# cdglissov/recurrent-flows-msc

Measured on AMD Instinct MI355X. Metric: frames/sec, RFN SM-MNIST 64x64 train step (fwd+bwd+Adam), higher is better.
Workload: dtype f32 (forward convolutions fp32-grade: fused scaled-fp16 split f16x3s / three-piece bf16x6 split; gradient convolutions bf16x3 split MFMA; fp32 accumulate everywhere); 1 GPU; RFN SM-MNIST 64x64 canonical (K=10 L=5 Hd=256 h=200 z=56), global_batch=32, seq_len=20, train step; global_batch=32, seq_len=20, parallelism=dp1

## Files before the change

include/rfn_hip.h:

```cpp
#ifndef RFN_HIP_H
#define RFN_HIP_H

#ifdef __cplusplus
extern "C" {
#endif

typedef void* rfn_stream_t;

int rfn_abi_version(void);
const char* rfn_last_error(void);

int rfn_squeeze2d_f32(const float* x, long x_ns, float* y, long y_ns, int N, int C, int H, int W, int undo,
                      rfn_stream_t stream);

int rfn_channel_stats_f32(const float* x, long x_ns, float* mean, float* var_unbiased, int N, int C, int HW,
                          rfn_stream_t stream);

int rfn_actnorm_invconv_fwd_f32(const float* x, long x_ns, const float* bias, const float* logs, const float* Wm,
                                float* z, long z_ns, int N, int C, int HW, rfn_stream_t stream);
int rfn_actnorm_invconv_bwd_f32(const float* x, long x_ns, const float* bias, const float* logs, const float* Wm,
                                const float* gz, long gz_ns, float* gx, long gx_ns, float* gW, float* gbias,
                                float* glogs, int N, int C, int HW, rfn_stream_t stream);
#define RFN_INVCONV_MAX_STEPS 32
#define RFN_INVCONV_MAX_CHANNELS 96
int rfn_invconv_weights_fwd_f32(const float* const* p, const float* const* lower, const float* const* upper,
                                const float* const* log_s, const float* const* sign_s, float* W, float* logdet, int K,
                                int C, int HW, rfn_stream_t stream);
int rfn_invconv_weights_bwd_f32(const float* const* p, const float* const* lower, const float* const* upper,
                                const float* const* log_s, const float* const* sign_s, const float* gW, const float* gc,
                                float* g_lower, float* g_upper, float* g_log_s, int K, int C, int HW, rfn_stream_t stream);
int rfn_invconv_actnorm_rev_f32(const float* z, long z_ns, const float* bias, const float* logs, const float* Winv,
                                float* x, long x_ns, int N, int C, int HW, rfn_stream_t stream);

int rfn_conv2d_fwd_f32(const float* in1, long in1_ns, int C1, const float* in2, long in2_ns, int C2,
                       const float* wpk, float* out1, long out1_ns, float* out2, long out2_ns, int Cout,
                       int cout_split, int acc1, int acc2, int N, int H, int W, int ks, int ep_mode,
                       const float* p0, const float* p1, int act, rfn_stream_t stream);
const char* rfn_conv2d_kernel_label_f32(int ks, int Cout, int N, int H, int W);

int rfn_conv2d_fwd_bf16x3(const float* in1, long in1_ns, int C1, const float* in2, long in2_ns, int C2,
                          const float* wpk, float* out1, long out1_ns, float* out2, long out2_ns, int Cout,
                          int cout_split, int acc1, int acc2, int N, int H, int W, int ks, int ep_mode,
                          const float* p0, const float* p1, int act, rfn_stream_t stream);
long rfn_packed_weight_size_bf16x3(int Cout, int Cin, int ks);
int rfn_pack_conv_weight_bf16x3(const float* w, float* wpk, int Cout, int Cin, int ks, int transpose_flip,
                                rfn_stream_t stream);
long rfn_packed_weight_size_bf16x6(int Cout, int Cin, int ks);
int rfn_pack_conv_weight_bf16x6(const float* w, float* wpk, int Cout, int Cin, int ks, int transpose_flip,
                                rfn_stream_t stream);
int rfn_conv2d_fwd_bf16x6(const float* in1, long in1_ns, int C1, const float* in2, long in2_ns, int C2,
                          const float* wpk, float* out1, long out1_ns, float* out2, long out2_ns, int Cout,
                          int cout_split, int acc1, int acc2, int N, int H, int W, int ks, int ep_mode,
                          const float* p0, const float* p1, int act, rfn_stream_t stream);
const char* rfn_conv2d_kernel_label_bf16x3(int npl, int ks, int C1, int C2, int Cout, int cout_split, int acc1,
                                          int ep_mode, int N, int H, int W);

int rfn_conv3x3_fewcin_supported(int Cin, int Cout);
int rfn_conv3x3_fewcin_fwd_f32(const float* in, long in_ns, int Cin, const float* w, float* out, long out_ns, int Cout,
                               int N, int H, int W, rfn_stream_t stream);
int rfn_conv3x3_c1_wgrad16_f32(const float* in, long in_ns, const float* g, long g_ns, float* gw, int N, int H, int W,
                               rfn_stream_t stream);

int rfn_conv2d_dgrad_act_rows_bf16x3(int N, int H, int W, int ks, int Cout, int Cin);
int rfn_conv2d_dgrad_act_bf16x3(const float* gin, long gin_ns, int Cin, const float* wpk, const float* y, long y_ns,
                                const float* logs, int act, float* out, long out_ns, float* part, int Cout, int N,
                                int H, int W, int ks, rfn_stream_t stream);

typedef struct {
    const float* w;
    float* wpk;
    int Cout, Cin, ks, mode;
} rfn_pack_desc;
int rfn_pack_conv_weights_hostdescs_bf16x3(const void* descs_host, int n, rfn_stream_t stream);

typedef struct {
    const float* w1;
    const float* w2;
    const float* w3;
    float* dst;
    int Cin, C;
} rfn_po_pack_desc;
int rfn_coupling_po_supported(int N, int C, int Cc, int Hd, int H, int W);
long rfn_coupling_po_packed_bytes(int Cin, int C);
int rfn_coupling_po_pack(const void* descs_device, int n, rfn_stream_t stream);
int rfn_coupling_po_fwd(const float* z, long z_ns, const float* cond, long cond_ns, const void* wpk, const float* n1b,
                        const float* n1l, const float* n2b, const float* n2l, float* h1, long h1_ns, float* h2,
                        long h2_ns, float* P, long P_ns, float* m1, float* m2, int N, int C, int Cc, int H, int W, int act,
                        rfn_stream_t stream);
long rfn_coupling_po_mask_floats(int N, int H, int W);
int rfn_coupling_po_bwd_supported(int N, int C, int H, int W);
long rfn_coupling_po_bwd_packed_bytes(int C);
int rfn_coupling_po_pack_bwd(const void* descs_device, int n, rfn_stream_t stream);
long rfn_coupling_po_bwd_part_floats(int N, int H, int W);
int rfn_coupling_po_bwd(const float* go, long go_ns, const void* wpk, const float* n1l, const float* n2l,
                        const float* m_h1, const float* m_h2, float* ga2, long ga2_ns, float* ga1, long ga1_ns,
                        float* part, int N, int C, int H, int W, int act, rfn_stream_t stream);
int rfn_coupling_po_bwd_finish(const float* const* part, const float* const* w1, const float* const* gw1,
                               const float* const* n1b, const float* const* w2, const float* const* gw2,
                               const float* const* n2b, float* const* out, int n, int nblk, int K1,
                               rfn_stream_t stream);

int rfn_gather_affine_f32(const float* P, const float* o_in, long o_ns, const float* b3, const float* l3, float* o_out,
                          float* z, long z_ns, const float* scale, const float* scale_shift, float* logdet,
                          int clamp_type, int N, int C, int H, int W, rfn_stream_t stream);
int rfn_affine_zeros_bwd_f32(const float* zout, long zout_ns, const float* o, long o_ns, const float* gout, long gout_ns,
                             const float* glogdet, const float* scale, const float* scale_shift, const float* l3,
                             float* gz, long gz_ns, float* gpre, long gpre_ns, float* gscale, float* gscale_shift,
                             float* gb3, float* gl3, int clamp_type, int N, int C, int HW, rfn_stream_t stream);

int rfn_glow_shell_fwd_f32(float* z, long z_ns, const float* P, const float* o_in, long o_ns, const float* b3,
                           const float* l3, float* o_out, const float* scale, const float* scale_shift, float* logdet,
                           int clamp_type, const float* bias, const float* logs, const float* Wm, float* znext,
                           long znext_ns, int ld_const, int N, int C, int H, int W, rfn_stream_t stream);
long rfn_glow_shell_fwd_ld_floats(int N, int C, int H, int W);
int rfn_logdet_reduce_f32(const float* part, int n_launch, float* logdet, int accumulate, int N, int C, int H, int W,
                          rfn_stream_t stream);
const char* rfn_glow_shell_fwd_kernel_label(int N, int C, int H, int W, int head);
const char* rfn_glow_shell_bwd_kernel_label(int N, int C, int HW, int tail);
int rfn_glow_shell_supported(int N, int C, int H, int W);
int rfn_glow_shell_bwd_f32(const float* x, long x_ns, const float* bias, const float* logs, const float* Wm,
                           const float* gz, long gz_ns, float* gW, float* gbias, float* glogs, const float* o, long o_ns,
                           const float* glogdet, const float* scale, const float* scale_shift, const float* l3,
                           float* gz_prev, long gz_prev_ns, float* gpre, long gpre_ns, float* gscale,
                           float* gscale_shift, float* gb3, float* gl3, int clamp_type, int ld_const, int N, int C,
                           int HW, rfn_stream_t stream);
int rfn_actnorm_invconv_bwd_ld_f32(const float* x, long x_ns, const float* bias, const float* logs, const float* Wm,
                                   const float* gz, long gz_ns, float* gx, long gx_ns, float* gW, float* gbias,
                                   float* glogs, const float* glogdet, int N, int C, int HW, rfn_stream_t stream);

int rfn_dgrad_small_supported(int N, int Cin, int Cout, int H, int W);
int rfn_conv3x3_smallcout_bf16x3(const float* in, long in_ns, int Cin, const float* wpk, float* out1, long out1_ns,
                                 float* out2, long out2_ns, int Cout, int cout_split, int acc1, int acc2, int N, int H,
                                 int W, rfn_stream_t stream);

int rfn_gemm_wgrad_bf16x3(const float* a, long a_ns, int M, const float* b, long b_ns, int Nc, float* gw, int F, int HW,
                          rfn_stream_t stream);
int rfn_gemm_wgrad_grouped_bf16x3(const float* const* a, long a_ns, int M, const float* const* b, long b_ns, int Nc,
                                  float* const* gw, int G, int F, int HW, rfn_stream_t stream);
const char* rfn_gemm_wgrad_kernel_label_bf16x3(int M, int Nc, long a_ns, long b_ns, int G, int F, int HW);
int rfn_conv3x3_wgrad_implicit_bf16x3(const float* g, long g_ns, int Cout, const float* in1, long in1_ns, int C1,
                                      const float* in2, long in2_ns, int C2, float* gw, int F, int H, int W,
                                      rfn_stream_t stream);
int rfn_conv3x3_wgrad_implicit_grouped_bf16x3(const float* const* g, long g_ns, int Cout, const float* const* in1,
                                              long in1_ns, int C1, const float* const* in2, long in2_ns, int C2,
                                              float* const* gw, int G, int F, int H, int W, rfn_stream_t stream);
const char* rfn_conv3x3_wgrad_implicit_kernel_label_bf16x3(int Cout, long g_ns, int G, int F, int H, int W);
int rfn_im2col3x3_f32(const float* in1, long in1_ns, int C1, const float* in2, long in2_ns, int C2, float* out, int N,
                      int H, int W, rfn_stream_t stream);

long rfn_packed_weight_size(int Cout, int Cin, int ks);
int rfn_pack_conv_weight_f32(const float* w, float* wpk, int Cout, int Cin, int ks, int transpose_flip,
                             rfn_stream_t stream);

int rfn_conv2d_wgrad_f32(const float* in1, long in1_ns, int C1, const float* in2, long in2_ns, int C2,
                         const float* g, long g_ns, int Cout, float* gwt, int N, int H, int W, int ks,
                         rfn_stream_t stream);
const char* rfn_conv2d_wgrad_kernel_label_f32(int ks, int Cin, int Cout, int H, int W);
int rfn_wgrad_finish_f32(const float* gwt, float* gw, int Cout, int Cin, int ks, int accumulate, rfn_stream_t stream);

int rfn_tap_gather_f32(const float* P, const float* bias, const float* logs, float* o, int N, int C, int H, int W,
                       rfn_stream_t stream);
int rfn_tap_scatter_f32(const float* g, float* Gs, int N, int C, int H, int W, rfn_stream_t stream);

int rfn_conv_epilogue_bwd_f32(const float* y, long y_ns, const float* gy, long gy_ns, float* gu, long gu_ns,
                              const float* logs, float* gb, float* gl, int N, int C, int HW, int ep_mode, int act,
                              rfn_stream_t stream);

int rfn_affine_coupling_f32(float* z, long z_ns, const float* o, long o_ns, const float* scale,
                            const float* scale_shift, float* logdet, int clamp_type, int reverse, int N, int C, int HW,
                            rfn_stream_t stream);
int rfn_affine_coupling_bwd_f32(const float* zout, long zout_ns, const float* o, long o_ns, const float* gout,
                                long gout_ns, const float* glogdet, const float* scale, const float* scale_shift,
                                float* gz, long gz_ns, float* go, long go_ns, float* gscale, float* gscale_shift,
                                int clamp_type, int N, int C, int HW, rfn_stream_t stream);

int rfn_gauss_logp_f32(const float* z, long z_ns, const float* o, long o_ns, float* logp, int layout, int std_mode,
                       int N, int Cz, int HW, rfn_stream_t stream);
int rfn_gauss_logp_bwd_f32(const float* z, long z_ns, const float* o, long o_ns, const float* glogp, float* gz,
                           long gz_ns, float* go, long go_ns, int layout, int std_mode, int N, int Cz, int HW,
                           rfn_stream_t stream);
int rfn_gauss_sample_f32(const float* o, long o_ns, const float* eps, float* z, long z_ns, float temperature, int layout,
                         int std_mode, int N, int Cz, int HW, rfn_stream_t stream);

int rfn_latent_step_fwd_f32(const float* enc, const float* pri, const float* eps_p, const float* eps_q, float* zt,
                            float* zxt, float* kl, float* em, float* es, int B, int ZHW, int res_q, rfn_stream_t stream);
int rfn_latent_step_bwd_f32(const float* enc, const float* pri, const float* eps_p, const float* eps_q,
                            const float* g_zt, long g_zt_ns, const float* g_zxt, long g_zxt_ns, const float* g_kl,
                            const float* g_em, const float* g_es, float* g_enc, float* g_pri, int B, int ZHW, int res_q,
                            rfn_stream_t stream);

long rfn_smallmap_packed_size(int Cout, int Cin, int H, int W, int transpose);
int rfn_smallmap_pack_bf16x3(const float* w, int Cout, int Cin, int H, int W, int transpose, float* packed,
                             rfn_stream_t stream);
typedef struct {
    const float* w;
    float* packed;
    int Cout, Cin, H, W, transpose, pad_;
} rfn_smallmap_pack_desc;
int rfn_smallmap_pack_batched_bf16x3(const void* descs_host, int n, rfn_stream_t stream);
int rfn_smallmap_dense_bf16x3(const float* a, const float* y, float slope_in, const float* packed, const float* bias,
                              const float* add, int act_out, float slope_out, float* out, float* a_out, int B, int K, int N,
                              int HW, rfn_stream_t stream);

int rfn_smallmap_dense_pair_bf16x3(const float* a0, const float* y0, float slope_in0, const float* packed0,
                                   const float* bias0, const float* add0, int act_out0, float slope_out0, float* out0,
                                   float* a_out0, int K0, int N0, const float* a1, const float* y1, float slope_in1,
                                   const float* packed1, const float* bias1, const float* add1, int act_out1,
                                   float slope_out1, float* out1, float* a_out1, int K1, int N1, int B, int HW,
                                   rfn_stream_t stream);

int rfn_smallmap_conv_bf16x3(const float* in1, long in1_ns, int C1, const float* in2, long in2_ns, int C2,
                             const float* packed, float* out1, long out1_ns, float* out2, long out2_ns, int Cout,
                             int cout_split, int acc1, int N, int H, int W, int ep_mode, const float* p0,
                             const float* p1, int act, rfn_stream_t stream);

long rfn_stepbn_scratch_floats(int S, int B, int C);
int rfn_stepbn_fwd_f32(const float* x, const float* gamma, const float* beta, float* y, float* mean, float* var, float* acc,
                       float* run_mean, float* run_var, const float* coef, const float* coef_u, float decay,
                       long long* num_batches_tracked, int S, int B, int C, int HW, float eps, int act, float slope,
                       rfn_stream_t stream);
int rfn_stepbn_bwd_f32(const float* x, const float* gamma, const float* beta, const float* g, const float* mean,
                       const float* var, float* sums, float* gx, float* ggamma, float* gbeta, int S, int B, int C, int HW,
                       float eps, int act, float slope, int stage, int world, rfn_stream_t stream);
int rfn_stepbn_apply_f32(const float* x, const float* gamma, const float* beta, float* y, const float* mean,
                         const float* var, int S, int B, int C, int HW, float eps, int act, float slope,
                         rfn_stream_t stream);
const char* rfn_stepbn_kernel_label(int S, int B, int C, int HW, int aligned, int bwd);

const char* rfn_latent_step_kernel_label(int B, int ZHW);
const char* rfn_convlstm_gates_kernel_label(int N, int Hc, int HW);
int rfn_convlstm_gates_fwd_f32(const float* cc, const float* c_prev, long c_ns, const float* Wci, const float* Wcf,
                               const float* Wco, float* h_out, long h_ns, float* c_out, long co_ns, float* gates,
                               int N, int Hc, int HW, rfn_stream_t stream);
int rfn_convlstm_gates_bwd_f32(const float* gates, const float* c_prev, long c_ns, const float* c_out, long co_ns,
                               const float* gh, long gh_ns, const float* gc_next, long gcn_ns, const float* Wci,
                               const float* Wcf, const float* Wco, float* gcc, float* gc_prev, long gcp_ns, int N,
                               int Hc, int HW, rfn_stream_t stream);

typedef struct rfn_adam_entry {
    float* p;
    const float* g;
    float* m;
    float* v;
    long n;
    int step_offset;
    int reserved;
} rfn_adam_entry;
int rfn_adam_chunk_elems(void);
int rfn_adam_step_f32(const rfn_adam_entry* table, const int* chunks, int n_chunks, double lr, double beta1, double beta2,
                      double eps, double weight_decay, int t, rfn_stream_t stream);

int rfn_frame_quality_u8(const void* a, long a_ns, const void* b, long b_ns, float* mse, float* psnr, float* ssim,
                         int N, int C, int H, int W, rfn_stream_t stream);

int rfn_moving_mnist_render_f32(const void* digits, int N, float* out, long long* traj, int B, int T, int C, int S,
                                int num_digits, int step_length, int deterministic, long seed, long split,
                                long first_id, rfn_stream_t stream);

int rfn_clip_gather_u8_f32(const void* store, long n_frames, const void* first, float* out, int B, int T, int C, int Cs,
                           int H, int W, rfn_stream_t stream);

#define RFN_SHEET_MAX_ROWS 32
typedef struct rfn_sheet_row {
    const void* ptr;
    long step;
    int kind;
    int count;
} rfn_sheet_row;
int rfn_sheet_max_rows(void);
int rfn_sheet_compose_u8(const void* rows_table, int R, int N, int C, int H, int W, int gutter, int bg, int n_bits,
                         int range_half, int lead, long out_addr, rfn_stream_t stream);

int rfn_lpips_alex_sizes(int H, int W, long long* out);
int rfn_lpips_alex_weight_layout(long long* out);
int rfn_lpips_alex_features_u8(const void* frames, long frame_stride, int N, int C, int H, int W, const float* wpack,
                               long wpack_floats, float* feats_out, float* workspace, long workspace_floats,
                               rfn_stream_t stream);
int rfn_lpips_alex_distance(const float* feats_a, const float* feats_b, const float* lin, int N, int H, int W,
                            float* per_layer_out, float* out, rfn_stream_t stream);

int rfn_i3d_same(int in, int k, int s, long long* out);
int rfn_i3d_conv_pack_dims(int Cin, int Cout, int k, long long* out);
int rfn_i3d_conv3d_f32(const float* in, long in_floats, int N, int T, int H, int W, int Cin, const float* wpack,
                       long wpack_floats, const float* bias, int Cout, int k, int stride, int relu, float* out,
                       long out_floats, int out_coff, int out_pitch, rfn_stream_t stream);
int rfn_i3d_maxpool3d_f32(const float* in, long in_floats, int N, int T, int H, int W, int C, int kt, int khw, int st,
                          int shw, float* out, long out_floats, rfn_stream_t stream);
int rfn_i3d_resize_u8(const void* frames, long frame_stride, int NF, int C, int H, int W, float* out, long out_floats,
                      rfn_stream_t stream);
int rfn_i3d_head_f32(const float* in, long in_floats, int N, int Tp, int P, int C, const float* wpack, long wpack_floats,
                     const float* bias, int Cout, float* out, rfn_stream_t stream);

#ifdef __cplusplus
}
#endif
#endif
```

recurrent-flows-msc_amd/csrc/wgrad_bf16x3.hip:

```cpp
#include "conv_common.h"

typedef __bf16 bf16x8 __attribute__((ext_vector_type(8)));

struct GemmWgradParams {
    const float* a;
    const float* b;
    long a_ns, b_ns;
    int M, N;
    float* gw;
    int F, HW;
    long total;
    int n_stages;
    const float* b2;
    long b2_ns;
    int C1, C2, H, W;
    int G, mtiles;
    const float* ga[16];
    const float* gb[16];
    const float* gb2[16];
    float* ggw[16];
};

struct WgOperands { const float* a; const float* b; const float* b2; float* gw; };
__device__ __forceinline__ WgOperands wg_operands(const GemmWgradParams& p, const int grp) {
    WgOperands o = {p.a, p.b, p.b2, p.gw};
    if (p.G > 0) {
#pragma unroll
        for (int i = 0; i < 16; ++i)
            if (i == grp) {
                o.a = p.ga[i];
                o.b = p.gb[i];
                o.b2 = p.gb2[i];
                o.gw = p.ggw[i];
            }
    }
    return o;
}

template <int WM, int WN, int TM, int TN, int KP, int IMPL = 0>
__global__ __launch_bounds__(64 * WM * WN) void gemm_wgrad_b3_kernel(const GemmWgradParams p) {
    constexpr int NT = 64 * WM * WN;
    constexpr int BM = 32 * TM * WM, BN = 32 * TN * WN;
    constexpr int NU = KP / 8;
    constexpr int RS = NU + 1;
    constexpr int AU = (BM * NU + NT - 1) / NT;
    constexpr int BU = (BN * NU + NT - 1) / NT;
    constexpr bool AX = (BM * NU) % NT == 0, BX = (BN * NU) % NT == 0;
    static_assert(WM * WN == 4 || WM * WN == 8, "tile/stage shape");
    extern __shared__ __attribute__((aligned(16))) unsigned char lds_raw[];
    bf16x8* Ah = reinterpret_cast<bf16x8*>(lds_raw);
    bf16x8* Al = Ah + BM * RS;
    bf16x8* Bh = Al + BM * RS;
    bf16x8* Bl = Bh + BN * RS;
    const int tid = threadIdx.x, lane = tid & 63, wave = tid >> 6;
    const int wm = wave / WN, wn = wave % WN;
    const int l31 = lane & 31, kk = lane >> 5;
    const int grp = p.G > 0 ? (int)blockIdx.z / p.mtiles : 0;
    const int m0 = (p.G > 0 ? (int)blockIdx.z - grp * p.mtiles : (int)blockIdx.z) * BM, n0 = blockIdx.y * BN;
    const WgOperands ops_ = wg_operands(p, grp);
    const float* const pa_ = ops_.a;
    const float* const pb_ = ops_.b;
    const float* const pb2_ = ops_.b2;
    float* const pgw_ = ops_.gw;

    f32x16 acc[TM][TN];
#pragma unroll
    for (int i = 0; i < TM; ++i)
#pragma unroll
        for (int j = 0; j < TN; ++j)
#pragma unroll
            for (int r = 0; r < 16; ++r) acc[i][j][r] = 0.f;

    float4 ast[AU][2], bst[BU][2];
    static_assert(NT % NU == 0, "k-group must be a per-thread constant");
    const int kg = tid % NU, r0 = tid / NU;
    const unsigned uHW = (unsigned)p.HW;
    bool okq[2] = {false, false};
    const float* uplane[IMPL ? BU : 1];
    long uns[IMPL ? BU : 1];
    int udy[IMPL ? BU : 1], udx[IMPL ? BU : 1];
    float bedge[IMPL ? BU : 1];
    unsigned rowmask = 0, edgemask = 0;
    if (IMPL) {
#pragma unroll
        for (int u = 0; u < BU; ++u) {
            int row = n0 + r0 + u * (NT / NU);
            if (row >= p.N) row = 0;
            const int ci = row / 9, tap = row - ci * 9;
            udy[u] = tap / 3 - 1;
            udx[u] = tap % 3 - 1;
            const bool first = ci < p.C1;
            uplane[u] = first ? pb_ + (long)ci * p.HW : pb2_ + (long)(ci - p.C1) * p.HW;
            uns[u] = first ? p.b_ns : p.b2_ns;
        }
    }
    auto prefetch = [&](int stage) {
        const unsigned q0 = (unsigned)stage * KP + 8u * kg;
        long offa[2], offb[2];
#pragma unroll
        for (int h = 0; h < 2; ++h) {
            const unsigned q = q0 + 4u * h;
            okq[h] = stage < p.n_stages && q < (unsigned)p.total;
            const unsigned qq = okq[h] ? q : 0u;
            const unsigned f = qq / uHW, px = qq - f * uHW;
            offa[h] = (long)f * p.a_ns + px;
            offb[h] = (long)f * p.b_ns + px;
        }
#pragma unroll
        for (int u = 0; u < AU; ++u) {
            const int row = m0 + r0 + u * (NT / NU);
            const float* base = pa_ + (long)(row < p.M ? row : 0) * p.HW;
#pragma unroll
            for (int h = 0; h < 2; ++h) ast[u][h] = *reinterpret_cast<const float4*>(base + offa[h]);
        }
        if (IMPL) {
            const unsigned qq = okq[0] ? q0 : 0u;
            const unsigned f = qq / uHW, pix = qq - f * uHW;
            const int y = (int)(pix / (unsigned)p.W), x0 = (int)(pix - (unsigned)y * (unsigned)p.W);
            rowmask = 0;
            edgemask = 0;
#pragma unroll
            for (int u = 0; u < BU; ++u) {
                const int yy = y + udy[u];
                const bool rok = yy >= 0 && yy < p.H;
                const float* src = uplane[u] + (long)f * uns[u] + (rok ? yy : y) * p.W + x0;
                bst[u][0] = *reinterpret_cast<const float4*>(src);
                bst[u][1] = *reinterpret_cast<const float4*>(src + 4);
                const bool eok = udx[u] < 0 ? x0 > 0 : x0 + 8 < p.W;
                bedge[u] = src[eok ? (udx[u] < 0 ? -1 : 8) : 0];
                rowmask |= (rok ? 1u : 0u) << u;
                edgemask |= (eok ? 1u : 0u) << u;
            }
        } else {
#pragma unroll
            for (int u = 0; u < BU; ++u) {
                const int row = n0 + r0 + u * (NT / NU);
                const float* base = pb_ + (long)(row < p.N ? row : 0) * p.HW;
#pragma unroll
                for (int h = 0; h < 2; ++h) bst[u][h] = *reinterpret_cast<const float4*>(base + offb[h]);
            }
        }
    };
    auto split_store_shift = [&](const float4 (&src)[2], float edge, int dx, bool okr, bool eok, bf16x8* hi_p, bf16x8* lo_p) {
        const float v[8] = {src[0].x, src[0].y, src[0].z, src[0].w, src[1].x, src[1].y, src[1].z, src[1].w};
        bf16x8 hi, lo;
#pragma unroll
        for (int c = 0; c < 8; ++c) {
            const float left = c == 0 ? (eok ? edge : 0.f) : v[c > 0 ? c - 1 : 0];
            const float right = c == 7 ? (eok ? edge : 0.f) : v[c < 7 ? c + 1 : 7];
            float x = dx < 0 ? left : (dx > 0 ? right : v[c]);
            x = (okr && okq[0]) ? x : 0.f;
            const __bf16 h = (__bf16)x;
            hi[c] = h;
            lo[c] = (__bf16)(x - (float)h);
        }
        *hi_p = hi;
        *lo_p = lo;
    };
    auto split_store = [&](const float4 (&src)[2], bool okr, bf16x8* hi_p, bf16x8* lo_p) {
        const float v[8] = {src[0].x, src[0].y, src[0].z, src[0].w, src[1].x, src[1].y, src[1].z, src[1].w};
        bf16x8 hi, lo;
#pragma unroll
        for (int c = 0; c < 8; ++c) {
            const float x = (okr && okq[c >> 2]) ? v[c] : 0.f;
            const __bf16 h = (__bf16)x;
            hi[c] = h;
            lo[c] = (__bf16)(x - (float)h);
        }
        *hi_p = hi;
        *lo_p = lo;
    };
    auto commit = [&]() {
#pragma unroll
        for (int u = 0; u < AU; ++u) {
            const int o = (r0 + u * (NT / NU)) * RS + kg;
            if (AX || r0 + u * (NT / NU) < BM) split_store(ast[u], m0 + r0 + u * (NT / NU) < p.M, Ah + o, Al + o);
        }
#pragma unroll
        for (int u = 0; u < BU; ++u) {
            const int o = (r0 + u * (NT / NU)) * RS + kg;
            if (BX || r0 + u * (NT / NU) < BN) {
                const bool okr = n0 + r0 + u * (NT / NU) < p.N;
                if (IMPL)
                    split_store_shift(bst[u], bedge[u], udx[u], okr && ((rowmask >> u) & 1u), (edgemask >> u) & 1u, Bh + o,
                                      Bl + o);
                else
                    split_store(bst[u], okr, Bh + o, Bl + o);
            }
        }
    };

    const int arow = (wm * TM * 32 + l31) * RS + kk;
    const int brow = (wn * TN * 32 + l31) * RS + kk;
    int stage = blockIdx.x;
    prefetch(stage);
    for (; stage < p.n_stages; stage += gridDim.x) {
        __syncthreads();
        commit();
        __syncthreads();
        prefetch(stage + gridDim.x);
        __builtin_amdgcn_sched_barrier(0);
#pragma unroll WM * WN == 8 && KP > 32 ? 1 : KP / 16
        for (int s = 0; s < KP / 16; ++s) {
            bf16x8 ah[TM], al[TM], bh[TN], bl[TN];
#pragma unroll
            for (int i = 0; i < TM; ++i) {
                ah[i] = Ah[arow + i * 32 * RS + 2 * s];
                al[i] = Al[arow + i * 32 * RS + 2 * s];
            }
#pragma unroll
            for (int j = 0; j < TN; ++j) {
                bh[j] = Bh[brow + j * 32 * RS + 2 * s];
                bl[j] = Bl[brow + j * 32 * RS + 2 * s];
            }
#pragma unroll
            for (int i = 0; i < TM; ++i)
#pragma unroll
                for (int j = 0; j < TN; ++j) {
                    acc[i][j] = __builtin_amdgcn_mfma_f32_32x32x16_bf16(al[i], bh[j], acc[i][j], 0, 0, 0);
                    acc[i][j] = __builtin_amdgcn_mfma_f32_32x32x16_bf16(ah[i], bl[j], acc[i][j], 0, 0, 0);
                    acc[i][j] = __builtin_amdgcn_mfma_f32_32x32x16_bf16(ah[i], bh[j], acc[i][j], 0, 0, 0);
                }
        }
    }
#pragma unroll
    for (int i = 0; i < TM; ++i)
#pragma unroll
        for (int j = 0; j < TN; ++j) {
            const int n = n0 + (wn * TN + j) * 32 + l31;
#pragma unroll
            for (int r = 0; r < 16; ++r) {
                const int m = m0 + (wm * TM + i) * 32 + (r & 3) + 8 * (r >> 2) + 4 * kk;
                if (m < p.M && n < p.N) atomicAdd(&pgw_[(long)m * p.N + n], acc[i][j][r]);
            }
        }
}

template <int N_>
__device__ __forceinline__ void wg_wait_vm() { asm volatile("s_waitcnt vmcnt(%0)" ::"n"(N_) : "memory"); }

__device__ __forceinline__ void wg_split8(const f32x4 lo4, const f32x4 hi4, bf16x8& hi, bf16x8& lo) {
    const float v[8] = {lo4[0], lo4[1], lo4[2], lo4[3], hi4[0], hi4[1], hi4[2], hi4[3]};
#pragma unroll
    for (int c = 0; c < 8; ++c) {
        const __bf16 h = (__bf16)v[c];
        hi[c] = h;
        lo[c] = (__bf16)(v[c] - (float)h);
    }
}

template <int WM, int WN, int TM, int TN, int KP, int NST>
__global__ __launch_bounds__(64 * WM * WN) void gemm_wgrad_dma_kernel(const GemmWgradParams p) {
    constexpr int NW = WM * WN;
    constexpr int BM = 32 * TM * WM, BN = 32 * TN * WN;
    constexpr int UPR = KP / 4, RPP = 64 / UPR, SWD = 16 / UPR;
    constexpr int RB = KP * 4;
    constexpr int ROWS = BM + BN, PIECES = ROWS / RPP, PPW = PIECES / NW;
    constexpr int STAGE = ROWS * RB;
    constexpr int NK = KP / 16, NU_ = NK * TM;
    static_assert(KP == 16 || KP == 32, "stage width");
    static_assert(PIECES % NW == 0 && BM % 16 == 0 && NST >= 2, "pieces shared evenly; swizzle period divides BM");
    constexpr bool LOOK = NST >= 3;
    static_assert(TM % 2 == 0 && TM >= TN + 1, "pipeline parities");
    extern __shared__ __attribute__((aligned(16))) unsigned char lds_raw[];
    const int tid = threadIdx.x, lane = tid & 63;
    const int wave = __builtin_amdgcn_readfirstlane(tid >> 6);
    const int wm = wave / WN, wn = wave % WN;
    const int l31 = lane & 31, kk = lane >> 5;
    const int grp = p.G > 0 ? (int)blockIdx.z / p.mtiles : 0;
    const int m0 = (p.G > 0 ? (int)blockIdx.z - grp * p.mtiles : (int)blockIdx.z) * BM, n0 = blockIdx.y * BN;
    const WgOperands ops_ = wg_operands(p, grp);
    const float* const pa_ = ops_.a;
    const float* const pb_ = ops_.b;
    float* const pgw_ = ops_.gw;

    f32x16 acc[TM][TN];
#pragma unroll
    for (int i = 0; i < TM; ++i)
#pragma unroll
        for (int j = 0; j < TN; ++j)
#pragma unroll
            for (int r = 0; r < 16; ++r) acc[i][j][r] = 0.f;

    const float* prow[PPW];
    bool pisa[PPW];
#pragma unroll
    for (int j = 0; j < PPW; ++j) {
        const int r = RPP * (wave + j * NW) + lane / UPR;
        const int u = (lane & (UPR - 1)) ^ ((r / SWD) & (UPR - 1));
        pisa[j] = r < BM;
        if (pisa[j]) {
            int row = m0 + r;
            row = row < p.M ? row : p.M - 1;
            prow[j] = pa_ + (long)row * p.HW + 4 * u;
        } else {
            int row = n0 + r - BM;
            row = row < p.N ? row : p.N - 1;
            prow[j] = pb_ + (long)row * p.HW + 4 * u;
        }
    }
    const unsigned uHW = (unsigned)p.HW;
    const int S = gridDim.x;
    const int nmine = (p.n_stages - (int)blockIdx.x + S - 1) / S;
    long offa = 0, offb = 0;
    auto stage_offsets = [&](int t) {
        t = t < nmine ? t : nmine - 1;
        const unsigned q0 = (unsigned)(blockIdx.x + t * S) * KP;
        const unsigned f = q0 / uHW, px = q0 - f * uHW;
        offa = (long)f * p.a_ns + px;
        offb = (long)f * p.b_ns + px;
    };
    auto piece = [&](const int j, const int slot) {
        __builtin_amdgcn_global_load_lds((const __attribute__((address_space(1))) void*)(prow[j] + (pisa[j] ? offa : offb)),
                                         (__attribute__((address_space(3))) void*)(lds_raw + slot * STAGE + (wave + j * NW) * 1024),
                                         16, 0, 0);
    };

    int aoff[TM], boff[TN];
#pragma unroll
    for (int i = 0; i < TM; ++i) {
        const int r = (wm * TM + i) * 32 + l31;
        aoff[i] = r * RB + (((2 * kk) ^ ((r / SWD) & (UPR - 1))) << 4);
    }
#pragma unroll
    for (int j = 0; j < TN; ++j) {
        const int r = BM + (wn * TN + j) * 32 + l31;
        boff[j] = r * RB + (((2 * kk) ^ ((r / SWD) & (UPR - 1))) << 4);
    }
    auto raw = [&](const unsigned char* sb, const int off, const int s_, f32x4 (&r)[2]) {
        const int o = off ^ (s_ << 6);
        r[0] = *reinterpret_cast<const f32x4*>(sb + o);
        r[1] = *reinterpret_cast<const f32x4*>(sb + (o ^ 16));
    };

#pragma unroll
    for (int t = 0; t < NST - 1; ++t) {
        stage_offsets(t);
#pragma unroll
        for (int j = 0; j < PPW; ++j) piece(j, t);
    }
    f32x4 ra[2][2], rb[TN][2];
    bf16x8 ah[2], al[2], bh[2][TN], bl[2][TN];
    auto first_fragments = [&](const unsigned char* sb0) {
#pragma unroll
        for (int j = 0; j < TN; ++j) raw(sb0, boff[j], 0, rb[j]);
        raw(sb0, aoff[0], 0, ra[0]);
        raw(sb0, aoff[1], 0, ra[1]);
#pragma unroll
        for (int j = 0; j < TN; ++j) wg_split8(rb[j][0], rb[j][1], bh[0][j], bl[0][j]);
        wg_split8(ra[0][0], ra[0][1], ah[0], al[0]);
    };
    if (LOOK) {
        wg_wait_vm<(NST - 2) * PPW>();
        __builtin_amdgcn_s_barrier();
        first_fragments(lds_raw);
    }

    int slot = 0;
    for (int it = 0; it < nmine; ++it) {
        wg_wait_vm<LOOK ? (NST - 3) * PPW : 0>();
        __builtin_amdgcn_s_barrier();
        const int nslot = slot + 1 == NST ? 0 : slot + 1;
        const int fslot = slot == 0 ? NST - 1 : slot - 1;
        const unsigned char* sb = lds_raw + slot * STAGE;
        const unsigned char* sn = lds_raw + nslot * STAGE;
        stage_offsets(it + NST - 1);
        if (!LOOK) {
#pragma unroll
            for (int j = 0; j < PPW; ++j) piece(j, fslot);
            first_fragments(sb);
        }
#pragma unroll
        for (int u = 0; u < NU_; ++u) {
            const int s_ = u / TM, i = u % TM, cur = u & 1, kb = s_ & 1;
            if (u + 2 < NU_) raw(sb, aoff[(u + 2) % TM], (u + 2) / TM, ra[cur]);
            else if (LOOK) raw(sn, aoff[(u + 2) % TM], 0, ra[cur]);
            if (i == 0) {
#pragma unroll
                for (int j = 0; j < TN; ++j) {
                    if (s_ + 1 < NK) raw(sb, boff[j], s_ + 1, rb[j]);
                    else if (LOOK) raw(sn, boff[j], 0, rb[j]);
                }
            }
            if (LOOK && u == 0) {
#pragma unroll
                for (int j = 0; j < PPW; ++j) piece(j, fslot);
            }
#pragma unroll
            for (int j = 0; j < TN; ++j) {
                acc[i][j] = __builtin_amdgcn_mfma_f32_32x32x16_bf16(al[cur], bh[kb][j], acc[i][j], 0, 0, 0);
                acc[i][j] = __builtin_amdgcn_mfma_f32_32x32x16_bf16(ah[cur], bl[kb][j], acc[i][j], 0, 0, 0);
                acc[i][j] = __builtin_amdgcn_mfma_f32_32x32x16_bf16(ah[cur], bh[kb][j], acc[i][j], 0, 0, 0);
            }
            if (LOOK || u + 1 < NU_) wg_split8(ra[cur ^ 1][0], ra[cur ^ 1][1], ah[cur ^ 1], al[cur ^ 1]);
            if (i >= 1 && i <= TN && (LOOK || s_ + 1 < NK))
                wg_split8(rb[i - 1][0], rb[i - 1][1], bh[kb ^ 1][i - 1], bl[kb ^ 1][i - 1]);
        }
        if (LOOK && (NK & 1)) {
#pragma unroll
            for (int j = 0; j < TN; ++j) {
                bh[0][j] = bh[1][j];
                bl[0][j] = bl[1][j];
            }
        }
        if (!LOOK) {
            __builtin_amdgcn_sched_group_barrier(0x020, PPW, 0);
            __builtin_amdgcn_sched_group_barrier(0x100, 2 * TN + 4, 0);
            __builtin_amdgcn_sched_group_barrier(0x002, 30 * (TN + 1), 0);
        }
#pragma unroll
        for (int g = 0; g < NU_ * TN * 3; ++g) {
            __builtin_amdgcn_sched_group_barrier(0x008, 1, 0);
            __builtin_amdgcn_sched_group_barrier(0x002, 6, 0);
            __builtin_amdgcn_sched_group_barrier(0x100, 1, 0);
            if (LOOK && g < PPW) __builtin_amdgcn_sched_group_barrier(0x020, 1, 0);
        }
        slot = nslot;
    }
    wg_wait_vm<0>();
#pragma unroll
    for (int i = 0; i < TM; ++i)
#pragma unroll
        for (int j = 0; j < TN; ++j) {
            const int n = n0 + (wn * TN + j) * 32 + l31;
#pragma unroll
            for (int r = 0; r < 16; ++r) {
                const int m = m0 + (wm * TM + i) * 32 + (r & 3) + 8 * (r >> 2) + 4 * kk;
                if (m < p.M && n < p.N) atomicAdd(&pgw_[(long)m * p.N + n], acc[i][j][r]);
            }
        }
}

template <int WM, int WN, int TM, int TN, int KP, int NST>
static void launch_gemm_wgrad_dma(GemmWgradParams& p, hipStream_t s) {
    constexpr int BM = 32 * TM * WM, BN = 32 * TN * WN;
    p.n_stages = (int)(p.total / KP);
    const size_t lds = (size_t)NST * (BM + BN) * KP * 4;
    const int tiles = ceil_div(p.M, BM) * ceil_div(p.N, BN);
    const int G = p.G > 0 ? p.G : 1;
    int S = 256 / (tiles * G);
    if (S > p.n_stages / 8) S = p.n_stages / 8;
    if (S < 1) S = 1;
    auto kern = gemm_wgrad_dma_kernel<WM, WN, TM, TN, KP, NST>;
    (void)hipFuncSetAttribute((const void*)kern, hipFuncAttributeMaxDynamicSharedMemorySize, (int)lds);
    p.mtiles = ceil_div(p.M, BM);
    dim3 grid(S, ceil_div(p.N, BN), p.mtiles * G);
    hipLaunchKernelGGL(kern, grid, dim3(64 * WM * WN), lds, s, p);
}

template <int WM, int WN, int TM, int TN>
__global__ __launch_bounds__(64 * WM * WN) void gemm_wgrad_dma_impl_kernel(const GemmWgradParams p) {
    constexpr int NW = WM * WN, NT = 64 * NW, KP = 32, NK = KP / 16;
    constexpr int BM = 32 * TM * WM, BN = 32 * TN * WN;
    constexpr int PIECES = BM / 8, PPW = PIECES / NW;
    constexpr int ASLOT = BM * 128;
    constexpr int NU = KP / 8, RS = NU + 1;
    constexpr int BU = (BN * NU + NT - 1) / NT;
    constexpr int BPLANE = BN * RS;
    static_assert(PIECES % NW == 0 && NT % NU == 0 && TM % 2 == 0, "shares / parities");
    extern __shared__ __attribute__((aligned(16))) unsigned char lds_raw[];
    bf16x8* const Bbase = reinterpret_cast<bf16x8*>(lds_raw + 2 * ASLOT);
    const int tid = threadIdx.x, lane = tid & 63;
    const int wave = __builtin_amdgcn_readfirstlane(tid >> 6);
    const int wm = wave / WN, wn = wave % WN;
    const int l31 = lane & 31, kk = lane >> 5;
    const int grp = p.G > 0 ? (int)blockIdx.z / p.mtiles : 0;
    const int m0 = (p.G > 0 ? (int)blockIdx.z - grp * p.mtiles : (int)blockIdx.z) * BM, n0 = blockIdx.y * BN;
    const WgOperands ops_ = wg_operands(p, grp);
    const float* const pa_ = ops_.a;
    const float* const pb_ = ops_.b;
    const float* const pb2_ = ops_.b2;
    float* const pgw_ = ops_.gw;

    f32x16 acc[TM][TN];
#pragma unroll
    for (int i = 0; i < TM; ++i)
#pragma unroll
        for (int j = 0; j < TN; ++j)
#pragma unroll
            for (int r = 0; r < 16; ++r) acc[i][j][r] = 0.f;

    const float* prow[PPW];
#pragma unroll
    for (int j = 0; j < PPW; ++j) {
        const int r = 8 * (wave + j * NW) + (lane >> 3);
        const int u = (lane & 7) ^ ((r >> 1) & 7);
        int row = m0 + r;
        row = row < p.M ? row : p.M - 1;
        prow[j] = pa_ + (long)row * p.HW + 4 * u;
    }
    int aoff[TM];
#pragma unroll
    for (int i = 0; i < TM; ++i) {
        const int r = (wm * TM + i) * 32 + l31;
        aoff[i] = r * 128 + (((2 * kk) ^ ((r >> 1) & 7)) << 4);
    }
    const int kg = tid % NU, r0 = tid / NU;
    const float* uplane[BU];
    long uns[BU];
    int udy[BU], udx[BU];
#pragma unroll
    for (int u = 0; u < BU; ++u) {
        int row = n0 + r0 + u * (NT / NU);
        if (row >= p.N) row = 0;
        const int ci = row / 9, tap = row - ci * 9;
        udy[u] = tap / 3 - 1;
        udx[u] = tap % 3 - 1;
        const bool first = ci < p.C1;
        uplane[u] = first ? pb_ + (long)ci * p.HW : pb2_ + (long)(ci - p.C1) * p.HW;
        uns[u] = first ? p.b_ns : p.b2_ns;
    }
    const unsigned uHW = (unsigned)p.HW;
    const int S = gridDim.x;
    const int nmine = (p.n_stages - (int)blockIdx.x + S - 1) / S;
    float4 bst[BU][2];
    float bedge[BU];
    unsigned rowmask = 0, edgemask = 0;
    auto fetch = [&](int t, const int slot) {
        t = t < nmine ? t : nmine - 1;
        const unsigned q0 = (unsigned)(blockIdx.x + t * S) * KP;
        const unsigned f = q0 / uHW, px = q0 - f * uHW;
        const long offa = (long)f * p.a_ns + px;
#pragma unroll
        for (int j = 0; j < PPW; ++j)
            __builtin_amdgcn_global_load_lds((const __attribute__((address_space(1))) void*)(prow[j] + offa),
                                             (__attribute__((address_space(3))) void*)(lds_raw + slot * ASLOT + (wave + j * NW) * 1024),
                                             16, 0, 0);
        const unsigned pix = px + 8u * kg;
        const int y = (int)(pix / (unsigned)p.W), x0 = (int)(pix - (unsigned)y * (unsigned)p.W);
        rowmask = 0;
        edgemask = 0;
#pragma unroll
        for (int u = 0; u < BU; ++u) {
            const int yy = y + udy[u];
            const bool rok = yy >= 0 && yy < p.H;
            const float* src = uplane[u] + (long)f * uns[u] + (rok ? yy : y) * p.W + x0;
            bst[u][0] = *reinterpret_cast<const float4*>(src);
            bst[u][1] = *reinterpret_cast<const float4*>(src + 4);
            const bool eok = udx[u] < 0 ? x0 > 0 : x0 + 8 < p.W;
            bedge[u] = src[eok ? (udx[u] < 0 ? -1 : 8) : 0];
            rowmask |= (rok ? 1u : 0u) << u;
            edgemask |= (eok ? 1u : 0u) << u;
        }
    };
    auto commit = [&](const int buf) {
        bf16x8* Bh = Bbase + buf * 2 * BPLANE;
        bf16x8* Bl = Bh + BPLANE;
#pragma unroll
        for (int u = 0; u < BU; ++u) {
            const int row = r0 + u * (NT / NU);
            if (row < BN) {
                const bool okr = n0 + row < p.N && ((rowmask >> u) & 1u);
                const bool eok = (edgemask >> u) & 1u;
                const float v[8] = {bst[u][0].x, bst[u][0].y, bst[u][0].z, bst[u][0].w,
                                    bst[u][1].x, bst[u][1].y, bst[u][1].z, bst[u][1].w};
                bf16x8 hi, lo;
#pragma unroll
                for (int c = 0; c < 8; ++c) {
                    const float left = c == 0 ? (eok ? bedge[u] : 0.f) : v[c > 0 ? c - 1 : 0];
                    const float right = c == 7 ? (eok ? bedge[u] : 0.f) : v[c < 7 ? c + 1 : 7];
                    float x = udx[u] < 0 ? left : (udx[u] > 0 ? right : v[c]);
                    x = okr ? x : 0.f;
                    const __bf16 h = (__bf16)x;
                    hi[c] = h;
                    lo[c] = (__bf16)(x - (float)h);
                }
                Bh[row * RS + kg] = hi;
                Bl[row * RS + kg] = lo;
            }
        }
    };
    auto rawA = [&](const unsigned char* sb, const int i, const int s_, f32x4 (&r)[2]) {
        const int o = aoff[i] ^ (s_ << 6);
        r[0] = *reinterpret_cast<const f32x4*>(sb + o);
        r[1] = *reinterpret_cast<const f32x4*>(sb + (o ^ 16));
    };
    const int brow = (wn * TN * 32 + l31) * RS + kk;

    fetch(0, 0);
    commit(0);
    int slot = 0;
    for (int it = 0; it < nmine; ++it) {
        wg_wait_vm<0>();
        asm volatile("s_waitcnt lgkmcnt(0)" ::: "memory");
        __builtin_amdgcn_s_barrier();
        fetch(it + 1, slot ^ 1);
        const unsigned char* sb = lds_raw + slot * ASLOT;
        const bf16x8* Bh = Bbase + slot * 2 * BPLANE;
        const bf16x8* Bl = Bh + BPLANE;
        f32x4 ra[2][TM][2];
        bf16x8 ah[2][TM], al[2][TM];
#pragma unroll
        for (int i = 0; i < TM; ++i) rawA(sb, i, 0, ra[0][i]);
#pragma unroll
        for (int i = 0; i < TM; ++i) wg_split8(ra[0][i][0], ra[0][i][1], ah[0][i], al[0][i]);
#pragma unroll
        for (int s_ = 0; s_ < NK; ++s_) {
            const int cur = s_ & 1;
            if (s_ + 1 < NK) {
#pragma unroll
                for (int i = 0; i < TM; ++i) rawA(sb, i, s_ + 1, ra[cur ^ 1][i]);
            }
            bf16x8 bh[TN], bl[TN];
#pragma unroll
            for (int j = 0; j < TN; ++j) {
                bh[j] = Bh[brow + j * 32 * RS + 2 * s_];
                bl[j] = Bl[brow + j * 32 * RS + 2 * s_];
            }
#pragma unroll
            for (int i = 0; i < TM; ++i)
#pragma unroll
                for (int j = 0; j < TN; ++j) {
                    acc[i][j] = __builtin_amdgcn_mfma_f32_32x32x16_bf16(al[cur][i], bh[j], acc[i][j], 0, 0, 0);
                    acc[i][j] = __builtin_amdgcn_mfma_f32_32x32x16_bf16(ah[cur][i], bl[j], acc[i][j], 0, 0, 0);
                    acc[i][j] = __builtin_amdgcn_mfma_f32_32x32x16_bf16(ah[cur][i], bh[j], acc[i][j], 0, 0, 0);
                }
            if (s_ + 1 < NK) {
#pragma unroll
                for (int i = 0; i < TM; ++i) wg_split8(ra[cur ^ 1][i][0], ra[cur ^ 1][i][1], ah[cur ^ 1][i], al[cur ^ 1][i]);
            }
        }
        commit(slot ^ 1);
        slot ^= 1;
    }
    wg_wait_vm<0>();
#pragma unroll
    for (int i = 0; i < TM; ++i)
#pragma unroll
        for (int j = 0; j < TN; ++j) {
            const int n = n0 + (wn * TN + j) * 32 + l31;
#pragma unroll
            for (int r = 0; r < 16; ++r) {
                const int m = m0 + (wm * TM + i) * 32 + (r & 3) + 8 * (r >> 2) + 4 * kk;
                if (m < p.M && n < p.N) atomicAdd(&pgw_[(long)m * p.N + n], acc[i][j][r]);
            }
        }
}

template <int WM, int WN, int TM, int TN>
static void launch_gemm_wgrad_dma_impl(GemmWgradParams& p, hipStream_t s) {
    constexpr int BM = 32 * TM * WM, BN = 32 * TN * WN;
    p.n_stages = (int)(p.total / 32);
    const size_t lds = (size_t)2 * BM * 128 + (size_t)2 * 2 * BN * 5 * 16;
    const int tiles = ceil_div(p.M, BM) * ceil_div(p.N, BN);
    const int G = p.G > 0 ? p.G : 1;
    int S = 256 / (tiles * G);
    if (S > p.n_stages / 8) S = p.n_stages / 8;
    if (S < 1) S = 1;
    auto kern = gemm_wgrad_dma_impl_kernel<WM, WN, TM, TN>;
    (void)hipFuncSetAttribute((const void*)kern, hipFuncAttributeMaxDynamicSharedMemorySize, (int)lds);
    p.mtiles = ceil_div(p.M, BM);
    dim3 grid(S, ceil_div(p.N, BN), p.mtiles * G);
    hipLaunchKernelGGL(kern, grid, dim3(64 * WM * WN), lds, s, p);
}

template <int WM, int WN, int TM, int TN, int KP, int IMPL = 0>
static void launch_gemm_wgrad(GemmWgradParams& p, hipStream_t s) {
    constexpr int BM = 32 * TM * WM, BN = 32 * TN * WN;
    p.n_stages = (int)((p.total + KP - 1) / KP);
    size_t lds = (size_t)2 * (BM + BN) * (KP / 8 + 1) * 16;
    int tiles = ceil_div(p.M, BM) * ceil_div(p.N, BN);
    static const int sdiv = getenv("RFN_WGRAD_SPLIT") ? atoi(getenv("RFN_WGRAD_SPLIT")) : 0;
    const int G = p.G > 0 ? p.G : 1;
    int S = (sdiv > 0 ? sdiv : (WM * WN == 8 ? 256 : 512)) / (tiles * G);
    if (S > p.n_stages / 4) S = p.n_stages / 4;
    if (S < 1) S = 1;
    auto kern = gemm_wgrad_b3_kernel<WM, WN, TM, TN, KP, IMPL>;
    if (lds > 65536) (void)hipFuncSetAttribute((const void*)kern, hipFuncAttributeMaxDynamicSharedMemorySize, (int)lds);
    p.mtiles = ceil_div(p.M, BM);
    dim3 grid(S, ceil_div(p.N, BN), p.mtiles * G);
    hipLaunchKernelGGL(kern, grid, dim3(64 * WM * WN), lds, s, p);
}

enum WgradB3Route { DMA_256x256, DMA_64x256, R_256x192, R_256x192_KP32, R_256x256, R_256x256_KP32, R_64x256, R_256x64,
                    R_128x128, IMPL_DMA_256x192, IMPL_256x192, IMPL_32x256, IMPL_128x128 };
static const char* const kWgradB3Labels[] = {
    "gemm_wgrad_dma_kernel<2,4,4,2,32,2>",
    "gemm_wgrad_dma_kernel<1,8,2,1,32,3>",
    "gemm_wgrad_b3_kernel<4,2,2,3,64>",
    "gemm_wgrad_b3_kernel<4,2,2,3,32>",
    "gemm_wgrad_b3_kernel<2,4,4,2,64>",
    "gemm_wgrad_b3_kernel<2,4,4,2,32>",
    "gemm_wgrad_b3_kernel<1,4,2,2,32>",
    "gemm_wgrad_b3_kernel<4,1,2,2,32>",
    "gemm_wgrad_b3_kernel<2,2,2,2,64>",
    "gemm_wgrad_dma_impl_kernel<4,2,2,3>",
    "gemm_wgrad_b3_kernel<4,2,2,3,64,1>",
    "gemm_wgrad_b3_kernel<1,4,1,2,32,1>",
    "gemm_wgrad_b3_kernel<2,2,2,2,64,1>",
};
static_assert(sizeof(kWgradB3Labels) / sizeof(kWgradB3Labels[0]) == IMPL_128x128 + 1, "one label per route");
static bool wgrad_dma_off() {
    static const int off = getenv("RFN_WGRAD_DMA") ? atoi(getenv("RFN_WGRAD_DMA")) == 0 : 0;
    return off;
}
static GemmWgradParams wgrad_shape(int M, int Nc, long a_ns, long b_ns, int G, int F, int HW) {
    GemmWgradParams p;
    memset(&p, 0, sizeof(p));
    p.M = M; p.N = Nc; p.a_ns = a_ns; p.b_ns = b_ns; p.G = G; p.F = F; p.HW = HW; p.total = (long)F * HW;
    return p;
}

static WgradB3Route choose_gemm_wgrad(const GemmWgradParams& p) {
    const int M = p.M, Nc = p.N;
    static const int variant = getenv("RFN_WGRAD_VARIANT") ? atoi(getenv("RFN_WGRAD_VARIANT")) : 0;
    if (variant == 0 && !wgrad_dma_off() && p.HW % 32 == 0 && p.total * (p.G > 0 ? p.G : 1) >= 100000 && p.total >= 2048 &&
        p.a_ns % 4 == 0 && p.b_ns % 4 == 0 && Nc > 128 && Nc % 256 == 0) {
        if (M >= 192) return DMA_256x256;
        if (M <= 64) return DMA_64x256;
    }
    if (variant != 1 && M > 128 && Nc > 128 && p.total >= 100000) {
        if (ceil_div(Nc, 192) * 192 < ceil_div(Nc, 256) * 256) return variant == 2 ? R_256x192_KP32 : R_256x192;
        return variant == 2 ? R_256x256_KP32 : R_256x256;
    }
    return M <= 64 ? R_64x256 : (Nc <= 64 ? R_256x64 : R_128x128);
}
extern "C" const char* rfn_gemm_wgrad_kernel_label_bf16x3(int M, int Nc, long a_ns, long b_ns, int G, int F, int HW) {
    return kWgradB3Labels[choose_gemm_wgrad(wgrad_shape(M, Nc, a_ns, b_ns, G, F, HW))];
}

static WgradB3Route choose_wgrad_implicit(const GemmWgradParams& p) {
    if (p.M > 128 && p.total * (p.G > 0 ? p.G : 1) >= 100000 && p.total >= 2048 && !wgrad_dma_off() && p.HW % 32 == 0 &&
        p.a_ns % 4 == 0)
        return IMPL_DMA_256x192;
    if (p.M > 128 && p.total >= 100000) return IMPL_256x192;
    return p.M <= 32 && p.G == 0 ? IMPL_32x256 : IMPL_128x128;
}
extern "C" const char* rfn_conv3x3_wgrad_implicit_kernel_label_bf16x3(int Cout, long g_ns, int G, int F, int H, int W) {
    return kWgradB3Labels[choose_wgrad_implicit(wgrad_shape(Cout, 0, g_ns, 0, G, F, H * W))];
}

static void launch_wgrad_route(GemmWgradParams& p, WgradB3Route r, hipStream_t s) {
    switch (r) {
        case DMA_256x256:      return launch_gemm_wgrad_dma<2, 4, 4, 2, 32, 2>(p, s);
        case DMA_64x256:       return launch_gemm_wgrad_dma<1, 8, 2, 1, 32, 3>(p, s);
        case R_256x192:        return launch_gemm_wgrad<4, 2, 2, 3, 64>(p, s);
        case R_256x192_KP32:   return launch_gemm_wgrad<4, 2, 2, 3, 32>(p, s);
        case R_256x256:        return launch_gemm_wgrad<2, 4, 4, 2, 64>(p, s);
        case R_256x256_KP32:   return launch_gemm_wgrad<2, 4, 4, 2, 32>(p, s);
        case R_64x256:         return launch_gemm_wgrad<1, 4, 2, 2, 32>(p, s);
        case R_256x64:         return launch_gemm_wgrad<4, 1, 2, 2, 32>(p, s);
        case R_128x128:        return launch_gemm_wgrad<2, 2, 2, 2, 64>(p, s);
        case IMPL_DMA_256x192: return launch_gemm_wgrad_dma_impl<4, 2, 2, 3>(p, s);
        case IMPL_256x192:     return launch_gemm_wgrad<4, 2, 2, 3, 64, 1>(p, s);
        case IMPL_32x256:      return launch_gemm_wgrad<1, 4, 1, 2, 32, 1>(p, s);
        case IMPL_128x128:     return launch_gemm_wgrad<2, 2, 2, 2, 64, 1>(p, s);
    }
}

extern "C" int rfn_gemm_wgrad_bf16x3(const float* a, long a_ns, int M, const float* b, long b_ns, int Nc, float* gw,
                                     int F, int HW, rfn_stream_t stream) {
    RFN_CHECK_ARG(a && b && gw && M > 0 && Nc > 0 && F >= 0 && HW > 0, -1);
    RFN_CHECK_ARG(HW % 4 == 0 && a_ns % 4 == 0 && b_ns % 4 == 0, -2);
    RFN_CHECK_ARG((((uintptr_t)a | (uintptr_t)b) & 15) == 0, -3);
    RFN_CHECK_ARG((long)F * HW < (1L << 31) - 4096, -4);
    if (F == 0) return 0;
    GemmWgradParams p;
    memset(&p, 0, sizeof(p));
    p.a = a; p.b = b; p.a_ns = a_ns; p.b_ns = b_ns; p.M = M; p.N = Nc; p.gw = gw; p.F = F; p.HW = HW;
    p.total = (long)F * HW;
    launch_wgrad_route(p, choose_gemm_wgrad(p), (hipStream_t)stream);
    RFN_LAUNCH_CHECK();
    return 0;
}

extern "C" int rfn_gemm_wgrad_grouped_bf16x3(const float* const* a, long a_ns, int M, const float* const* b, long b_ns,
                                             int Nc, float* const* gw, int G, int F, int HW, rfn_stream_t stream) {
    RFN_CHECK_ARG(a && b && gw && G >= 1 && G <= 16 && M > 0 && Nc > 0 && F >= 0 && HW > 0, -1);
    RFN_CHECK_ARG(HW % 4 == 0 && a_ns % 4 == 0 && b_ns % 4 == 0, -2);
    RFN_CHECK_ARG((long)F * HW < (1L << 31) - 4096, -4);
    if (F == 0) return 0;
    GemmWgradParams p;
    memset(&p, 0, sizeof(p));
    for (int g = 0; g < G; ++g) {
        RFN_CHECK_ARG(a[g] && b[g] && gw[g] && (((uintptr_t)a[g] | (uintptr_t)b[g]) & 15) == 0, -3);
        p.ga[g] = a[g]; p.gb[g] = b[g]; p.gb2[g] = b[g]; p.ggw[g] = gw[g];
    }
    p.G = G; p.a = a[0]; p.b = b[0]; p.gw = gw[0];
    p.a_ns = a_ns; p.b_ns = b_ns; p.M = M; p.N = Nc; p.F = F; p.HW = HW;
    p.total = (long)F * HW;
    launch_wgrad_route(p, choose_gemm_wgrad(p), (hipStream_t)stream);
    RFN_LAUNCH_CHECK();
    return 0;
}

extern "C" int rfn_conv3x3_wgrad_implicit_bf16x3(const float* g, long g_ns, int Cout, const float* in1, long in1_ns, int C1,
                                                 const float* in2, long in2_ns, int C2, float* gw, int F, int H, int W,
                                                 rfn_stream_t stream) {
    RFN_CHECK_ARG(g && in1 && gw && Cout > 0 && C1 > 0 && C2 >= 0 && (C2 == 0 || in2) && F >= 0 && H > 0 && W > 0, -1);
    RFN_CHECK_ARG(W % 8 == 0 && g_ns % 4 == 0 && in1_ns % 4 == 0 && (C2 == 0 || in2_ns % 4 == 0), -2);
    RFN_CHECK_ARG((((uintptr_t)g | (uintptr_t)in1 | (uintptr_t)(C2 ? in2 : in1)) & 15) == 0, -3);
    RFN_CHECK_ARG((long)F * H * W < (1L << 31) - 4096, -4);
    if (F == 0) return 0;
    GemmWgradParams p;
    memset(&p, 0, sizeof(p));
    p.a = g; p.a_ns = g_ns; p.M = Cout; p.b = in1; p.b_ns = in1_ns; p.b2 = C2 ? in2 : in1; p.b2_ns = C2 ? in2_ns : in1_ns;
    p.C1 = C1; p.C2 = C2; p.H = H; p.W = W; p.N = 9 * (C1 + C2); p.gw = gw; p.F = F; p.HW = H * W;
    p.total = (long)F * H * W;
    launch_wgrad_route(p, choose_wgrad_implicit(p), (hipStream_t)stream);
    RFN_LAUNCH_CHECK();
    return 0;
}

extern "C" int rfn_conv3x3_wgrad_implicit_grouped_bf16x3(const float* const* g, long g_ns, int Cout,
                                                         const float* const* in1, long in1_ns, int C1,
                                                         const float* const* in2, long in2_ns, int C2, float* const* gw,
                                                         int G, int F, int H, int W, rfn_stream_t stream) {
    RFN_CHECK_ARG(g && in1 && gw && G >= 1 && G <= 16 && Cout > 0 && C1 > 0 && C2 >= 0 && (C2 == 0 || in2) && F >= 0, -1);
    RFN_CHECK_ARG(H > 0 && W > 0 && W % 8 == 0 && g_ns % 4 == 0 && in1_ns % 4 == 0 && (C2 == 0 || in2_ns % 4 == 0), -2);
    RFN_CHECK_ARG((long)F * H * W < (1L << 31) - 4096, -4);
    if (F == 0) return 0;
    GemmWgradParams p;
    memset(&p, 0, sizeof(p));
    for (int i = 0; i < G; ++i) {
        RFN_CHECK_ARG(g[i] && in1[i] && gw[i] && (C2 == 0 || in2[i]), -3);
        RFN_CHECK_ARG((((uintptr_t)g[i] | (uintptr_t)in1[i] | (uintptr_t)(C2 ? in2[i] : in1[i])) & 15) == 0, -3);
        p.ga[i] = g[i]; p.gb[i] = in1[i]; p.gb2[i] = C2 ? in2[i] : in1[i]; p.ggw[i] = gw[i];
    }
    p.G = G; p.a = g[0]; p.b = in1[0]; p.b2 = p.gb2[0]; p.gw = gw[0];
    p.a_ns = g_ns; p.M = Cout; p.b_ns = in1_ns; p.b2_ns = C2 ? in2_ns : in1_ns;
    p.C1 = C1; p.C2 = C2; p.H = H; p.W = W; p.N = 9 * (C1 + C2); p.F = F; p.HW = H * W;
    p.total = (long)F * H * W;
    launch_wgrad_route(p, choose_wgrad_implicit(p), (hipStream_t)stream);
    RFN_LAUNCH_CHECK();
    return 0;
}

__global__ void im2col3x3_kernel(const float* __restrict__ in1, long in1_ns, int C1, const float* __restrict__ in2,
                                 long in2_ns, int C2, float* __restrict__ out, int N, int H, int W) {
    const int Cin = C1 + C2;
    const long HW = (long)H * W, total = (long)N * 9 * Cin * HW;
    for (long idx = (long)blockIdx.x * blockDim.x + threadIdx.x; idx < total; idx += (long)gridDim.x * blockDim.x) {
        const int x = (int)(idx % W);
        long r = idx / W;
        const int y = (int)(r % H);
        r /= H;
        const int tc = (int)(r % (9 * Cin));
        const long n = r / (9 * Cin);
        const int t = tc / Cin, ci = tc - t * Cin;
        const int yy = y + t / 3 - 1, xx = x + t % 3 - 1;
        float v = 0.f;
        if (yy >= 0 && yy < H && xx >= 0 && xx < W)
            v = ci < C1 ? in1[n * in1_ns + (long)ci * HW + (long)yy * W + xx]
                        : in2[n * in2_ns + (long)(ci - C1) * HW + (long)yy * W + xx];
        out[idx] = v;
    }
}
__global__ void im2col3x3_v4_kernel(const float* __restrict__ in1, long in1_ns, int C1, const float* __restrict__ in2,
                                    long in2_ns, int C2, float* __restrict__ out, int N, int H, int W) {
    const int Cin = C1 + C2, HW4 = H * W / 4, W4 = W / 4;
    const long HW = (long)H * W, total = (long)N * 9 * Cin * HW4;
    for (long idx = (long)blockIdx.x * blockDim.x + threadIdx.x; idx < total; idx += (long)gridDim.x * blockDim.x) {
        const int q = (int)(idx % HW4);
        const long r = idx / HW4;
        const int tc = (int)(r % (9 * Cin));
        const long n = r / (9 * Cin);
        const int t = tc / Cin, ci = tc - t * Cin;
        const int y = q / W4, x0 = (q - y * W4) * 4;
        const int yy = y + t / 3 - 1, dx = t % 3 - 1;
        float4 v = {0.f, 0.f, 0.f, 0.f};
        if (yy >= 0 && yy < H) {
            const float* src = (ci < C1 ? in1 + n * in1_ns + (long)ci * HW : in2 + n * in2_ns + (long)(ci - C1) * HW) +
                               (long)yy * W;
            if (dx == 0) {
                v = *reinterpret_cast<const float4*>(src + x0);
            } else {
                const float4 c = *reinterpret_cast<const float4*>(src + x0);
                if (dx < 0) {
                    v.x = x0 > 0 ? src[x0 - 1] : 0.f;
                    v.y = c.x; v.z = c.y; v.w = c.z;
                } else {
                    v.x = c.y; v.y = c.z; v.z = c.w;
                    v.w = x0 + 4 < W ? src[x0 + 4] : 0.f;
                }
            }
        }
        *reinterpret_cast<float4*>(out + idx * 4) = v;
    }
}
extern "C" int rfn_im2col3x3_f32(const float* in1, long in1_ns, int C1, const float* in2, long in2_ns, int C2,
                                 float* out, int N, int H, int W, rfn_stream_t stream) {
    RFN_CHECK_ARG(in1 && out && C1 > 0 && C2 >= 0 && (C2 == 0 || in2) && N >= 0 && H > 0 && W > 0, -1);
    if (N == 0) return 0;
    hipStream_t s = (hipStream_t)stream;
    const long HWl = (long)H * W;
    if (W % 4 == 0 && in1_ns % 4 == 0 && (C2 == 0 || in2_ns % 4 == 0) && HWl % 4 == 0 &&
        (((uintptr_t)in1 | (uintptr_t)out | (uintptr_t)(C2 ? in2 : in1)) & 15) == 0) {
        long tot4 = (long)N * 9 * (C1 + C2) * (HWl / 4);
        int grid4 = (int)((tot4 + 255) / 256 < 16384 ? (tot4 + 255) / 256 : 16384);
        hipLaunchKernelGGL(im2col3x3_v4_kernel, dim3(grid4), dim3(256), 0, s, in1, in1_ns, C1, in2, in2_ns, C2, out, N, H, W);
        RFN_LAUNCH_CHECK();
        return 0;
    }
    long tot = (long)N * 9 * (C1 + C2) * H * W;
    int grid = (int)((tot + 255) / 256 < 8192 ? (tot + 255) / 256 : 8192);
    hipLaunchKernelGGL(im2col3x3_kernel, dim3(grid), dim3(256), 0, (hipStream_t)stream, in1, in1_ns, C1, in2, in2_ns, C2,
                       out, N, H, W);
    RFN_LAUNCH_CHECK();
    return 0;
}
```

recurrent-flows-msc_amd/rfn_hip/lib.py:

```python
import ctypes
import os

import torch

_HERE = os.path.dirname(os.path.abspath(__file__))
LIB_PATH = os.path.join(_HERE, "librfn_hip.so")

_c_f = ctypes.c_void_p
_c_i = ctypes.c_int
_c_l = ctypes.c_long
_c_s = ctypes.c_void_p

SIGNATURES = {
    "rfn_abi_version": [],
    "rfn_last_error": [],
    "rfn_squeeze2d_f32": [_c_f, _c_l, _c_f, _c_l, _c_i, _c_i, _c_i, _c_i, _c_i, _c_s],
    "rfn_channel_stats_f32": [_c_f, _c_l, _c_f, _c_f, _c_i, _c_i, _c_i, _c_s],
    "rfn_actnorm_invconv_fwd_f32": [_c_f, _c_l, _c_f, _c_f, _c_f, _c_f, _c_l, _c_i, _c_i, _c_i, _c_s],
    "rfn_actnorm_invconv_bwd_f32": [_c_f, _c_l, _c_f, _c_f, _c_f, _c_f, _c_l, _c_f, _c_l, _c_f, _c_f, _c_f,
                                    _c_i, _c_i, _c_i, _c_s],
    "rfn_invconv_weights_fwd_f32": [ctypes.c_void_p] * 5 + [_c_f, _c_f, _c_i, _c_i, _c_i, _c_s],
    "rfn_invconv_weights_bwd_f32": [ctypes.c_void_p] * 5 + [_c_f, _c_f, _c_f, _c_f, _c_f, _c_i, _c_i, _c_i, _c_s],
    "rfn_invconv_actnorm_rev_f32": [_c_f, _c_l, _c_f, _c_f, _c_f, _c_f, _c_l, _c_i, _c_i, _c_i, _c_s],
    "rfn_conv2d_fwd_f32": [_c_f, _c_l, _c_i, _c_f, _c_l, _c_i, _c_f, _c_f, _c_l, _c_f, _c_l, _c_i, _c_i, _c_i, _c_i,
                           _c_i, _c_i, _c_i, _c_i, _c_i, _c_f, _c_f, _c_i, _c_s],
    "rfn_conv2d_kernel_label_f32": [_c_i] * 5,
    "rfn_conv2d_fwd_bf16x3": [_c_f, _c_l, _c_i, _c_f, _c_l, _c_i, _c_f, _c_f, _c_l, _c_f, _c_l, _c_i, _c_i, _c_i, _c_i,
                              _c_i, _c_i, _c_i, _c_i, _c_i, _c_f, _c_f, _c_i, _c_s],
    "rfn_packed_weight_size_bf16x3": [_c_i, _c_i, _c_i],
    "rfn_pack_conv_weight_bf16x3": [_c_f, _c_f, _c_i, _c_i, _c_i, _c_i, _c_s],
    "rfn_packed_weight_size_bf16x6": [_c_i, _c_i, _c_i],
    "rfn_pack_conv_weight_bf16x6": [_c_f, _c_f, _c_i, _c_i, _c_i, _c_i, _c_s],
    "rfn_conv2d_fwd_bf16x6": [_c_f, _c_l, _c_i, _c_f, _c_l, _c_i, _c_f, _c_f, _c_l, _c_f, _c_l, _c_i, _c_i, _c_i, _c_i,
                              _c_i, _c_i, _c_i, _c_i, _c_i, _c_f, _c_f, _c_i, _c_s],
    "rfn_conv2d_kernel_label_bf16x3": [_c_i] * 11,
    "rfn_conv2d_dgrad_act_rows_bf16x3": [_c_i, _c_i, _c_i, _c_i, _c_i, _c_i],
    "rfn_conv2d_dgrad_act_bf16x3": [_c_f, _c_l, _c_i, _c_f, _c_f, _c_l, _c_f, _c_i, _c_f, _c_l, _c_f, _c_i, _c_i, _c_i,
                                    _c_i, _c_i, _c_s],
    "rfn_gather_affine_f32": [_c_f, _c_f, _c_l, _c_f, _c_f, _c_f, _c_f, _c_l, _c_f, _c_f, _c_f, _c_i, _c_i, _c_i, _c_i,
                              _c_i, _c_s],
    "rfn_affine_zeros_bwd_f32": [_c_f, _c_l, _c_f, _c_l, _c_f, _c_l, _c_f, _c_f, _c_f, _c_f, _c_f, _c_l, _c_f, _c_l, _c_f,
                                 _c_f, _c_f, _c_f, _c_i, _c_i, _c_i, _c_i, _c_s],
    "rfn_glow_shell_fwd_f32": [_c_f, _c_l, _c_f, _c_f, _c_l, _c_f, _c_f, _c_f, _c_f, _c_f, _c_f, _c_i, _c_f, _c_f, _c_f,
                               _c_f, _c_l, _c_i, _c_i, _c_i, _c_i, _c_i, _c_s],
    "rfn_glow_shell_bwd_f32": [_c_f, _c_l, _c_f, _c_f, _c_f, _c_f, _c_l, _c_f, _c_f, _c_f, _c_f, _c_l, _c_f, _c_f, _c_f,
                               _c_f, _c_f, _c_l, _c_f, _c_l, _c_f, _c_f, _c_f, _c_f, _c_i, _c_i, _c_i, _c_i, _c_i, _c_s],
    "rfn_actnorm_invconv_bwd_ld_f32": [_c_f, _c_l, _c_f, _c_f, _c_f, _c_f, _c_l, _c_f, _c_l, _c_f, _c_f, _c_f, _c_f, _c_i,
                                       _c_i, _c_i, _c_s],
    "rfn_dgrad_small_supported": [_c_i, _c_i, _c_i, _c_i, _c_i],
    "rfn_conv3x3_smallcout_bf16x3": [_c_f, _c_l, _c_i, _c_f, _c_f, _c_l, _c_f, _c_l, _c_i, _c_i, _c_i, _c_i, _c_i, _c_i,
                                     _c_i, _c_s],
    "rfn_gemm_wgrad_grouped_bf16x3": [_c_f, _c_l, _c_i, _c_f, _c_l, _c_i, _c_f, _c_i, _c_i, _c_i, _c_s],
    "rfn_conv3x3_wgrad_implicit_grouped_bf16x3": [_c_f, _c_l, _c_i, _c_f, _c_l, _c_i, _c_f, _c_l, _c_i, _c_f, _c_i, _c_i,
                                                  _c_i, _c_i, _c_s],
    "rfn_coupling_po_supported": [_c_i, _c_i, _c_i, _c_i, _c_i, _c_i],
    "rfn_coupling_po_packed_bytes": [_c_i, _c_i],
    "rfn_coupling_po_pack": [_c_f, _c_i, _c_s],
    "rfn_coupling_po_fwd": [_c_f, _c_l, _c_f, _c_l, _c_f, _c_f, _c_f, _c_f, _c_f, _c_f, _c_l, _c_f, _c_l, _c_f, _c_l,
                            _c_f, _c_f, _c_i, _c_i, _c_i, _c_i, _c_i, _c_i, _c_s],
    "rfn_glow_shell_fwd_ld_floats": [_c_i, _c_i, _c_i, _c_i],
    "rfn_logdet_reduce_f32": [_c_f, _c_i, _c_f, _c_i, _c_i, _c_i, _c_i, _c_i, _c_s],
    "rfn_glow_shell_fwd_kernel_label": [_c_i] * 5,
    "rfn_glow_shell_bwd_kernel_label": [_c_i] * 4,
    "rfn_glow_shell_supported": [_c_i] * 4,
    "rfn_coupling_po_mask_floats": [_c_i, _c_i, _c_i],
    "rfn_coupling_po_bwd_supported": [_c_i, _c_i, _c_i, _c_i],
    "rfn_coupling_po_bwd_packed_bytes": [_c_i],
    "rfn_coupling_po_pack_bwd": [_c_f, _c_i, _c_s],
    "rfn_coupling_po_bwd_part_floats": [_c_i, _c_i, _c_i],
    "rfn_coupling_po_bwd": [_c_f, _c_l, _c_f, _c_f, _c_f, _c_f, _c_f, _c_f, _c_l, _c_f, _c_l, _c_f, _c_i, _c_i, _c_i, _c_i,
                            _c_i, _c_s],
    "rfn_coupling_po_bwd_finish": [ctypes.c_void_p] * 8 + [_c_i, _c_i, _c_i, _c_s],
    "rfn_gemm_wgrad_bf16x3": [_c_f, _c_l, _c_i, _c_f, _c_l, _c_i, _c_f, _c_i, _c_i, _c_s],
    "rfn_conv3x3_wgrad_implicit_bf16x3": [_c_f, _c_l, _c_i, _c_f, _c_l, _c_i, _c_f, _c_l, _c_i, _c_f, _c_i, _c_i, _c_i,
                                          _c_s],
    "rfn_gemm_wgrad_kernel_label_bf16x3": [_c_i, _c_i, _c_l, _c_l, _c_i, _c_i, _c_i],
    "rfn_conv3x3_wgrad_implicit_kernel_label_bf16x3": [_c_i, _c_l, _c_i, _c_i, _c_i, _c_i],
    "rfn_im2col3x3_f32": [_c_f, _c_l, _c_i, _c_f, _c_l, _c_i, _c_f, _c_i, _c_i, _c_i, _c_s],
    "rfn_packed_weight_size": [_c_i, _c_i, _c_i],
    "rfn_pack_conv_weight_f32": [_c_f, _c_f, _c_i, _c_i, _c_i, _c_i, _c_s],
    "rfn_conv2d_wgrad_f32": [_c_f, _c_l, _c_i, _c_f, _c_l, _c_i, _c_f, _c_l, _c_i, _c_f, _c_i, _c_i, _c_i, _c_i, _c_s],
    "rfn_conv2d_wgrad_kernel_label_f32": [_c_i] * 5,
    "rfn_wgrad_finish_f32": [_c_f, _c_f, _c_i, _c_i, _c_i, _c_i, _c_s],
    "rfn_tap_gather_f32": [_c_f, _c_f, _c_f, _c_f, _c_i, _c_i, _c_i, _c_i, _c_s],
    "rfn_tap_scatter_f32": [_c_f, _c_f, _c_i, _c_i, _c_i, _c_i, _c_s],
    "rfn_conv_epilogue_bwd_f32": [_c_f, _c_l, _c_f, _c_l, _c_f, _c_l, _c_f, _c_f, _c_f, _c_i, _c_i, _c_i, _c_i, _c_i,
                                  _c_s],
    "rfn_affine_coupling_f32": [_c_f, _c_l, _c_f, _c_l, _c_f, _c_f, _c_f, _c_i, _c_i, _c_i, _c_i, _c_i, _c_s],
    "rfn_affine_coupling_bwd_f32": [_c_f, _c_l, _c_f, _c_l, _c_f, _c_l, _c_f, _c_f, _c_f, _c_f, _c_l, _c_f, _c_l,
                                    _c_f, _c_f, _c_i, _c_i, _c_i, _c_i, _c_s],
    "rfn_gauss_logp_f32": [_c_f, _c_l, _c_f, _c_l, _c_f, _c_i, _c_i, _c_i, _c_i, _c_i, _c_s],
    "rfn_gauss_logp_bwd_f32": [_c_f, _c_l, _c_f, _c_l, _c_f, _c_f, _c_l, _c_f, _c_l, _c_i, _c_i, _c_i, _c_i, _c_i,
                               _c_s],
    "rfn_gauss_sample_f32": [_c_f, _c_l, _c_f, _c_f, _c_l, ctypes.c_float, _c_i, _c_i, _c_i, _c_i, _c_i, _c_s],
    "rfn_latent_step_fwd_f32": [_c_f, _c_f, _c_f, _c_f, _c_f, _c_f, _c_f, _c_f, _c_f, _c_i, _c_i, _c_i, _c_s],
    "rfn_latent_step_bwd_f32": [_c_f, _c_f, _c_f, _c_f, _c_f, _c_l, _c_f, _c_l, _c_f, _c_f, _c_f, _c_f, _c_f, _c_i, _c_i, _c_i,
                                _c_s],
    "rfn_conv3x3_fewcin_supported": [_c_i, _c_i],
    "rfn_conv3x3_fewcin_fwd_f32": [_c_f, _c_l, _c_i, _c_f, _c_f, _c_l, _c_i, _c_i, _c_i, _c_i, _c_s],
    "rfn_conv3x3_c1_wgrad16_f32": [_c_f, _c_l, _c_f, _c_l, _c_f, _c_i, _c_i, _c_i, _c_s],
    "rfn_smallmap_packed_size": [_c_i, _c_i, _c_i, _c_i, _c_i],
    "rfn_smallmap_pack_bf16x3": [_c_f, _c_i, _c_i, _c_i, _c_i, _c_i, _c_f, _c_s],
    "rfn_smallmap_pack_batched_bf16x3": [ctypes.c_void_p, _c_i, _c_s],
    "rfn_pack_conv_weights_hostdescs_bf16x3": [ctypes.c_void_p, _c_i, _c_s],
    "rfn_smallmap_dense_bf16x3": [_c_f, _c_f, ctypes.c_float, _c_f, _c_f, _c_f, _c_i, ctypes.c_float, _c_f, _c_f, _c_i,
                                  _c_i, _c_i, _c_i, _c_s],
    "rfn_smallmap_dense_pair_bf16x3": [_c_f, _c_f, ctypes.c_float, _c_f, _c_f, _c_f, _c_i, ctypes.c_float, _c_f, _c_f, _c_i,
                                       _c_i, _c_f, _c_f, ctypes.c_float, _c_f, _c_f, _c_f, _c_i, ctypes.c_float, _c_f, _c_f,
                                       _c_i, _c_i, _c_i, _c_i, _c_s],
    "rfn_smallmap_conv_bf16x3": [_c_f, _c_l, _c_i, _c_f, _c_l, _c_i, _c_f, _c_f, _c_l, _c_f, _c_l, _c_i, _c_i, _c_i, _c_i,
                                 _c_i, _c_i, _c_i, _c_f, _c_f, _c_i, _c_s],
    "rfn_stepbn_scratch_floats": [_c_i, _c_i, _c_i],
    "rfn_stepbn_kernel_label": [_c_i] * 6,
    "rfn_convlstm_gates_kernel_label": [_c_i] * 3,
    "rfn_latent_step_kernel_label": [_c_i] * 2,
    "rfn_stepbn_fwd_f32": [_c_f, _c_f, _c_f, _c_f, _c_f, _c_f, _c_f, _c_f, _c_f, _c_f, _c_f, ctypes.c_float, ctypes.c_void_p,
                           _c_i, _c_i, _c_i, _c_i, ctypes.c_float, _c_i, ctypes.c_float, _c_s],
    "rfn_stepbn_bwd_f32": [_c_f, _c_f, _c_f, _c_f, _c_f, _c_f, _c_f, _c_f, _c_f, _c_f, _c_i, _c_i, _c_i, _c_i, ctypes.c_float,
                           _c_i, ctypes.c_float, _c_i, _c_i, _c_s],
    "rfn_stepbn_apply_f32": [_c_f, _c_f, _c_f, _c_f, _c_f, _c_f, _c_i, _c_i, _c_i, _c_i, ctypes.c_float, _c_i, ctypes.c_float,
                             _c_s],
    "rfn_adam_chunk_elems": [],
    "rfn_adam_step_f32": [ctypes.c_void_p, ctypes.c_void_p, _c_i, ctypes.c_double, ctypes.c_double, ctypes.c_double,
                          ctypes.c_double, ctypes.c_double, _c_i, _c_s],
    "rfn_convlstm_gates_fwd_f32": [_c_f, _c_f, _c_l, _c_f, _c_f, _c_f, _c_f, _c_l, _c_f, _c_l, _c_f, _c_i, _c_i, _c_i,
                                   _c_s],
    "rfn_convlstm_gates_bwd_f32": [_c_f, _c_f, _c_l, _c_f, _c_l, _c_f, _c_l, _c_f, _c_l, _c_f, _c_f, _c_f, _c_f, _c_f,
                                   _c_l, _c_i, _c_i, _c_i, _c_s],
    "rfn_frame_quality_u8": [ctypes.c_void_p, _c_l, ctypes.c_void_p, _c_l, _c_f, _c_f, _c_f, _c_i, _c_i, _c_i, _c_i, _c_s],
    "rfn_moving_mnist_render_f32": [ctypes.c_void_p, _c_i, _c_f, ctypes.c_void_p, _c_i, _c_i, _c_i, _c_i, _c_i, _c_i, _c_i,
                                    _c_l, _c_l, _c_l, _c_s],
    "rfn_clip_gather_u8_f32": [ctypes.c_void_p, _c_l, ctypes.c_void_p, _c_f, _c_i, _c_i, _c_i, _c_i, _c_i, _c_i, _c_s],
    "rfn_sheet_max_rows": [],
    "rfn_sheet_compose_u8": [ctypes.c_void_p] + [_c_i] * 10 + [_c_l, _c_s],
    "rfn_lpips_alex_sizes": [_c_i, _c_i, ctypes.c_void_p],
    "rfn_lpips_alex_weight_layout": [ctypes.c_void_p],
    "rfn_lpips_alex_features_u8": [ctypes.c_void_p, _c_l, _c_i, _c_i, _c_i, _c_i, _c_f, _c_l, _c_f, _c_f, _c_l, _c_s],
    "rfn_lpips_alex_distance": [_c_f, _c_f, _c_f, _c_i, _c_i, _c_i, _c_f, _c_f, _c_s],
    "rfn_i3d_same": [_c_i, _c_i, _c_i, ctypes.c_void_p],
    "rfn_i3d_conv_pack_dims": [_c_i, _c_i, _c_i, ctypes.c_void_p],
    "rfn_i3d_conv3d_f32": [_c_f, _c_l, _c_i, _c_i, _c_i, _c_i, _c_i, _c_f, _c_l, _c_f, _c_i, _c_i, _c_i, _c_i, _c_f, _c_l,
                           _c_i, _c_i, _c_s],
    "rfn_i3d_maxpool3d_f32": [_c_f, _c_l, _c_i, _c_i, _c_i, _c_i, _c_i, _c_i, _c_i, _c_i, _c_i, _c_f, _c_l, _c_s],
    "rfn_i3d_resize_u8": [ctypes.c_void_p, _c_l, _c_i, _c_i, _c_i, _c_i, _c_f, _c_l, _c_s],
    "rfn_i3d_head_f32": [_c_f, _c_l, _c_i, _c_i, _c_i, _c_i, _c_f, _c_l, _c_f, _c_i, _c_f, _c_s],
}
_RESTYPES = {"rfn_last_error": ctypes.c_char_p, "rfn_conv2d_kernel_label_f32": ctypes.c_char_p,
             "rfn_conv2d_kernel_label_bf16x3": ctypes.c_char_p, "rfn_conv2d_wgrad_kernel_label_f32": ctypes.c_char_p,
             "rfn_gemm_wgrad_kernel_label_bf16x3": ctypes.c_char_p,
             "rfn_conv3x3_wgrad_implicit_kernel_label_bf16x3": ctypes.c_char_p,
             "rfn_glow_shell_fwd_kernel_label": ctypes.c_char_p, "rfn_glow_shell_bwd_kernel_label": ctypes.c_char_p,
             "rfn_stepbn_kernel_label": ctypes.c_char_p, "rfn_convlstm_gates_kernel_label": ctypes.c_char_p,
             "rfn_latent_step_kernel_label": ctypes.c_char_p,
             "rfn_stepbn_scratch_floats": ctypes.c_long, "rfn_packed_weight_size": ctypes.c_long,
             "rfn_packed_weight_size_bf16x3": ctypes.c_long, "rfn_packed_weight_size_bf16x6": ctypes.c_long,
             "rfn_smallmap_packed_size": ctypes.c_long,
             "rfn_coupling_po_packed_bytes": ctypes.c_long, "rfn_coupling_po_mask_floats": ctypes.c_long, "rfn_glow_shell_fwd_ld_floats": ctypes.c_long,
             "rfn_coupling_po_bwd_packed_bytes": ctypes.c_long, "rfn_coupling_po_bwd_part_floats": ctypes.c_long}

ABI_VERSION = 2

_lib = None


def load():
    global _lib
    if _lib is not None:
        return _lib
    if not os.path.exists(LIB_PATH):
        raise RuntimeError(
            "librfn_hip.so not found at %s — build it with `python -c 'import __graft_entry__ as g; g.build()'` "
            "or `make -C recurrent-flows-msc_amd/csrc`. There is no fallback path." % LIB_PATH)
    lib = ctypes.CDLL(LIB_PATH)
    lib.rfn_abi_version.restype = ctypes.c_int
    if lib.rfn_abi_version() != ABI_VERSION:
        raise RuntimeError("%s has ABI version %d, this package needs %d: rebuild the library (`make -C "
                           "recurrent-flows-msc_amd/csrc`)" % (LIB_PATH, lib.rfn_abi_version(), ABI_VERSION))
    for name, argtypes in SIGNATURES.items():
        fn = getattr(lib, name)
        fn.argtypes = argtypes
        fn.restype = _RESTYPES.get(name, ctypes.c_int)
    _lib = lib
    return lib


PROFILE = None


def call(name, *args, meta=None):
    lib = load()
    cur = torch.cuda.current_stream()
    stream = ctypes.c_void_p(cur.cuda_stream)
    if PROFILE is not None:
        e0, e1 = torch.cuda.Event(enable_timing=True), torch.cuda.Event(enable_timing=True)
        e0.record(cur)
        rc = getattr(lib, name)(*args, stream)
        e1.record(cur)
        PROFILE.append((name, meta, e0, e1))
    else:
        rc = getattr(lib, name)(*args, stream)
    if rc != 0:
        raise RuntimeError("%s failed (code %d): %s" % (name, rc, lib.rfn_last_error().decode()))


def ptr_array(tensors, name="tensor"):
    arr = (ctypes.c_void_p * len(tensors))(*[dev(t, name, check_contiguous=False).value for t in tensors])
    return arr


def dev(t, name="tensor", check_contiguous=True):
    if t is None:
        return None
    if not t.is_cuda:
        raise RuntimeError("rfn_hip kernels need device tensors; %s is on %s (no CPU fallback)" % (name, t.device))
    if t.dtype != torch.float32:
        raise RuntimeError("rfn_hip kernels are fp32; %s is %s" % (name, t.dtype))
    if check_contiguous and not t.is_contiguous():
        raise RuntimeError("rfn_hip kernels need dense tensors; %s has shape %s stride %s" %
                           (name, tuple(t.shape), tuple(t.stride())))
    return ctypes.c_void_p(t.data_ptr())


def frames(t, name="tensor"):
    p = dev(t, name, check_contiguous=False)
    shape, stride = t.shape, t.stride()
    exp = 1
    for d in range(t.dim() - 1, 0, -1):
        if shape[d] != 1 and stride[d] != exp:
            raise RuntimeError("%s: per-frame layout must be dense NCHW, got shape %s stride %s" %
                               (name, tuple(shape), tuple(stride)))
        exp *= shape[d]
    ns = stride[0] if shape[0] > 1 else exp
    return p, int(ns)
```

recurrent-flows-msc_amd/rfn_hip/ops.py:

```python
import collections
import ctypes
import functools

import torch

from . import lib as L

_i = ctypes.c_int
_l = ctypes.c_long

import os

CONV_PRECISION = os.environ.get("RFN_CONV_PRECISION", "mixed")


def bwd_b3():
    return CONV_PRECISION in ("bf16x3", "mixed")


MIXED_FWD = os.environ.get("RFN_MIXED_FWD", "bf16x6")


def fwd_prec(H, W):
    if CONV_PRECISION == "mixed":
# ... 101 lines not shown
    _fields_ = [("w", ctypes.c_void_p), ("wpk", ctypes.c_void_p), ("Cout", ctypes.c_int), ("Cin", ctypes.c_int),
                ("ks", ctypes.c_int), ("mode", ctypes.c_int)]


class _SmallmapPackDesc(ctypes.Structure):
    _fields_ = [("w", ctypes.c_void_p), ("packed", ctypes.c_void_p), ("Cout", ctypes.c_int), ("Cin", ctypes.c_int),
                ("H", ctypes.c_int), ("W", ctypes.c_int), ("transpose", ctypes.c_int), ("pad_", ctypes.c_int)]


class PackBatch:

    def __init__(self):
        self._conv, self._dense, self._keep = [], [], []

    def __enter__(self):
        return self

    def __exit__(self, exc_type, exc, tb):
        if exc_type is None:
            if self._conv:
                arr = (_ConvPackDesc * len(self._conv))(*self._conv)
                L.call("rfn_pack_conv_weights_hostdescs_bf16x3", ctypes.cast(arr, ctypes.c_void_p), _i(len(arr)))
            if self._dense:
                arr = (_SmallmapPackDesc * len(self._dense))(*self._dense)
                L.call("rfn_smallmap_pack_batched_bf16x3", ctypes.cast(arr, ctypes.c_void_p), _i(len(arr)))
        self._conv, self._dense, self._keep = [], [], []

    def conv(self, w, flip=False, prec=None):
        Cout, Cin, ks = int(w.shape[0]), int(w.shape[1]), int(w.shape[2])
        prec = prec if prec is not None else ("bf16x3" if bwd_b3() else "f32")
        sfx = {"bf16x3": "_bf16x3", "bf16x6": "_bf16x6", "f32": ""}[prec]
        wpk = torch.empty(getattr(L.load(), "rfn_packed_weight_size" + sfx)(Cout, Cin, ks), device=w.device,
                          dtype=torch.float32)
        wc = w.detach().contiguous()
        if prec == "f32":
            L.call("rfn_pack_conv_weight_f32", L.dev(wc, "w"), L.dev(wpk), _i(Cout), _i(Cin), _i(ks), _i(1 if flip else 0))
            return wpk
        self._conv.append(_ConvPackDesc(L.dev(wc, "w").value, wpk.data_ptr(), Cout, Cin, ks,
                                        (1 if flip else 0) + (4 if prec == "bf16x6" else 0)))
        self._keep += [wc, wpk]
        return wpk

    def dense(self, w, H, W, transpose):
        Cout, Cin = int(w.shape[0]), int(w.shape[1])
        nbytes = int(L.load().rfn_smallmap_packed_size(Cout, Cin, H, W, 1 if transpose else 0))
        buf = torch.empty(nbytes // 4, device=w.device, dtype=torch.float32)
        wc = w.detach().contiguous()
        self._dense.append(_SmallmapPackDesc(L.dev(wc, "w").value, buf.data_ptr(), Cout, Cin, int(H), int(W),
                                             1 if transpose else 0, 0))
        self._keep += [wc, buf]
        return buf


def pack_weight(w, flip=False, prec=None):
    with PackBatch() as b:
        return b.conv(w, flip, prec)


def conv2d_dgrad_act(gin, wpk_flip, y, logs, act, Cout, ks, arena=None):
    N, Cin, H, W = gin.shape
    gp, gns = L.frames(gin, "gin")
    yp, yns = L.frames(y, "y")
    gu = torch.empty((N, Cout, H, W), device=gin.device, dtype=torch.float32)
    up, uns = L.frames(gu, "gu")
    sums = _zeros(arena, 2, Cout, device=gin.device)
    L.call("rfn_conv2d_dgrad_act_bf16x3", gp, _l(gns), _i(Cin), L.dev(wpk_flip), yp, _l(yns), L.dev(logs), _i(act), up,
           _l(uns), L.dev(sums), _i(Cout), _i(N), _i(H), _i(W), _i(ks),
           meta=("conv", kernel_label("rfn_conv2d_kernel_label_bf16x3", 2, ks, Cin, 0, Cout, Cout, 0, 4, N, H, W) + "+actbwd",
                 2.0 * N * H * W * Cin * Cout * ks * ks,
                 "N%d %d->%d %dx%d k%d dgrad+actbwd" % (N, Cin, Cout, H, W, ks),
                 4.0 * (N * H * W * (Cin + 2 * Cout) + Cin * Cout * ks * ks)))
    return gu, sums[0], sums[1]


class PackPlan:

    def __init__(self, items):
        self.items = list(items)
        self.ptrs = [w.data_ptr() for w, _ in self.items]
        lib = L.load()
        self.bufs = []
        for w, mode in self.items:
            Cout, Cin, ks = int(w.shape[0]), int(w.shape[1]), int(w.shape[2])
            assert w.is_contiguous() and w.dtype == torch.float32
            lc, lk = (9 * Cout, 1) if (mode & 3) == 2 else (Cout, ks)
            size_fn = lib.rfn_packed_weight_size_bf16x6 if (mode & 4) else lib.rfn_packed_weight_size_bf16x3
            self.bufs.append(torch.empty(size_fn(lc, Cin, lk), device=w.device, dtype=torch.float32))
        self.descs = (_ConvPackDesc * len(self.items))(*[
            _ConvPackDesc(w.data_ptr(), b.data_ptr(), int(w.shape[0]), int(w.shape[1]), int(w.shape[2]), mode)
            for (w, mode), b in zip(self.items, self.bufs)])

    def valid_for(self, items):
        return (len(items) == len(self.items) and all(w.data_ptr() == p for (w, _), p in zip(items, self.ptrs))
                and all(m == m0 for (_, m), (_, m0) in zip(items, self.items)))

    def run(self):
        L.call("rfn_pack_conv_weights_hostdescs_bf16x3", ctypes.cast(self.descs, ctypes.c_void_p), _i(len(self.descs)))


def coupling_po_ok(N, C, Cc, Hd, H, W, w1, w3, any_size=False):
    if os.environ.get("RFN_COUPLING_PO") == "0" or CONV_PRECISION != "mixed":
        return False
    if tuple(w1.shape[2:]) != (3, 3) or tuple(w3.shape[2:]) != (3, 3):
        return False
    if not any_size and C // 2 + Cc > 40 and N * H * W < 128 * 128:
        return False
    return bool(L.load().rfn_coupling_po_supported(int(N), int(C), int(Cc), int(Hd), int(H), int(W)))


class POPackPlan:

    def __init__(self, nets):
        import numpy as np
        self.nets = [tuple(n) for n in nets]
        self.ptrs = [tuple(w.data_ptr() for w in n) for n in self.nets]
        dev = self.nets[0][0].device
        lib = L.load()
        rec = np.zeros(len(self.nets), dtype=np.dtype([("w1", "<u8"), ("w2", "<u8"), ("w3", "<u8"), ("dst", "<u8"),
                                                       ("Cin", "<i4"), ("C", "<i4")]))
        self.bufs = []
        for i, (w1, w2, w3) in enumerate(self.nets):
            Cin, C = int(w1.shape[1]), int(w3.shape[0])
            for w in (w1, w2, w3):
                assert w.is_contiguous() and w.dtype == torch.float32
            assert tuple(w2.shape) == (256, 256, 1, 1) and int(w1.shape[0]) == 256 and int(w3.shape[1]) == 256
            buf = torch.empty(int(lib.rfn_coupling_po_packed_bytes(Cin, C)) // 4, device=dev, dtype=torch.float32)
            self.bufs.append(buf)
            rec[i] = (w1.data_ptr(), w2.data_ptr(), w3.data_ptr(), buf.data_ptr(), Cin, C)
        self.table = torch.from_numpy(rec.view(np.uint8).copy()).to(dev)

        self.bwd_bufs = [None] * len(self.nets)
        recb = []
        for i, (w1, w2, w3) in enumerate(self.nets):
            C = int(w3.shape[0])
            if C <= 16:
                buf = torch.empty(int(lib.rfn_coupling_po_bwd_packed_bytes(C)) // 4, device=dev, dtype=torch.float32)
                self.bwd_bufs[i] = buf
                recb.append((w1.data_ptr(), w2.data_ptr(), w3.data_ptr(), buf.data_ptr(), int(w1.shape[1]), C))
        self.n_bwd = len(recb)
        if recb:
            rb = np.zeros(len(recb), dtype=rec.dtype)
            for i, r in enumerate(recb):
                rb[i] = r
            self.table_bwd = torch.from_numpy(rb.view(np.uint8).copy()).to(dev)

    def valid_for(self, nets):
        return len(nets) == len(self.nets) and all(tuple(w.data_ptr() for w in n) == p for n, p in zip(nets, self.ptrs))

    def run(self, bwd=True):
        L.call("rfn_coupling_po_pack", L._c_f(self.table.data_ptr()), _i(len(self.nets)))
        if bwd and self.n_bwd:
            L.call("rfn_coupling_po_pack_bwd", L._c_f(self.table_bwd.data_ptr()), _i(self.n_bwd))


def coupling_po_fwd(z, cond, wpk, n1b, n1l, n2b, n2l, C, act, want_masks=False):
    N, _, H, W = z.shape
    Cc = 0 if cond is None else int(cond.shape[1])
    zp, zns = L.frames(z, "z")
    cp, cns = (None, 0) if cond is None else L.frames(cond, "cond")
    h1 = torch.empty((N, 256, H, W), device=z.device, dtype=torch.float32)
    h2 = torch.empty((N, 256, H, W), device=z.device, dtype=torch.float32)
    P = torch.empty((N, 9 * C, H, W), device=z.device, dtype=torch.float32)
    Cin = C // 2 + Cc
    npx = float(N * H * W)
    masks = None
    if want_masks and act != 0:
        nm = int(L.load().rfn_coupling_po_mask_floats(N, H, W))
        masks = (torch.empty(nm, device=z.device, dtype=torch.float32), torch.empty(nm, device=z.device, dtype=torch.float32))
    m1, m2 = masks if masks is not None else (None, None)
    L.call("rfn_coupling_po_fwd", zp, _l(zns), cp, _l(cns), L.dev(wpk), L.dev(n1b), L.dev(n1l), L.dev(n2b), L.dev(n2l),
           L.dev(h1), _l(256 * H * W), L.dev(h2), _l(256 * H * W), L.dev(P), _l(9 * C * H * W), L.dev(m1), L.dev(m2),
           _i(N), _i(C), _i(Cc), _i(H), _i(W), _i(act),
           meta=("conv", "coupling_po_fwd_kernel", 2.0 * npx * (9 * Cin * 256 + 256 * 256 + 9 * C * 256),
                 "N%d %d+%d->256->256->9x%d %dx%d" % (N, C // 2, Cc, C, H, W),
                 4.0 * npx * (Cin + 512 + 9 * C + (16 if masks is not None else 0))
                 + 4.0 * (9 * Cin * 256 + 65536 + 9 * C * 256)))
    return h1, h2, P, masks


def coupling_po_bwd_ok(N, C, H, W):
    return (os.environ.get("RFN_COUPLING_PO_BWD") != "0" and CONV_PRECISION == "mixed"
            and bool(L.load().rfn_coupling_po_bwd_supported(int(N), int(C), int(H), int(W))))


def coupling_po_bwd(go, wpk_bwd, n1l, n2l, masks, act):
    N, C, H, W = go.shape
    gp, gns = L.frames(go, "go")
    ga2 = torch.empty((N, 256, H, W), device=go.device, dtype=torch.float32)
    ga1 = torch.empty((N, 256, H, W), device=go.device, dtype=torch.float32)
    part = torch.empty(int(L.load().rfn_coupling_po_bwd_part_floats(N, H, W)), device=go.device, dtype=torch.float32)
    m1, m2 = masks if masks is not None else (None, None)
    npx = float(N * H * W)
    L.call("rfn_coupling_po_bwd", gp, _l(gns), L.dev(wpk_bwd), L.dev(n1l), L.dev(n2l), L.dev(m1), L.dev(m2),
           L.dev(ga2), _l(256 * H * W), L.dev(ga1), _l(256 * H * W), L.dev(part), _i(N), _i(C), _i(H), _i(W), _i(act),
           meta=("conv", "coupling_po_bwd_kernel", 2.0 * npx * (9 * C * 256 + 256 * 256),
                 "N%d %d->256->256 %dx%d dgrad chain" % (N, C, H, W),
                 4.0 * npx * (C + 512 + (16 if masks is not None else 0)) + 4.0 * (9 * C * 256 + 65536)))
    return ga2, ga1, part


def coupling_po_bwd_finish(tickets):
    for i0 in range(0, len(tickets), 16):
        tk = tickets[i0:i0 + 16]
        cols = [L.ptr_array([t[j].detach() for t in tk], "finish") for j in range(8)]
        nblk = int(tk[0][0].numel()) // 512
        K1 = int(tk[0][1].numel()) // 256
        for t in tk:
            assert t[0].numel() == nblk * 512 and t[1].numel() == K1 * 256 and t[2].numel() == K1 * 256
            assert t[4].numel() == 65536 and t[5].numel() == 65536 and t[2].is_contiguous() and t[5].is_contiguous()
        L.call("rfn_coupling_po_bwd_finish", *cols, _i(len(tk)), _i(nblk), _i(K1),
               meta=_shell("po_bwd_finish", tk[0][7], len(tk) * (nblk * 512 + 512 * K1 + 131072 + 1024) / 1024.0))


def conv2d_raw(in1, in2, wpk, Cout, ks, ep_mode=0, p0=None, p1=None, act=0, out1=None, out2=None, cout_split=None,
               acc1=False, acc2=False, prec=None):
    N, C1, H, W = in1.shape
    C2 = 0 if in2 is None else int(in2.shape[1])
    i1p, i1ns = L.frames(in1, "in1")
    i2p, i2ns = (None, 0) if in2 is None else L.frames(in2, "in2")
    if cout_split is None:
        cout_split = Cout
    if out1 is None:
        out1 = torch.empty((N, cout_split, H, W), device=in1.device, dtype=torch.float32)
    o1p, o1ns = L.frames(out1, "out1")
    o2p, o2ns = (None, 0) if out2 is None else L.frames(out2, "out2")
    prec = prec if prec is not None else ("bf16x3" if bwd_b3() else "f32")
    fn = {"bf16x3": "rfn_conv2d_fwd_bf16x3", "bf16x6": "rfn_conv2d_fwd_bf16x6", "f32": "rfn_conv2d_fwd_f32"}[prec]
    x6 = prec == "bf16x6"
    kname = (kernel_label("rfn_conv2d_kernel_label_f32", ks, Cout, N, H, W) if prec == "f32" else
             kernel_label("rfn_conv2d_kernel_label_bf16x3", 3 if x6 else 2, ks, C1, C2, Cout, cout_split, 1 if acc1 else 0,
                          ep_mode, N, H, W) + (" x6" if x6 else ""))
    L.call(fn, i1p, _l(i1ns), _i(C1), i2p, _l(i2ns), _i(C2),
           L.dev(wpk), o1p, _l(o1ns), o2p,
           _l(o2ns), _i(Cout), _i(cout_split), _i(1 if acc1 else 0), _i(1 if acc2 else 0), _i(N), _i(H), _i(W), _i(ks),
           _i(ep_mode), L.dev(p0), L.dev(p1), _i(act),
           meta=("conv", kname,
                 2.0 * N * H * W * (C1 + C2) * Cout * ks * ks,
                 "N%d %d+%d->%d %dx%d k%d ep%d%s" % (N, C1, C2, Cout, H, W, ks, ep_mode,
                                                  "" if cout_split == Cout else " split"),
                 4.0 * (N * H * W * (C1 + C2 + Cout) + (C1 + C2) * Cout * ks * ks)))
    return out1


def gemm_wgrad(a, b, M, Nc, arena=None):
    F_, HW = int(a.shape[0]), _hw(a)
    ap, ans = L.frames(a, "a")
    bp, bns = L.frames(b, "b")
    gw = _zeros(arena, M, Nc, device=a.device)
    L.call("rfn_gemm_wgrad_bf16x3", ap, _l(ans), _i(M), bp, _l(bns), _i(Nc), L.dev(gw), _i(F_), _i(HW),
           meta=("wgrad", kernel_label("rfn_gemm_wgrad_kernel_label_bf16x3", M, Nc, ans, bns, 0, F_, HW),
                 2.0 * F_ * HW * M * Nc, "F%d %dx%d HW%d" % (F_, M, Nc, HW), 4.0 * (F_ * HW * (M + Nc) + M * Nc)))
    return gw


def conv2d_wgrad_b3(in1, in2, g, Cout, ks, arena=None):
    N, C1, H, W = in1.shape
    C2 = 0 if in2 is None else int(in2.shape[1])
    Cin = C1 + C2
    if ks == 1:
        x = in1 if in2 is None else torch.cat((in1, in2), 1)
        return gemm_wgrad(g, x, Cout, Cin, arena).view(Cout, Cin, 1, 1)
    if Cin <= Cout and W % 8 == 0 and os.environ.get("RFN_WGRAD_IMPLICIT") != "0":
        i1p, i1ns = L.frames(in1, "in1")
        i2p, i2ns = (None, 0) if in2 is None else L.frames(in2, "in2")
        gp, gns = L.frames(g, "g")
        gw = _zeros(arena, Cout, 9 * Cin, device=in1.device)
        L.call("rfn_conv3x3_wgrad_implicit_bf16x3", gp, _l(gns), _i(Cout), i1p, _l(i1ns), _i(C1), i2p, _l(i2ns), _i(C2),
               L.dev(gw), _i(N), _i(H), _i(W),
               meta=("wgrad", kernel_label("rfn_conv3x3_wgrad_implicit_kernel_label_bf16x3", Cout, gns, 0, N, H, W),
                     2.0 * N * H * W * Cout * 9 * Cin, "F%d %dx%d HW%d implicit3x3" % (N, Cout, 9 * Cin, H * W),
                     4.0 * (N * H * W * (Cout + Cin) + Cout * 9 * Cin)))
        return gw.view(Cout, Cin, 3, 3)
    if Cin <= Cout:
        i1p, i1ns = L.frames(in1, "in1")
        i2p, i2ns = (None, 0) if in2 is None else L.frames(in2, "in2")
        x9 = torch.empty((N, 9 * Cin, H, W), device=in1.device, dtype=torch.float32)
        L.call("rfn_im2col3x3_f32", i1p, _l(i1ns), _i(C1), i2p, _l(i2ns), _i(C2), L.dev(x9), _i(N), _i(H), _i(W),
               meta=_shell("im2col3x3", x9, 10.0 / 9.0))
        gw = gemm_wgrad(g, x9, Cout, 9 * Cin, arena)
        return gw.view(Cout, 9, Cin).permute(0, 2, 1).reshape(Cout, Cin, 3, 3)
    x = in1 if in2 is None else torch.cat((in1, in2), 1)
    gs = torch.empty((N, 9 * Cout, H, W), device=in1.device, dtype=torch.float32)
    L.call("rfn_tap_scatter_f32", L.dev(g.contiguous()), L.dev(gs), _i(N), _i(Cout), _i(H), _i(W),
           meta=_shell("tap_scatter", gs, 10.0 / 9.0))
    gw = gemm_wgrad(gs, x, 9 * Cout, Cin, arena)
    return gw.view(3, 3, Cout, Cin).permute(2, 3, 0, 1).contiguous()


def gemm_wgrad_grouped(a_list, b_list, M, Nc, arena=None):
    G = len(a_list)
    F_, HW = int(a_list[0].shape[0]), _hw(a_list[0])
    ans, bns = L.frames(a_list[0], "a")[1], L.frames(b_list[0], "b")[1]
    gw = _zeros(arena, G, M, Nc, device=a_list[0].device)
    pa, pb = L.ptr_array(a_list, "a"), L.ptr_array(b_list, "b")
    pg = L.ptr_array([gw[g] for g in range(G)], "gw")
    L.call("rfn_gemm_wgrad_grouped_bf16x3", pa, _l(ans), _i(M), pb, _l(bns), _i(Nc), pg, _i(G), _i(F_), _i(HW),
           meta=("wgrad", kernel_label("rfn_gemm_wgrad_kernel_label_bf16x3", M, Nc, ans, bns, G, F_,
                                       HW).replace("<", "<grouped "),
                 2.0 * G * F_ * HW * M * Nc, "G%d F%d %dx%d HW%d" % (G, F_, M, Nc, HW),
                 4.0 * G * (F_ * HW * (M + Nc) + M * Nc)))
    return gw


GROUPED_WGRAD_MAX_PIX = 100000


def conv2d_wgrad_grouped(in1_list, in2_list, g_list, Cout, ks, arena=None, g_stacked=None):
    G = len(g_list)
    N, C1, H, W = in1_list[0].shape
    has2 = in2_list is not None and in2_list[0] is not None
    C2 = int(in2_list[0].shape[1]) if has2 else 0
    Cin = C1 + C2
    dev_ = in1_list[0].device
    if ks == 1:
        xs = in1_list if not has2 else [torch.cat((a, b), 1) for a, b in zip(in1_list, in2_list)]
        gw = gemm_wgrad_grouped(g_list, xs, Cout, Cin, arena)
        return [gw[i].view(Cout, Cin, 1, 1) for i in range(G)]
    if Cin <= Cout and W % 8 == 0 and os.environ.get("RFN_WGRAD_IMPLICIT") != "0":
        gw = _zeros(arena, G, Cout, 9 * Cin, device=dev_)
        gns, i1ns = L.frames(g_list[0], "g")[1], L.frames(in1_list[0], "in1")[1]
        i2ns = L.frames(in2_list[0], "in2")[1] if has2 else 0
        pg, p1 = L.ptr_array(g_list, "g"), L.ptr_array(in1_list, "in1")
        p2 = L.ptr_array(in2_list, "in2") if has2 else None
        pw = L.ptr_array([gw[i] for i in range(G)], "gw")
        L.call("rfn_conv3x3_wgrad_implicit_grouped_bf16x3", pg, _l(gns), _i(Cout), p1, _l(i1ns), _i(C1), p2, _l(i2ns),
               _i(C2), pw, _i(G), _i(N), _i(H), _i(W),
               meta=("wgrad", kernel_label("rfn_conv3x3_wgrad_implicit_kernel_label_bf16x3", Cout, gns, G, N, H,
                                           W).replace("<", "<grouped "),
                     2.0 * G * N * H * W * Cout * 9 * Cin,
                     "G%d F%d %dx%d HW%d implicit3x3" % (G, N, Cout, 9 * Cin, H * W),
                     4.0 * G * (N * H * W * (Cout + Cin) + Cout * 9 * Cin)))
        return [gw[i].view(Cout, Cin, 3, 3) for i in range(G)]
    if Cin <= Cout:
        x9s = []
        for i in range(G):
            i1p, i1ns = L.frames(in1_list[i], "in1")
            i2p, i2ns = (None, 0) if not has2 else L.frames(in2_list[i], "in2")
            x9 = torch.empty((N, 9 * Cin, H, W), device=dev_, dtype=torch.float32)
            L.call("rfn_im2col3x3_f32", i1p, _l(i1ns), _i(C1), i2p, _l(i2ns), _i(C2), L.dev(x9), _i(N), _i(H), _i(W),
                   meta=_shell("im2col3x3", x9, 10.0 / 9.0))
            x9s.append(x9)
        gw = gemm_wgrad_grouped(g_list, x9s, Cout, 9 * Cin, arena)
        gwt = gw.view(G, Cout, 9, Cin).permute(0, 1, 3, 2).reshape(G, Cout, Cin, 3, 3)
        return [gwt[i] for i in range(G)]
    xs = in1_list if not has2 else [torch.cat((a, b), 1) for a, b in zip(in1_list, in2_list)]
    gss = []
    if g_stacked is not None and g_stacked.is_contiguous() and tuple(g_stacked.shape) == (G, N, Cout, H, W):
        gs_all = torch.empty((G, N, 9 * Cout, H, W), device=dev_, dtype=torch.float32)
        L.call("rfn_tap_scatter_f32", L.dev(g_stacked), L.dev(gs_all), _i(G * N), _i(Cout), _i(H), _i(W),
               meta=_shell("tap_scatter", gs_all, 10.0 / 9.0))
        gss = [gs_all[i] for i in range(G)]
    else:
        for i in range(G):
            gs = torch.empty((N, 9 * Cout, H, W), device=dev_, dtype=torch.float32)
            gi = g_list[i].contiguous()
            L.call("rfn_tap_scatter_f32", L.dev(gi), L.dev(gs), _i(N), _i(Cout), _i(H), _i(W),
                   meta=_shell("tap_scatter", gs, 10.0 / 9.0))
            gss.append(gs)
    gw = gemm_wgrad_grouped(gss, xs, 9 * Cout, Cin, arena)
    gwt = gw.view(G, 3, 3, Cout, Cin).permute(0, 3, 4, 1, 2).contiguous()
    return [gwt[i] for i in range(G)]


def conv2d_wgrad(in1, in2, g, Cout, ks, arena=None):
    N, C1, H, W = in1.shape
    C2 = 0 if in2 is None else int(in2.shape[1])
    Cin = C1 + C2
    if bwd_b3() and (H * W) % 4 == 0:
        return conv2d_wgrad_b3(in1, in2, g, Cout, ks, arena)
    i1p, i1ns = L.frames(in1, "in1")
    i2p, i2ns = (None, 0) if in2 is None else L.frames(in2, "in2")
    gp, gns = L.frames(g, "g")
    gwt = _zeros(arena, ks * ks, Cout, Cin, device=in1.device)
    L.call("rfn_conv2d_wgrad_f32", i1p, _l(i1ns), _i(C1), i2p, _l(i2ns), _i(C2), gp, _l(gns), _i(Cout), L.dev(gwt),
           _i(N), _i(H), _i(W), _i(ks),
           meta=("wgrad", kernel_label("rfn_conv2d_wgrad_kernel_label_f32", ks, Cin, Cout, H, W),
                 2.0 * N * H * W * Cin * Cout * ks * ks,
                 "N%d %d->%d %dx%d k%d" % (N, Cin, Cout, H, W, ks), 4.0 * (N * H * W * (Cin + Cout) + Cin * Cout * ks * ks)))
    if ks == 1:
        return gwt.view(Cout, Cin, 1, 1)
    gw = torch.empty((Cout, Cin, ks, ks), device=in1.device, dtype=torch.float32)
    L.call("rfn_wgrad_finish_f32", L.dev(gwt), L.dev(gw), _i(Cout), _i(Cin), _i(ks), _i(0), meta=_shell("wgrad_finish", gw, 2))
    return gw


TAP_MAX_COUT = 8


def zeros_conv_uses_taps(w):
    return int(w.shape[2]) == 3 and int(w.shape[0]) <= TAP_MAX_COUT


def zeros_conv_fwd(x, w, b, logs, wpk=None, prec=None):
    C, Cin, ks = int(w.shape[0]), int(w.shape[1]), int(w.shape[2])
    N, _, H, W = x.shape
    if prec is None:
        prec = fwd_prec(H, W)
    if not zeros_conv_uses_taps(w):
        return conv2d_raw(x, None, wpk if wpk is not None else pack_weight(w, prec=prec), C, ks, 2, b, logs, 0, prec=prec)
    if wpk is None:
        wpk = pack_weight(w.detach().permute(2, 3, 0, 1).reshape(9 * C, Cin, 1, 1).contiguous(), prec=prec)
    P = conv2d_raw(x, None, wpk, 9 * C, 1, prec=prec)
    o = torch.empty((N, C, H, W), device=x.device, dtype=torch.float32)
    L.call("rfn_tap_gather_f32", L.dev(P), L.dev(b), L.dev(logs), L.dev(o), _i(N), _i(C), _i(H), _i(W),
           meta=_shell("tap_gather", P, 10.0 / 9.0))
    return o


def zeros_conv_wgrad(x, g_pre, C, ks, arena=None):
    if ks != 3 or C > TAP_MAX_COUT or (bwd_b3() and _hw(x) % 4 == 0):
        return conv2d_wgrad(x, None, g_pre, C, ks, arena)
    N, Cin, H, W = x.shape
    Gs = torch.empty((N, 9 * C, H, W), device=x.device, dtype=torch.float32)
    L.call("rfn_tap_scatter_f32", L.dev(g_pre.contiguous()), L.dev(Gs), _i(N), _i(C), _i(H), _i(W),
           meta=_shell("tap_scatter", Gs, 10.0 / 9.0))
    gw = conv2d_wgrad(x, None, Gs, 9 * C, 1, arena)
    return gw.view(3, 3, C, Cin).permute(2, 3, 0, 1).contiguous()


def conv_epilogue_bwd(y, gy, logs, ep_mode, act, want_gl=True, arena=None, inplace=True):
    N, C = gy.shape[0], gy.shape[1]
    yp, yns = (None, 0) if y is None else L.frames(y, "y")
    gp, gns = L.frames(gy, "gy")
    gu = gy if inplace else torch.empty_like(gy, memory_format=torch.contiguous_format)
    up, uns = L.frames(gu, "gu")
    gbl = _zeros(arena, 2 if want_gl else 1, C, device=gy.device)
    gb, gl = gbl[0], (gbl[1] if want_gl else None)
    L.call("rfn_conv_epilogue_bwd_f32", yp, _l(yns), gp, _l(gns), up, _l(uns), L.dev(logs), L.dev(gb), L.dev(gl),
           _i(N), _i(C), _i(_hw(gy)), _i(ep_mode), _i(act), meta=_shell("conv_epilogue_bwd", gy, 3))
    return gu, gb, gl


def affine_coupling_(z, o, scale, scale_shift, logdet, clamp_type, reverse):
    N, C = z.shape[0], z.shape[1]
    zp, zns = L.frames(z, "z")
    op, ons = L.frames(o, "o")
    L.call("rfn_affine_coupling_f32", zp, _l(zns), op, _l(ons), L.dev(scale), L.dev(scale_shift), L.dev(logdet),
           _i(clamp_type), _i(1 if reverse else 0), _i(N), _i(C), _i(_hw(z)), meta=_shell("affine_coupling", z, 2))


def gather_affine_(z, o, P, b3, l3, scale, scale_shift, clamp_type):
    N, C, H, W = z.shape
    zp, zns = L.frames(z, "z")
    dlogdet = torch.empty(N, device=z.device, dtype=torch.float32)
    if P is not None:
        o = torch.empty((N, C, H, W), device=z.device, dtype=torch.float32)
        L.call("rfn_gather_affine_f32", L.dev(P), None, _l(0), L.dev(b3), L.dev(l3), L.dev(o), zp, _l(zns), L.dev(scale),
               L.dev(scale_shift), L.dev(dlogdet), _i(clamp_type), _i(N), _i(C), _i(H), _i(W),
               meta=_shell("gather_affine", z, 9 + 1 + 1))
    else:
        op, ons = L.frames(o, "o")
        L.call("rfn_gather_affine_f32", None, op, _l(ons), None, None, None, zp, _l(zns), L.dev(scale),
               L.dev(scale_shift), L.dev(dlogdet), _i(clamp_type), _i(N), _i(C), _i(H), _i(W),
               meta=_shell("gather_affine", z, 2))
    return o, dlogdet


def gauss_logp(z, o, layout, std_mode):
    N, Cz = z.shape[0], z.shape[1]
    zp, zns = L.frames(z, "z")
    op, ons = L.frames(o, "o")
    logp = torch.zeros(N, device=z.device, dtype=torch.float32)
    L.call("rfn_gauss_logp_f32", zp, _l(zns), op, _l(ons), L.dev(logp), _i(layout), _i(std_mode), _i(N), _i(Cz),
           _i(_hw(z)), meta=_shell("gauss_logp", z, 3))
    return logp


def gauss_sample(o, eps, layout, std_mode, temperature):
    N, C2 = o.shape[0], o.shape[1]
    Cz = C2 // 2
    z = torch.empty((N, Cz) + tuple(o.shape[2:]), device=o.device, dtype=torch.float32)
    op, ons = L.frames(o, "o")
    zp, zns = L.frames(z, "z")
    L.call("rfn_gauss_sample_f32", op, _l(ons), L.dev(eps.contiguous(), "eps"), zp, _l(zns),
           ctypes.c_float(float(temperature)), _i(layout), _i(std_mode), _i(N), _i(Cz), _i(_hw(o)))
    return z


class Squeeze2dFn(torch.autograd.Function):

    @staticmethod
    def forward(ctx, x, undo):
        ctx.undo = undo
        return squeeze2d_raw(x, undo)

    @staticmethod
    def backward(ctx, g):
        return squeeze2d_raw(g.contiguous(), not ctx.undo), None


def fewcin_ok(in1, in2, w, ep_mode):
    return (in2 is None and ep_mode == 0 and tuple(w.shape[2:]) == (3, 3) and os.environ.get("RFN_FEWCIN") != "0"
            and bool(L.load().rfn_conv3x3_fewcin_supported(int(w.shape[1]), int(w.shape[0]))))


def conv3x3_fewcin(x, w):
    N, Cin, H, W = x.shape
    Cout = int(w.shape[0])
    xp, xns = L.frames(x, "x")
    out = torch.empty((N, Cout, H, W), device=x.device, dtype=torch.float32)
    wc = w.detach().contiguous()
    L.call("rfn_conv3x3_fewcin_fwd_f32", xp, _l(xns), _i(Cin), L.dev(wc), L.dev(out), _l(Cout * H * W), _i(Cout), _i(N),
           _i(H), _i(W), meta=_shell("conv3x3_fewcin_fwd", out, 1.0 + Cin / Cout))
    return out


def conv3x3_c1_wgrad16(x, g):
    N, _, H, W = x.shape
    xp, xns = L.frames(x, "x")
    gp, gns = L.frames(g, "g")
    gw = torch.zeros((16, 1, 3, 3), device=x.device, dtype=torch.float32)
    L.call("rfn_conv3x3_c1_wgrad16_f32", xp, _l(xns), gp, _l(gns), L.dev(gw), _i(N), _i(H), _i(W),
           meta=_shell("conv3x3_c1_wgrad", g, 1.0 + 1.0 / 16))
    return gw


class ConvFn(torch.autograd.Function):

    @staticmethod
    def forward(ctx, in1, in2, w, p0, p1, ep_mode, act, prec=None, packs=None):
        Cout, ks = int(w.shape[0]), int(w.shape[2])
        ctx.pk_b = None if packs is None else packs[1]
        p0f = None if p0 is None else p0.detach().reshape(-1).contiguous()
        p1f = None if p1 is None else p1.detach().reshape(-1).contiguous()
        fp = prec if prec is not None else fwd_prec(int(in1.shape[2]), int(in1.shape[3]))
        if fewcin_ok(in1, in2, w, ep_mode):
            y = conv3x3_fewcin(in1, w)
        else:
            y = conv2d_raw(in1, in2, packs[0] if packs is not None and packs[0] is not None else pack_weight(w, prec=fp),
                           Cout, ks, ep_mode, p0f, p1f, act, prec=fp)
        ctx.save_for_backward(in1, in2, w, p1f, y)
        ctx.cfg = (ep_mode, act, None if p0 is None else p0.shape, None if p1 is None else p1.shape)
        return y

    @staticmethod
    def backward(ctx, gy):
        in1, in2, w, p1f, y = ctx.saved_tensors
        ep_mode, act, p0shape, p1shape = ctx.cfg
        Cout, Cin, ks = int(w.shape[0]), int(w.shape[1]), int(w.shape[2])
        gy = gy.contiguous()
        gp0 = gp1 = None
        if ep_mode != 0:
            gy, gb, gl = conv_epilogue_bwd(y if ep_mode != 3 else None, gy, p1f, ep_mode, act, ep_mode != 3, inplace=False)
            gp0 = gb.view(p0shape)
            gp1 = gl.view(p1shape) if gl is not None else None
        g1 = g2 = gw = None
        C1 = int(in1.shape[1])
        need1, need2 = ctx.needs_input_grad[0], in2 is not None and ctx.needs_input_grad[1]
        if need1 or need2:
            wt = ctx.pk_b if ctx.pk_b is not None else pack_weight(w, flip=True)
            N, _, H, W = in1.shape
            g1 = torch.empty(in1.shape, device=gy.device, dtype=torch.float32)
            if in2 is not None:
                g2 = torch.empty(in2.shape, device=gy.device, dtype=torch.float32)
            conv2d_raw(gy, None, wt, Cin, ks, 0, None, None, 0, out1=g1, out2=g2, cout_split=C1)
        if ctx.needs_input_grad[2]:
            if fewcin_ok(in1, in2, w, ep_mode) and Cin == 1 and Cout == 16:
                gw = conv3x3_c1_wgrad16(in1, gy)
            else:
                gw = conv2d_wgrad(in1, in2, gy, Cout, ks)
        return g1, g2, gw, gp0, gp1, None, None, None, None


def conv_ep(in1, in2, w, p0, p1, ep_mode, act, prec=None, packs=None):
    return ConvFn.apply(in1, in2, w, p0, p1, ep_mode, act, prec, packs)


def _f(t):
    return None if t is None else t.detach().reshape(-1).contiguous()


StepPacks = collections.namedtuple("StepPacks", ["w1_fwd", "w1_dgrad", "w2_fwd", "w2_dgrad", "w3_fwd", "w3_dgrad",
                                                 "po_fwd", "po_bwd", "w1_dense_fwd", "w3_dense_fwd", "w1_dense_dgrad"],
                                   defaults=(None,) * 11)


def dgrad_small_ok(N, Cin, Cout, H, W, ks):
    return (ks == 3 and bwd_b3() and os.environ.get("RFN_DGRAD_SMALL") != "0"
            and bool(L.load().rfn_dgrad_small_supported(int(N), int(Cin), int(Cout), int(H), int(W))))


def conv3x3_smallcout(x, wpk, Cout, out1, out2=None, cout_split=None, acc1=False, acc2=False):
    N, Cin, H, W = x.shape
    if cout_split is None:
        cout_split = Cout
    xp, xns = L.frames(x, "x")
    o1p, o1ns = L.frames(out1, "out1")
    o2p, o2ns = (None, 0) if out2 is None else L.frames(out2, "out2")
    L.call("rfn_conv3x3_smallcout_bf16x3", xp, _l(xns), _i(Cin), L.dev(wpk), o1p, _l(o1ns), o2p, _l(o2ns), _i(Cout),
           _i(cout_split), _i(1 if acc1 else 0), _i(1 if acc2 else 0), _i(N), _i(H), _i(W),
           meta=("conv", "dgrad_small_kernel", 2.0 * N * H * W * Cin * Cout * 9,
                 "N%d %d->%d %dx%d k3 dgrad" % (N, Cin, Cout, H, W), 4.0 * (N * H * W * (Cin + Cout) + Cin * Cout * 9)))
    return out1


def _net_fwd(z, cond, w1, n1b, n1l, w2, n2b, n2l, w3, b3, l3, act, pk, want_masks=False):
    N, C, H, W = z.shape
    Ch = C // 2
    Hd = int(w1.shape[0])
    z1 = z[:, :Ch]
    cin2 = cond if cond.shape[1] > 0 else None
    Cc_ = 0 if cin2 is None else int(cin2.shape[1])
    k33 = int(w1.shape[2]) == 3 and int(w3.shape[2]) == 3
    fp = fwd_prec(H, W)
    if coupling_po_ok(N, C, Cc_, Hd, H, W, w1, w3) and int(w2.shape[2]) == 1:
        po = pk.po_fwd
        if po is None:
            plan = POPackPlan([(w1.detach(), w2.detach(), w3.detach())])
            plan.run()
            po = plan.bufs[0]
        want = want_masks and pk.po_bwd is not None and coupling_po_bwd_ok(N, C, H, W)
        h1, h2, P, masks = coupling_po_fwd(z, cin2, po, _f(n1b), _f(n1l), _f(n2b), _f(n2l), C, act, want_masks=want)
        return h1, h2, None, P, masks
    dense = k33 and smallmap_conv_ok(H, W, Ch, Cc_, Hd, N)
    dense3 = k33 and smallmap_conv_ok(H, W, Hd, 0, C, N) and not zeros_conv_uses_taps(w3)
    b3fwd = fp in ("bf16x3", "bf16x6")
    if dense:
        h1 = smallmap_conv(z1, cin2, pk.w1_dense_fwd if pk.w1_dense_fwd is not None else smallmap_pack(w1, H, W, False),
                           Hd, 1, _f(n1b), _f(n1l), act)
    else:
        h1 = conv2d_raw(z1, cin2, pk.w1_fwd if (pk.w1_fwd is not None and b3fwd) else pack_weight(w1, prec=fp), Hd,
                        int(w1.shape[2]), 1, _f(n1b), _f(n1l), act, prec=fp)
    h2 = conv2d_raw(h1, None, pk.w2_fwd if (pk.w2_fwd is not None and b3fwd) else pack_weight(w2, prec=fp), Hd,
                    int(w2.shape[2]), 1, _f(n2b), _f(n2l), act, prec=fp)
    if dense3:
        o = smallmap_conv(h2, None, pk.w3_dense_fwd if pk.w3_dense_fwd is not None else smallmap_pack(w3, H, W, False), C, 2,
                          _f(b3), _f(l3), 0)
    else:
        o = zeros_conv_fwd(h2, w3, _f(b3), _f(l3), pk.w3_fwd if b3fwd else None, prec=fp)
    return h1, h2, o, None, None


def _net_bwd(go, out, cond, h1, h2, w1, n1l, w2, n2l, w3, act, pk, arena, gz, gcond, acc_cond, defer=None,
             n1b=None, n2b=None, masks=None, fin=None):
    N, C, H, W = out.shape
    Ch = C // 2
    Hd = int(w1.shape[0])
    Cc = int(cond.shape[1])
    k1, k2, k3 = int(w1.shape[2]), int(w2.shape[2]), int(w3.shape[2])
    dfr = defer is not None and bwd_b3() and Hd % 64 == 0 and _hw(h2) % 4 == 0
    gw3 = None if dfr else zeros_conv_wgrad(h2, go, C, k3, arena)
    fused = (pk.po_bwd is not None and (masks is not None or act == 0) and n1b is not None and n2b is not None
             and k2 == 1 and k1 == 3 and k3 == 3 and Hd == 256 and coupling_po_bwd_ok(N, C, H, W))
    w3f, w2f = pk.w3_dgrad, pk.w2_dgrad
    if not fused and (w3f is None or w2f is None):
        with PackBatch() as b:
            w3f = w3f if w3f is not None else b.conv(w3, True)
            w2f = w2f if w2f is not None else b.conv(w2, True)
    if fused:
        gh2, gh1, part = coupling_po_bwd(go.contiguous(), pk.po_bwd, _f(n1l), _f(n2l), masks, act)
        gw2 = None if dfr else conv2d_wgrad(h1, None, gh2, Hd, k2, arena)
        o4 = torch.empty((4, 256), device=go.device, dtype=torch.float32)
        gn1b, gn1l, gn2b, gn2l = o4[0], o4[1], o4[2], o4[3]
    elif bwd_b3() and Hd % 64 == 0:
        gh2, gn2b, gn2l = conv2d_dgrad_act(go, w3f, h2, _f(n2l), act, Hd, k3, arena)
        gw2 = None if dfr else conv2d_wgrad(h1, None, gh2, Hd, k2, arena)
        gh1, gn1b, gn1l = conv2d_dgrad_act(gh2, w2f, h1, _f(n1l), act, Hd, k2, arena)
    else:
        gh2 = conv2d_raw(go, None, w3f, Hd, k3)
        gh2, gn2b, gn2l = conv_epilogue_bwd(h2, gh2, _f(n2l), 1, act, arena=arena)
        gw2 = conv2d_wgrad(h1, None, gh2, Hd, k2, arena)
        gh1 = conv2d_raw(gh2, None, w2f, Hd, k2)
        gh1, gn1b, gn1l = conv_epilogue_bwd(h1, gh1, _f(n1l), 1, act, arena=arena)
    z1 = out[:, :Ch]
    has_cond = Cc > 0
    gw1 = None if dfr else conv2d_wgrad(z1, cond if has_cond else None, gh1, Hd, k1, arena)
    if fused:
        ticket = [part, w1, gw1, _f(n1b), w2, gw2, _f(n2b), o4]
        if fin is not None:
            fin.append(ticket)
        else:
            assert not dfr
            coupling_po_bwd_finish([ticket])
    if dfr:
        defer["w3"].append((h2, go))
        defer["w2"].append((h1, gh2))
        defer["w1"].append((z1, cond if has_cond else None, gh1))
    if k1 == 3 and k3 == 3 and smallmap_conv_ok(H, W, Hd, 0, Ch + Cc, N, bwd=True):
        smallmap_conv(gh1, None, pk.w1_dense_dgrad if pk.w1_dense_dgrad is not None else smallmap_pack(w1, H, W, True),
                      Ch + Cc, 0, out1=gz[:, :Ch], out2=gcond if has_cond else None, cout_split=Ch, acc1=True,
                      acc2=acc_cond)
    elif dgrad_small_ok(N, Hd, Ch + Cc, H, W, k1):
        conv3x3_smallcout(gh1, pk.w1_dgrad if pk.w1_dgrad is not None else pack_weight(w1, True), Ch + Cc, gz[:, :Ch],
                          gcond if has_cond else None, Ch, True, acc_cond)
    else:
        conv2d_raw(gh1, None, pk.w1_dgrad if pk.w1_dgrad is not None else pack_weight(w1, True), Ch + Cc, k1, 0,
                   None, None, 0, out1=gz[:, :Ch], out2=gcond if has_cond else None, cout_split=Ch, acc1=True,
                   acc2=acc_cond)
    return gw1, gn1b, gn1l, gw2, gn2b, gn2l, gw3


def _net_arena_numel(C, Cc, Hd, k1, k2, k3):
    Ch = C // 2
    return (2 * Ch + 8 + 3 * 2 * (Hd + 4) + 2 * (C + 4) + k1 * k1 * Hd * (Ch + Cc) + k2 * k2 * Hd * Hd
            + max(k3 * k3 * C * Hd, 9 * C * Hd) + C * C + 2 * C + 64)


def _affine_zeros_bwd(out, o, gout, gdl, scale, scale_shift, l3, clamp_type, arena, go=None):
    N, C, H, W = out.shape
    Ch, HW = C // 2, H * W
    gz = torch.empty_like(gout)
    if go is None:
        go = torch.empty_like(o)
    gscale = gshift = None
    if clamp_type == 0:
        gscale = arena.take(Ch)
        gshift = arena.take(Ch)
    gb3 = arena.take(C)
    gl3 = arena.take(C)
    op, ons = L.frames(o, "o")
    outp, outns = L.frames(out, "out")
    gop, gons = L.frames(gout, "gout")
    gzp, gzns = L.frames(gz, "gz")
    gonp, gonns = L.frames(go, "go")
    scf, shf, l3f = _f(scale), _f(scale_shift), _f(l3)
    L.call("rfn_affine_zeros_bwd_f32", outp, _l(outns), op, _l(ons), gop, _l(gons), L.dev(gdl), L.dev(scf),
           L.dev(shf), L.dev(l3f), gzp, _l(gzns), gonp, _l(gonns), L.dev(gscale), L.dev(gshift), L.dev(gb3),
           L.dev(gl3), _i(clamp_type), _i(N), _i(C), _i(HW), meta=_shell("affine_zeros_bwd", gout, 4.5))
    return gz, go, gscale, gshift, gb3, gl3


class GlowStepFn(torch.autograd.Function):

    @staticmethod
    def forward(ctx, x, cond, Wm, an_bias, an_logs, w1, n1b, n1l, w2, n2b, n2l, w3, b3, l3, scale, scale_shift,
                act, clamp_type, packs=None):
        out = actnorm_invconv_fwd(x, _f(an_bias), _f(an_logs), Wm.detach())
        pk = StepPacks(*packs) if packs is not None else StepPacks()
        ctx.packs = pk
        h1, h2, o, P, masks = _net_fwd(out, cond, w1, n1b, n1l, w2, n2b, n2l, w3, b3, l3, act, pk,
                                       want_masks=any(ctx.needs_input_grad))
        o, dlogdet = gather_affine_(out, o, P, _f(b3), _f(l3), _f(scale), _f(scale_shift), clamp_type)
        ctx.save_for_backward(x, cond, Wm, an_bias, an_logs, w1, n1l, w2, n2l, w3, l3, scale, scale_shift, out, h1, h2, o,
                              n1b, n2b, *(masks if masks is not None else ()))
        ctx.cfg = (act, clamp_type)
        return out, dlogdet

    @staticmethod
    def backward(ctx, gout, gdl):
        (x, cond, Wm, an_bias, an_logs, w1, n1l, w2, n2l, w3, l3, scale, scale_shift, out, h1, h2, o, n1b, n2b) = ctx.saved_tensors[:19]
        masks = tuple(ctx.saved_tensors[19:21]) if len(ctx.saved_tensors) > 19 else None
        act, clamp_type = ctx.cfg
        N, C, H, W = x.shape
        gout = gout.contiguous()
        gdl = None if gdl is None else gdl.contiguous()
        Cc = int(cond.shape[1])
        k1, k2, k3 = int(w1.shape[2]), int(w2.shape[2]), int(w3.shape[2])
        arena = ZeroArena(_net_arena_numel(C, Cc, int(w1.shape[0]), k1, k2, k3), x.device)
        gz, go, gscale, gshift, gb3, gl3 = _affine_zeros_bwd(out, o, gout, gdl, scale, scale_shift, l3, clamp_type, arena)
        gcond = torch.empty_like(cond) if Cc > 0 else torch.zeros_like(cond)
        gw1, gn1b, gn1l, gw2, gn2b, gn2l, gw3 = _net_bwd(go, out, cond, h1, h2, w1, n1l, w2, n2l, w3, act, ctx.packs,
                                                         arena, gz, gcond, False, n1b=n1b, n2b=n2b, masks=masks)
        gx, gW, gab, gal = actnorm_invconv_bwd(x, _f(an_bias), _f(an_logs), Wm.detach(), gz, arena)
        return (gx, gcond, gW, gab.view(an_bias.shape), gal.view(an_logs.shape), gw1, gn1b.view(1, -1, 1, 1),
                gn1l.view(n1l.shape), gw2, gn2b.view(1, -1, 1, 1), gn2l.view(n2l.shape), gw3, gb3, gl3.view(l3.shape),
                None if gscale is None else gscale.view(scale.shape),
                None if gshift is None else gshift.view(scale_shift.shape), None, None, None)


STEP_NPARAM = 13


class GlowLevelFn(torch.autograd.Function):

    @staticmethod
    def forward(ctx, x, cond, Wst, act, clamp_type, packs, *flat):
        Kn = int(Wst.shape[0])
        assert len(flat) == STEP_NPARAM * Kn
        N, C, H, W = x.shape
        if not L.load().rfn_glow_shell_supported(N, C, H, W):
            raise RuntimeError("GlowLevelFn: a flow level of C=%d channels on %dx%d maps does not fit the shell kernels "
                               "(C must be even and at most 144: rfn_glow_shell_supported)" % (C, H, W))
        prm = [flat[STEP_NPARAM * k:STEP_NPARAM * (k + 1)] for k in range(Kn)]
        pks = [StepPacks(*packs[k]) if packs is not None and packs[k] is not None else StepPacks() for k in range(Kn)]
        want_masks = any(ctx.needs_input_grad)
        Wd = Wst.detach().contiguous()
        ldf = int(L.load().rfn_glow_shell_fwd_ld_floats(N, C, H, W))
        ldp = torch.empty((Kn + 1, ldf), device=x.device, dtype=torch.float32)
        dl = torch.empty(N, device=x.device, dtype=torch.float32)
        xp, xns = L.frames(x, "x")
        z = torch.empty_like(x)
        zp, zns = L.frames(z, "z")
        ab0, al0 = _f(prm[0][0]), _f(prm[0][1])
        L.call("rfn_glow_shell_fwd_f32", xp, _l(xns), None, None, _l(0), None, None, None, None, None, L.dev(ldp[0]), _i(0),
               L.dev(ab0), L.dev(al0), L.dev(Wd[0]), zp, _l(zns), _i(1), _i(N), _i(C), _i(H), _i(W),
               meta=_shell("glow_shell_fwd", x, 2))
        outs, h1s, h2s, os_, mks = [], [], [], [], []
        for k in range(Kn):
            (_, _, w1, n1b, n1l, w2, n2b, n2l, w3, b3, l3, scale, scale_shift) = prm[k]
            h1, h2, o, P, masks = _net_fwd(z, cond, w1, n1b, n1l, w2, n2b, n2l, w3, b3, l3, act, pks[k], want_masks)
            mks.append(masks)
            last = k == Kn - 1
            zn = None if last else torch.empty_like(z)
            znp, znns = (None, 0) if last else L.frames(zn, "znext")
            hold = [_f(b3), _f(l3), _f(scale), _f(scale_shift)] + ([None, None] if last else [_f(prm[k + 1][0]), _f(prm[k + 1][1])])
            zp, zns = L.frames(z, "z")
            if P is not None:
                o = torch.empty((N, C, H, W), device=x.device, dtype=torch.float32)
                args = (L.dev(P), None, _l(0), L.dev(hold[0]), L.dev(hold[1]), L.dev(o))
                nt = 12 + (0 if last else 1)
            else:
                op, ons = L.frames(o, "o")
                args = (None, op, _l(ons), None, None, None)
                nt = 2 + (0 if last else 1.5)
            L.call("rfn_glow_shell_fwd_f32", zp, _l(zns), *args, L.dev(hold[2]), L.dev(hold[3]), L.dev(ldp[k + 1]),
                   _i(clamp_type), L.dev(hold[4]), L.dev(hold[5]), None if last else L.dev(Wd[k + 1]), znp, _l(znns),
                   _i(0 if last else 1), _i(N), _i(C), _i(H), _i(W), meta=_shell("glow_shell_fwd", z, nt))
            outs.append(z)
            h1s.append(h1)
            h2s.append(h2)
            os_.append(o)
            z = zn
        L.call("rfn_logdet_reduce_f32", L.dev(ldp), _i(Kn + 1), L.dev(dl), _i(0), _i(N), _i(C), _i(H), _i(W),
               meta=_shell("logdet_reduce", ldp, 1))
        has_masks = all(m is not None for m in mks)
        ctx.save_for_backward(x, cond, Wst, *flat, *outs, *h1s, *h2s, *os_,
                              *([m[0] for m in mks] + [m[1] for m in mks] if has_masks else []))
        ctx.cfg = (act, clamp_type, Kn, pks, has_masks)
        return outs[-1], dl

    @staticmethod
    def backward(ctx, gout, gdl):
        act, clamp_type, Kn, pks, has_masks = ctx.cfg
        sv = ctx.saved_tensors
        x, cond, Wst = sv[0], sv[1], sv[2]
        nf = STEP_NPARAM * Kn
        flat = sv[3:3 + nf]
        rest = sv[3 + nf:]
        outs, h1s, h2s, os_ = (rest[i * Kn:(i + 1) * Kn] for i in range(4))
        mks = [(rest[4 * Kn + k], rest[5 * Kn + k]) for k in range(Kn)] if has_masks else [None] * Kn
        fin = []
        prm = [flat[STEP_NPARAM * k:STEP_NPARAM * (k + 1)] for k in range(Kn)]
        N, C, H, W = x.shape
        Ch, HW = C // 2, H * W
        Cc = int(cond.shape[1])
        gout = gout.contiguous()
        gdl = None if gdl is None else gdl.contiguous()
        Wd = Wst.detach().contiguous()
        w1 = prm[0][2]
        k1, k2, k3 = int(prm[0][2].shape[2]), int(prm[0][5].shape[2]), int(prm[0][8].shape[2])
        arena = ZeroArena(Kn * _net_arena_numel(C, Cc, int(w1.shape[0]), k1, k2, k3), x.device)
        gWst = arena.take(Kn, C, C)
        gcond = torch.empty_like(cond) if Cc > 0 else torch.zeros_like(cond)
        grads = [None] * nf
        (_, _, _, _, _, _, _, _, _, _, l3, scale, scale_shift) = prm[Kn - 1]
        go_all = (torch.empty((Kn,) + tuple(os_[0].shape), device=x.device, dtype=torch.float32)
                  if (N * HW <= GROUPED_WGRAD_MAX_PIX and 1 < Kn <= 16 and os.environ.get("RFN_WGRAD_GROUPED") != "0")
                  else None)
        gz, go, gscale, gshift, gb3, gl3 = _affine_zeros_bwd(outs[Kn - 1], os_[Kn - 1], gout, gdl, scale, scale_shift, l3,
                                                            clamp_type, arena, None if go_all is None else go_all[Kn - 1])
        gx = None
        defer = ({"w1": [], "w2": [], "w3": []}
                 if (N * HW <= GROUPED_WGRAD_MAX_PIX and 1 < Kn <= 16 and os.environ.get("RFN_WGRAD_GROUPED") != "0")
                 else None)
        for k in range(Kn - 1, -1, -1):
            (an_bias, an_logs, w1, n1b, n1l, w2, n2b, n2l, w3, b3, l3, scale, scale_shift) = prm[k]
            nfin = len(fin)
            gw1, gn1b, gn1l, gw2, gn2b, gn2l, gw3 = _net_bwd(go, outs[k], cond, h1s[k], h2s[k], w1, n1l, w2, n2l, w3, act,
                                                             pks[k], arena, gz, gcond, k != Kn - 1, defer,
                                                             n1b=n1b, n2b=n2b, masks=mks[k], fin=fin)
            if len(fin) > nfin:
                fin[-1].append(k)
            base = STEP_NPARAM * k
            grads[base + 2:base + 13] = [gw1, gn1b.view(1, -1, 1, 1), gn1l.view(n1l.shape), gw2, gn2b.view(1, -1, 1, 1),
                                         gn2l.view(n2l.shape), gw3, gb3, gl3.view(l3.shape),
                                         None if gscale is None else gscale.view(scale.shape),
                                         None if gshift is None else gshift.view(scale_shift.shape)]
            gab, gal = arena.take(C), arena.take(C)
            grads[base], grads[base + 1] = gab.view(an_bias.shape), gal.view(an_logs.shape)
            abf, alf = _f(an_bias), _f(an_logs)
            gzp, gzns = L.frames(gz, "gz")
            if k == 0:
                gx = torch.empty_like(x)
                xp, xns = L.frames(x, "x")
                gxp, gxns = L.frames(gx, "gx")
                L.call("rfn_actnorm_invconv_bwd_ld_f32", xp, _l(xns), L.dev(abf), L.dev(alf), L.dev(Wd[0]), gzp, _l(gzns),
                       gxp, _l(gxns), L.dev(gWst[0]), L.dev(gab), L.dev(gal), L.dev(gdl), _i(N), _i(C), _i(HW),
                       meta=_shell("actnorm_invconv_bwd", x, 3))
                break
            (_, _, _, _, _, _, _, _, _, _, l3p, scalep, shiftp) = prm[k - 1]
            xin, op_ = outs[k - 1], os_[k - 1]
            gzn = torch.empty_like(gz)
            gon = torch.empty_like(op_) if go_all is None else go_all[k - 1]
            gscale = gshift = None
            if clamp_type == 0:
                gscale, gshift = arena.take(Ch), arena.take(Ch)
            gb3, gl3 = arena.take(C), arena.take(C)
            xp, xns = L.frames(xin, "x")
            opp, ons = L.frames(op_, "o")
            gznp, gznns = L.frames(gzn, "gz_prev")
            gonp, gonns = L.frames(gon, "gpre")
            hold = [_f(scalep), _f(shiftp), _f(l3p)]
            L.call("rfn_glow_shell_bwd_f32", xp, _l(xns), L.dev(abf), L.dev(alf), L.dev(Wd[k]), gzp, _l(gzns),
                   L.dev(gWst[k]), L.dev(gab), L.dev(gal), opp, _l(ons), L.dev(gdl), L.dev(hold[0]), L.dev(hold[1]),
                   L.dev(hold[2]), gznp, _l(gznns), gonp, _l(gonns), L.dev(gscale), L.dev(gshift), L.dev(gb3),
                   L.dev(gl3), _i(clamp_type), _i(1), _i(N), _i(C), _i(HW), meta=_shell("glow_shell_bwd", xin, 5.5))
            gz, go = gzn, gon
        if defer is not None and defer["w2"]:
            for key in ("w1", "w2", "w3"):
                defer[key].reverse()
            Hd_ = int(prm[0][2].shape[0])
            g1 = conv2d_wgrad_grouped([t[0] for t in defer["w1"]],
                                      None if defer["w1"][0][1] is None else [t[1] for t in defer["w1"]],
                                      [t[2] for t in defer["w1"]], Hd_, k1, arena)
            g2 = conv2d_wgrad_grouped([t[0] for t in defer["w2"]], None, [t[1] for t in defer["w2"]], Hd_, k2, arena)
            g3 = conv2d_wgrad_grouped([t[0] for t in defer["w3"]], None, [t[1] for t in defer["w3"]], C, k3, arena,
                                      g_stacked=go_all)
            for k in range(Kn):
                base = STEP_NPARAM * k
                grads[base + 2], grads[base + 5], grads[base + 8] = g1[k], g2[k], g3[k]
        if fin:
            for t in fin:
                base = STEP_NPARAM * t.pop()
                t[2], t[5] = grads[base + 2], grads[base + 5]
            coupling_po_bwd_finish(fin)
        return (gx, gcond, gWst, None, None, None) + tuple(grads)


class GlowStepRevFn(torch.autograd.Function):

    @staticmethod
    def forward(ctx, x, cond, Winv, an_bias, an_logs, w1, n1b, n1l, w2, n2b, n2l, w3, b3, l3, scale, scale_shift,
                act, clamp_type, pkcache=None):
        N, C, H, W = x.shape
        Ch = C // 2
        Hd = int(w1.shape[0])
        f = lambda t: None if t is None else t.detach().reshape(-1).contiguous()
        z = x.detach().clone()
        cin2 = cond if cond.shape[1] > 0 else None
        fp = fwd_prec(H, W)
        Cc_ = 0 if cin2 is None else int(cin2.shape[1])
        pkc = pkcache if pkcache is not None else {}

        def cached(key, make):
            if key not in pkc:
                pkc[key] = make()
            return pkc[key]
        if coupling_po_ok(N, C, Cc_, Hd, H, W, w1, w3) and int(w2.shape[2]) == 1:
            def make_po():
                plan = POPackPlan([(w1.detach(), w2.detach(), w3.detach())])
                plan.run()
                return plan.bufs[0]
            _, _, P, _ = coupling_po_fwd(z, cin2, cached("po", make_po), f(n1b), f(n1l), f(n2b), f(n2l), C, act)
            o = torch.empty((N, C, H, W), device=x.device, dtype=torch.float32)
            b3f, l3f = f(b3), f(l3)
            L.call("rfn_tap_gather_f32", L.dev(P), L.dev(b3f), L.dev(l3f), L.dev(o), _i(N), _i(C), _i(H), _i(W))
        else:
            h1 = conv2d_raw(z[:, :Ch], cin2, cached(("w1", fp), lambda: pack_weight(w1, prec=fp)), Hd, int(w1.shape[2]), 1,
                            f(n1b), f(n1l), act, prec=fp)
            h2 = conv2d_raw(h1, None, cached(("w2", fp), lambda: pack_weight(w2, prec=fp)), Hd, int(w2.shape[2]), 1,
                            f(n2b), f(n2l), act, prec=fp)
            if zeros_conv_uses_taps(w3):
                C3, Cin3 = int(w3.shape[0]), int(w3.shape[1])
                pk3 = cached(("w3t", fp), lambda: pack_weight(
                    w3.detach().permute(2, 3, 0, 1).reshape(9 * C3, Cin3, 1, 1).contiguous(), prec=fp))
            else:
                pk3 = cached(("w3", fp), lambda: pack_weight(w3, prec=fp))
            o = zeros_conv_fwd(h2, w3, f(b3), f(l3), pk3, prec=fp)
        dlogdet = torch.zeros(N, device=x.device, dtype=torch.float32)
        affine_coupling_(z, o, f(scale), f(scale_shift), dlogdet, clamp_type, True)
        out = invconv_actnorm_rev(z, f(an_bias), f(an_logs), Winv.detach())
        ctx.mark_non_differentiable(out, dlogdet)
        return out, dlogdet


class GaussLogpFn(torch.autograd.Function):

    @staticmethod
    def forward(ctx, z, o, layout, std_mode):
        ctx.save_for_backward(z, o)
        ctx.cfg = (layout, std_mode)
        return gauss_logp(z, o, layout, std_mode)

    @staticmethod
    def backward(ctx, g):
        z, o = ctx.saved_tensors
        layout, std_mode = ctx.cfg
        N, Cz = z.shape[0], z.shape[1]
        gz = torch.empty(z.shape, device=z.device, dtype=torch.float32)
        go = torch.empty(o.shape, device=z.device, dtype=torch.float32)
        zp, zns = L.frames(z, "z")
        op, ons = L.frames(o, "o")
        gzp, gzns = L.frames(gz, "gz")
        gop, gons = L.frames(go, "go")
        L.call("rfn_gauss_logp_bwd_f32", zp, _l(zns), op, _l(ons), L.dev(g.contiguous()), gzp, _l(gzns), gop, _l(gons),
               _i(layout), _i(std_mode), _i(N), _i(Cz), _i(_hw(z)), meta=_shell("gauss_logp_bwd", z, 6))
        return gz, go, None, None


def smallmap_arith_ok(H, W):
    return CONV_PRECISION == "bf16x3" or (CONV_PRECISION == "mixed" and H * W <= 4)


def smallmap_supported(conv, H, W):
    return (smallmap_arith_ok(H, W) and tuple(conv.kernel_size) == (3, 3) and tuple(conv.stride) == (1, 1)
            and tuple(conv.padding) == (1, 1) and tuple(conv.dilation) == (1, 1) and conv.groups == 1
            and conv.bias is not None and H * W <= 16 and (conv.in_channels * H * W) % 8 == 0
            and (conv.out_channels * H * W) % 8 == 0)


def smallmap_pack(w, H, W, transpose):
    with PackBatch() as b:
        return b.dense(w, H, W, transpose)


def smallmap_dense(a, packed, n_channels, bias=None, slope_out=None, y=None, slope_in=0.0, want_a_out=False, add=None):
    a = a.contiguous()
    B, H, W = int(a.shape[0]), int(a.shape[2]), int(a.shape[3])
    K, HW = int(a.shape[1]) * H * W, H * W
    out = torch.empty((B, n_channels, H, W), device=a.device, dtype=torch.float32)
    a_out = torch.empty_like(a) if want_a_out else None
    yc = None if y is None else y.contiguous()
    addc = None if add is None else add.contiguous()
    L.call("rfn_smallmap_dense_bf16x3", L.dev(a), L.dev(yc), ctypes.c_float(slope_in), L.dev(packed), L.dev(bias),
           L.dev(addc), _i(0 if slope_out is None else 1), ctypes.c_float(0.0 if slope_out is None else slope_out), L.dev(out),
           L.dev(a_out), _i(B), _i(K), _i(n_channels * HW), _i(HW))
    return (out, a_out) if want_a_out else out


def smallmap_dense_pair(a0, packed0, n_ch0, a1, packed1, n_ch1, bias0=None, bias1=None, slope_out0=None, slope_out1=None,
                        y0=None, y1=None, slope_in0=0.0, slope_in1=0.0, want_a_out=False, add0=None, add1=None):
    a0, a1 = a0.contiguous(), a1.contiguous()
    B, H, W = int(a0.shape[0]), int(a0.shape[2]), int(a0.shape[3])
    assert int(a1.shape[0]) == B and tuple(a1.shape[2:]) == (H, W)
    HW = H * W
    K0, K1 = int(a0.shape[1]) * HW, int(a1.shape[1]) * HW
    out0 = torch.empty((B, n_ch0, H, W), device=a0.device, dtype=torch.float32)
    out1 = torch.empty((B, n_ch1, H, W), device=a0.device, dtype=torch.float32)
    ao0 = torch.empty_like(a0) if want_a_out and y0 is not None else None
    ao1 = torch.empty_like(a1) if want_a_out and y1 is not None else None
    y0c = None if y0 is None else y0.contiguous()
    y1c = None if y1 is None else y1.contiguous()
    ad0 = None if add0 is None else add0.contiguous()
    ad1 = None if add1 is None else add1.contiguous()
    fl = ctypes.c_float
    L.call("rfn_smallmap_dense_pair_bf16x3",
           L.dev(a0), L.dev(y0c), fl(slope_in0), L.dev(packed0), L.dev(bias0), L.dev(ad0), _i(0 if slope_out0 is None else 1),
           fl(0.0 if slope_out0 is None else slope_out0), L.dev(out0), L.dev(ao0), _i(K0), _i(n_ch0 * HW),
           L.dev(a1), L.dev(y1c), fl(slope_in1), L.dev(packed1), L.dev(bias1), L.dev(ad1), _i(0 if slope_out1 is None else 1),
           fl(0.0 if slope_out1 is None else slope_out1), L.dev(out1), L.dev(ao1), _i(K1), _i(n_ch1 * HW), _i(B), _i(HW))
    if want_a_out:
        return out0, (ao0 if ao0 is not None else a0), out1, (ao1 if ao1 is not None else a1)
    return out0, out1


def smallmap_conv_ok(H, W, C1, C2, Cout, N, bwd=False):
    HW = H * W
    stream = -(-N // 32) * (C1 + C2) * HW * Cout * HW
    return ((bwd_b3() if bwd else smallmap_arith_ok(H, W)) and HW <= 16 and (C1 * HW) % 8 == 0 and ((C1 + C2) * HW) % 8 == 0
            and stream <= 32 * 1024 * 1024 and os.environ.get("RFN_SMALLMAP_GLOW") != "0")


def smallmap_conv(in1, in2, packed, Cout, ep_mode=0, p0=None, p1=None, act=0, out1=None, out2=None, cout_split=None,
                  acc1=False, acc2=False):
    N, C1, H, W = in1.shape
    C2 = 0 if in2 is None else int(in2.shape[1])
    if cout_split is None:
        cout_split = Cout
    if out1 is None:
        out1 = torch.empty((N, cout_split, H, W), device=in1.device, dtype=torch.float32)
    i1p, i1ns = L.frames(in1, "in1")
    i2p, i2ns = (None, 0) if in2 is None else L.frames(in2, "in2")
    o1p, o1ns = L.frames(out1, "out1")
    o2p, o2ns = (None, 0) if out2 is None else L.frames(out2, "out2")
    L.call("rfn_smallmap_conv_bf16x3", i1p, _l(i1ns), _i(C1), i2p, _l(i2ns), _i(C2), L.dev(packed), o1p, _l(o1ns), o2p,
           _l(o2ns), _i(Cout), _i(cout_split), _i((1 if acc1 else 0) | (2 if acc2 else 0)), _i(N), _i(H), _i(W), _i(ep_mode), L.dev(p0),
           L.dev(p1), _i(act),
           meta=("conv", "smallmap_dense_kernel", 2.0 * N * H * W * (C1 + C2) * Cout * 9,
                 "N%d %d+%d->%d %dx%d k3 ep%d dense" % (N, C1, C2, Cout, H, W, ep_mode),
                 4.0 * (N * H * W * (C1 + C2 + Cout) + (C1 + C2) * Cout * H * W * H * W)))
    return out1


INVCONV_MAX_STEPS, INVCONV_MAX_CHANNELS = 32, 96


def invconv_weights_ok(ics):
    return (0 < len(ics) <= INVCONV_MAX_STEPS and all(ic.LU_decomposed for ic in ics) and ics[0].lower.is_cuda
            and int(ics[0].lower.shape[0]) <= INVCONV_MAX_CHANNELS and os.environ.get("RFN_INVCONV_KERNEL") != "0")


class InvConvWeightsFn(torch.autograd.Function):

    @staticmethod
    def _pointers(P, S, Lw, U, LS):
        out = []
        for grp, nm in ((P, "p"), (Lw, "lower"), (U, "upper"), (LS, "log_s"), (S, "sign_s")):
            for x in grp:
                L.dev(x, nm)
            out.append(L.ptr_array(list(grp), nm))
        return out

    @staticmethod
    def forward(ctx, hw, Kn, *t):
        ctx.set_materialize_grads(False)
        P, S, Lw, U, LS = (t[i * Kn:(i + 1) * Kn] for i in range(5))
        C = int(Lw[0].shape[0])
        arrs = InvConvWeightsFn._pointers(P, S, Lw, U, LS)
        W = torch.empty((Kn, C, C), device=Lw[0].device, dtype=torch.float32)
        c = torch.empty((), device=Lw[0].device, dtype=torch.float32)
        L.call("rfn_invconv_weights_fwd_f32", *arrs, L.dev(W), L.dev(c), _i(Kn), _i(C), _i(int(hw)),
               meta=_shell("invconv_weights_fwd", W, 4))
        ctx.cfg = (int(hw), Kn, C)
        ctx.save_for_backward(*t)
        return W, c

    @staticmethod
    def backward(ctx, gW, gc):
        hw, Kn, C = ctx.cfg
        t = ctx.saved_tensors
        P, S, Lw, U, LS = (t[i * Kn:(i + 1) * Kn] for i in range(5))
        dev_ = Lw[0].device
        if gW is None:
            gW = torch.zeros((Kn, C, C), device=dev_, dtype=torch.float32)
        arrs = InvConvWeightsFn._pointers(P, S, Lw, U, LS)
        gl = torch.empty((Kn, C, C), device=dev_, dtype=torch.float32)
        gu = torch.empty((Kn, C, C), device=dev_, dtype=torch.float32)
        gs = torch.empty((Kn, C), device=dev_, dtype=torch.float32)
        gcc = None if gc is None else gc.contiguous()
        L.call("rfn_invconv_weights_bwd_f32", *arrs, L.dev(gW.contiguous()), L.dev(gcc), L.dev(gl), L.dev(gu), L.dev(gs),
               _i(Kn), _i(C), _i(hw), meta=_shell("invconv_weights_bwd", gW, 4))
        return (None, None) + (None,) * (2 * Kn) + tuple(gl.unbind(0)) + tuple(gu.unbind(0)) + tuple(gs.unbind(0))


class LatentStepFn(torch.autograd.Function):

    @staticmethod
    def forward(ctx, enc, pri, eps_p, eps_q, res_q):
        ctx.set_materialize_grads(False)
        B = int(enc.shape[0])
        shp = (B, enc.shape[1] // 2) + tuple(enc.shape[2:])
        ZHW = 1
        for d in shp[1:]:
            ZHW *= int(d)
        enc, pri, eps_p, eps_q = enc.contiguous(), pri.contiguous(), eps_p.contiguous(), eps_q.contiguous()
        outs = [torch.empty(shp, device=enc.device, dtype=torch.float32) for _ in range(5)]
        L.call("rfn_latent_step_fwd_f32", L.dev(enc), L.dev(pri), L.dev(eps_p), L.dev(eps_q), *[L.dev(o) for o in outs],
               _i(B), _i(ZHW), _i(1 if res_q else 0), meta=_shell("latent_step_fwd", enc, 5.5))
        ctx.save_for_backward(enc, pri, eps_p, eps_q)
        ctx.cfg = (B, ZHW, bool(res_q))
        return tuple(outs)

    @staticmethod
    def backward(ctx, g_zt, g_zxt, g_kl, g_em, g_es):
        enc, pri, eps_p, eps_q = ctx.saved_tensors
        B, ZHW, res_q = ctx.cfg
        strided, keep = [], []
        for g in (g_zt, g_zxt):
            if g is None:
                strided += [None, _l(0)]
                continue
            if B > 0 and (not g[0].is_contiguous() or (B > 1 and g.stride(0) < ZHW)):
                g = g.contiguous()
            keep.append(g)
            gp, gns = L.frames(g, "g_z")
            strided += [gp, _l(gns)]
        gs = [None if g is None else g.contiguous() for g in (g_kl, g_em, g_es)]
# ... 418 lines not shown
```

Baseline: 10920 frames/s.

## Split grouped wgrad stages across workgroups instead of one grid slice per group

Grouped weight-gradient GEMM kernels now flatten all groups' K-stages into a single range and hand each workgroup a contiguous slice, which may cross group boundaries. The grid no longer multiplies by G. Each part rebases its row pointers, reads operands from the kernarg segment, re-primes the pipeline and atomically adds its partial sums. This aims to balance work when many groups each have few stages, at the cost of extra pipeline restarts and atomics at part boundaries. The Python gating for grouped wgrad also changes from a pixel-count threshold to a memory-budget check based on retained bytes.

```diff
diff --git a/include/rfn_hip.h b/include/rfn_hip.h
--- a/include/rfn_hip.h
+++ b/include/rfn_hip.h
@@ -145,6 +145,8 @@
                                               long in1_ns, int C1, const float* const* in2, long in2_ns, int C2,
                                               float* const* gw, int G, int F, int H, int W, rfn_stream_t stream);
 const char* rfn_conv3x3_wgrad_implicit_kernel_label_bf16x3(int Cout, long g_ns, int G, int F, int H, int W);
+int rfn_wgrad_split_workgroups(int tiles, int G, int n_stages);
+int rfn_wgrad_split_parts(int G, int n_stages, int Wt, int w, long long* parts, int max_parts);
 int rfn_im2col3x3_f32(const float* in1, long in1_ns, int C1, const float* in2, long in2_ns, int C2, float* out, int N,
                       int H, int W, rfn_stream_t stream);
 
diff --git a/recurrent-flows-msc_amd/csrc/wgrad_bf16x3.hip b/recurrent-flows-msc_amd/csrc/wgrad_bf16x3.hip
--- a/recurrent-flows-msc_amd/csrc/wgrad_bf16x3.hip
+++ b/recurrent-flows-msc_amd/csrc/wgrad_bf16x3.hip
@@ -35,6 +35,38 @@
             }
     }
     return o;
+}
+__device__ __forceinline__ WgOperands wg_operands_kernarg(const int grp) {
+    typedef const GemmWgradParams __attribute__((address_space(4))) KernargParams;
+    KernargParams* kp = (KernargParams*)__builtin_amdgcn_kernarg_segment_ptr();
+    WgOperands o = {kp->ga[grp], kp->gb[grp], kp->gb2[grp], kp->ggw[grp]};
+    return o;
+}
+template <class Kern>
+constexpr bool wg_sole_argument(Kern) { return std::is_same<Kern, void (*)(GemmWgradParams)>::value; }
+__device__ __forceinline__ const float* wg_rebase(const float* q, const float* from, const float* to) {
+    return reinterpret_cast<const float*>((uintptr_t)q - (uintptr_t)from + (uintptr_t)to);
+}
+
+struct WgPart { int grp, s0, cnt; };
+__host__ __device__ inline long wg_split_begin(int G, int n_stages, int Wt, int w) {
+    return (long)w * ((long)G * n_stages) / Wt;
+}
+__host__ __device__ inline bool wg_split_part(int G, int n_stages, int Wt, int w, long& pos, WgPart& part) {
+    const long end = (long)(w + 1) * ((long)G * n_stages) / Wt;
+    if (pos >= end) return false;
+    const long g = pos / n_stages;
+    part.grp = (int)g;
+    part.s0 = (int)(pos - g * n_stages);
+    const long left = end - pos, in_group = (long)n_stages - part.s0;
+    part.cnt = (int)(left < in_group ? left : in_group);
+    pos += part.cnt;
+    return true;
+}
+__host__ __device__ inline int wg_split_workgroups(int tiles, int G, int n_stages) {
+    long Wt = 256 / tiles, cap = (long)G * n_stages / 8;
+    if (Wt > cap) Wt = cap;
+    return Wt < 1 ? 1 : (int)Wt;
 }
 
 template <int WM, int WN, int TM, int TN, int KP, int IMPL = 0>
@@ -267,20 +299,12 @@
     const int wave = __builtin_amdgcn_readfirstlane(tid >> 6);
     const int wm = wave / WN, wn = wave % WN;
     const int l31 = lane & 31, kk = lane >> 5;
-    const int grp = p.G > 0 ? (int)blockIdx.z / p.mtiles : 0;
-    const int m0 = (p.G > 0 ? (int)blockIdx.z - grp * p.mtiles : (int)blockIdx.z) * BM, n0 = blockIdx.y * BN;
-    const WgOperands ops_ = wg_operands(p, grp);
-    const float* const pa_ = ops_.a;
-    const float* const pb_ = ops_.b;
-    float* const pgw_ = ops_.gw;
+    const int m0 = blockIdx.z * BM, n0 = blockIdx.y * BN;
+    const float* pa_ = p.a;
+    const float* pb_ = p.b;
+    float* pgw_ = p.gw;
 
     f32x16 acc[TM][TN];
-#pragma unroll
-    for (int i = 0; i < TM; ++i)
-#pragma unroll
-        for (int j = 0; j < TN; ++j)
-#pragma unroll
-            for (int r = 0; r < 16; ++r) acc[i][j][r] = 0.f;
 
     const float* prow[PPW];
     bool pisa[PPW];
@@ -301,11 +325,11 @@
     }
     const unsigned uHW = (unsigned)p.HW;
     const int S = gridDim.x;
-    const int nmine = (p.n_stages - (int)blockIdx.x + S - 1) / S;
+    int first = blockIdx.x, step = S, nmine = (p.n_stages - (int)blockIdx.x + S - 1) / S;
     long offa = 0, offb = 0;
     auto stage_offsets = [&](int t) {
         t = t < nmine ? t : nmine - 1;
-        const unsigned q0 = (unsigned)(blockIdx.x + t * S) * KP;
+        const unsigned q0 = (unsigned)(first + t * step) * KP;
         const unsigned f = q0 / uHW, px = q0 - f * uHW;
         offa = (long)f * p.a_ns + px;
         offb = (long)f * p.b_ns + px;
@@ -333,12 +357,6 @@
         r[1] = *reinterpret_cast<const f32x4*>(sb + (o ^ 16));
     };
 
-#pragma unroll
-    for (int t = 0; t < NST - 1; ++t) {
-        stage_offsets(t);
-#pragma unroll
-        for (int j = 0; j < PPW; ++j) piece(j, t);
-    }
     f32x4 ra[2][2], rb[TN][2];
     bf16x8 ah[2], al[2], bh[2][TN], bl[2][TN];
     auto first_fragments = [&](const unsigned char* sb0) {
@@ -350,85 +368,121 @@
         for (int j = 0; j < TN; ++j) wg_split8(rb[j][0], rb[j][1], bh[0][j], bl[0][j]);
         wg_split8(ra[0][0], ra[0][1], ah[0], al[0]);
     };
-    if (LOOK) {
-        wg_wait_vm<(NST - 2) * PPW>();
-        __builtin_amdgcn_s_barrier();
-        first_fragments(lds_raw);
-    }
-
-    int slot = 0;
-    for (int it = 0; it < nmine; ++it) {
-        wg_wait_vm<LOOK ? (NST - 3) * PPW : 0>();
-        __builtin_amdgcn_s_barrier();
-        const int nslot = slot + 1 == NST ? 0 : slot + 1;
-        const int fslot = slot == 0 ? NST - 1 : slot - 1;
-        const unsigned char* sb = lds_raw + slot * STAGE;
-        const unsigned char* sn = lds_raw + nslot * STAGE;
-        stage_offsets(it + NST - 1);
-        if (!LOOK) {
-#pragma unroll
-            for (int j = 0; j < PPW; ++j) piece(j, fslot);
-            first_fragments(sb);
-        }
-#pragma unroll
-        for (int u = 0; u < NU_; ++u) {
-            const int s_ = u / TM, i = u % TM, cur = u & 1, kb = s_ & 1;
-            if (u + 2 < NU_) raw(sb, aoff[(u + 2) % TM], (u + 2) / TM, ra[cur]);
-            else if (LOOK) raw(sn, aoff[(u + 2) % TM], 0, ra[cur]);
-            if (i == 0) {
+
+    WgPart part;
+    long pos = p.G > 0 ? wg_split_begin(p.G, p.n_stages, S, blockIdx.x) : 0;
+    for (int part_i = 0; p.G > 0 ? wg_split_part(p.G, p.n_stages, S, blockIdx.x, pos, part) : part_i == 0; ++part_i) {
+        if (p.G > 0) {
+            const WgOperands o = wg_operands_kernarg(part.grp);
+#pragma unroll
+            for (int j = 0; j < PPW; ++j) prow[j] = pisa[j] ? wg_rebase(prow[j], pa_, o.a) : wg_rebase(prow[j], pb_, o.b);
+            pa_ = o.a;
+            pb_ = o.b;
+            pgw_ = o.gw;
+            first = part.s0;
+            step = 1;
+            nmine = part.cnt;
+        }
+        if (part_i > 0) {
+            wg_wait_vm<0>();
+            asm volatile("s_waitcnt lgkmcnt(0)" ::: "memory");
+            __builtin_amdgcn_s_barrier();
+        }
+#pragma unroll
+        for (int i = 0; i < TM; ++i)
+#pragma unroll
+            for (int j = 0; j < TN; ++j)
+#pragma unroll
+                for (int r = 0; r < 16; ++r) acc[i][j][r] = 0.f;
+
+#pragma unroll
+        for (int t = 0; t < NST - 1; ++t) {
+            stage_offsets(t);
+#pragma unroll
+            for (int j = 0; j < PPW; ++j) piece(j, t);
+        }
+        if (LOOK) {
+            wg_wait_vm<(NST - 2) * PPW>();
+            __builtin_amdgcn_s_barrier();
+            first_fragments(lds_raw);
+        }
+
+        int slot = 0;
+        for (int it = 0; it < nmine; ++it) {
+            wg_wait_vm<LOOK ? (NST - 3) * PPW : 0>();
+            __builtin_amdgcn_s_barrier();
+            const int nslot = slot + 1 == NST ? 0 : slot + 1;
+            const int fslot = slot == 0 ? NST - 1 : slot - 1;
+            const unsigned char* sb = lds_raw + slot * STAGE;
+            const unsigned char* sn = lds_raw + nslot * STAGE;
+            stage_offsets(it + NST - 1);
+            if (!LOOK) {
+#pragma unroll
+                for (int j = 0; j < PPW; ++j) piece(j, fslot);
+                first_fragments(sb);
+            }
+#pragma unroll
+            for (int u = 0; u < NU_; ++u) {
+                const int s_ = u / TM, i = u % TM, cur = u & 1, kb = s_ & 1;
+                if (u + 2 < NU_) raw(sb, aoff[(u + 2) % TM], (u + 2) / TM, ra[cur]);
+                else if (LOOK) raw(sn, aoff[(u + 2) % TM], 0, ra[cur]);
+                if (i == 0) {
+#pragma unroll
+                    for (int j = 0; j < TN; ++j) {
+                        if (s_ + 1 < NK) raw(sb, boff[j], s_ + 1, rb[j]);
+                        else if (LOOK) raw(sn, boff[j], 0, rb[j]);
+                    }
+                }
+                if (LOOK && u == 0) {
+#pragma unroll
+                    for (int j = 0; j < PPW; ++j) piece(j, fslot);
+                }
 #pragma unroll
                 for (int j = 0; j < TN; ++j) {
-                    if (s_ + 1 < NK) raw(sb, boff[j], s_ + 1, rb[j]);
-                    else if (LOOK) raw(sn, boff[j], 0, rb[j]);
-                }
-            }
-            if (LOOK && u == 0) {
-#pragma unroll
-                for (int j = 0; j < PPW; ++j) piece(j, fslot);
-            }
+                    acc[i][j] = __builtin_amdgcn_mfma_f32_32x32x16_bf16(al[cur], bh[kb][j], acc[i][j], 0, 0, 0);
+                    acc[i][j] = __builtin_amdgcn_mfma_f32_32x32x16_bf16(ah[cur], bl[kb][j], acc[i][j], 0, 0, 0);
+                    acc[i][j] = __builtin_amdgcn_mfma_f32_32x32x16_bf16(ah[cur], bh[kb][j], acc[i][j], 0, 0, 0);
+                }
+                if (LOOK || u + 1 < NU_) wg_split8(ra[cur ^ 1][0], ra[cur ^ 1][1], ah[cur ^ 1], al[cur ^ 1]);
+                if (i >= 1 && i <= TN && (LOOK || s_ + 1 < NK))
+                    wg_split8(rb[i - 1][0], rb[i - 1][1], bh[kb ^ 1][i - 1], bl[kb ^ 1][i - 1]);
+            }
+            if (LOOK && (NK & 1)) {
+#pragma unroll
+                for (int j = 0; j < TN; ++j) {
+                    bh[0][j] = bh[1][j];
+                    bl[0][j] = bl[1][j];
+                }
+            }
+            if (!LOOK) {
+                __builtin_amdgcn_sched_group_barrier(0x020, PPW, 0);
+                __builtin_amdgcn_sched_group_barrier(0x100, 2 * TN + 4, 0);
+                __builtin_amdgcn_sched_group_barrier(0x002, 30 * (TN + 1), 0);
+            }
+#pragma unroll
+            for (int g = 0; g < NU_ * TN * 3; ++g) {
+                __builtin_amdgcn_sched_group_barrier(0x008, 1, 0);
+                __builtin_amdgcn_sched_group_barrier(0x002, 6, 0);
+                __builtin_amdgcn_sched_group_barrier(0x100, 1, 0);
+                if (LOOK && g < PPW) __builtin_amdgcn_sched_group_barrier(0x020, 1, 0);
+            }
+            slot = nslot;
+        }
+        wg_wait_vm<0>();
+        int m0e = m0, n0e = n0;
+        asm volatile("" : "+s"(m0e), "+s"(n0e));
+#pragma unroll
+        for (int i = 0; i < TM; ++i)
 #pragma unroll
             for (int j = 0; j < TN; ++j) {
-                acc[i][j] = __builtin_amdgcn_mfma_f32_32x32x16_bf16(al[cur], bh[kb][j], acc[i][j], 0, 0, 0);
-                acc[i][j] = __builtin_amdgcn_mfma_f32_32x32x16_bf16(ah[cur], bl[kb][j], acc[i][j], 0, 0, 0);
-                acc[i][j] = __builtin_amdgcn_mfma_f32_32x32x16_bf16(ah[cur], bh[kb][j], acc[i][j], 0, 0, 0);
-            }
-            if (LOOK || u + 1 < NU_) wg_split8(ra[cur ^ 1][0], ra[cur ^ 1][1], ah[cur ^ 1], al[cur ^ 1]);
-            if (i >= 1 && i <= TN && (LOOK || s_ + 1 < NK))
-                wg_split8(rb[i - 1][0], rb[i - 1][1], bh[kb ^ 1][i - 1], bl[kb ^ 1][i - 1]);
-        }
-        if (LOOK && (NK & 1)) {
-#pragma unroll
-            for (int j = 0; j < TN; ++j) {
-                bh[0][j] = bh[1][j];
-                bl[0][j] = bl[1][j];
-            }
-        }
-        if (!LOOK) {
-            __builtin_amdgcn_sched_group_barrier(0x020, PPW, 0);
-            __builtin_amdgcn_sched_group_barrier(0x100, 2 * TN + 4, 0);
-            __builtin_amdgcn_sched_group_barrier(0x002, 30 * (TN + 1), 0);
-        }
-#pragma unroll
-        for (int g = 0; g < NU_ * TN * 3; ++g) {
-            __builtin_amdgcn_sched_group_barrier(0x008, 1, 0);
-            __builtin_amdgcn_sched_group_barrier(0x002, 6, 0);
-            __builtin_amdgcn_sched_group_barrier(0x100, 1, 0);
-            if (LOOK && g < PPW) __builtin_amdgcn_sched_group_barrier(0x020, 1, 0);
-        }
-        slot = nslot;
-    }
-    wg_wait_vm<0>();
-#pragma unroll
-    for (int i = 0; i < TM; ++i)
-#pragma unroll
-        for (int j = 0; j < TN; ++j) {
-            const int n = n0 + (wn * TN + j) * 32 + l31;
-#pragma unroll
-            for (int r = 0; r < 16; ++r) {
-                const int m = m0 + (wm * TM + i) * 32 + (r & 3) + 8 * (r >> 2) + 4 * kk;
-                if (m < p.M && n < p.N) atomicAdd(&pgw_[(long)m * p.N + n], acc[i][j][r]);
-            }
-        }
+                const int n = n0e + (wn * TN + j) * 32 + l31;
+#pragma unroll
+                for (int r = 0; r < 16; ++r) {
+                    const int m = m0e + (wm * TM + i) * 32 + (r & 3) + 8 * (r >> 2) + 4 * kk;
+                    if (m < p.M && n < p.N) atomicAdd(&pgw_[(long)m * p.N + n], acc[i][j][r]);
+                }
+            }
+    }
 }
 
 template <int WM, int WN, int TM, int TN, int KP, int NST>
@@ -437,14 +491,12 @@
     p.n_stages = (int)(p.total / KP);
     const size_t lds = (size_t)NST * (BM + BN) * KP * 4;
     const int tiles = ceil_div(p.M, BM) * ceil_div(p.N, BN);
-    const int G = p.G > 0 ? p.G : 1;
-    int S = 256 / (tiles * G);
-    if (S > p.n_stages / 8) S = p.n_stages / 8;
-    if (S < 1) S = 1;
+    const int S = wg_split_workgroups(tiles, p.G > 0 ? p.G : 1, p.n_stages);
     auto kern = gemm_wgrad_dma_kernel<WM, WN, TM, TN, KP, NST>;
+    static_assert(wg_sole_argument(decltype(kern){}), "wg_operands_kernarg reads p from the kernel-argument segment");
     (void)hipFuncSetAttribute((const void*)kern, hipFuncAttributeMaxDynamicSharedMemorySize, (int)lds);
     p.mtiles = ceil_div(p.M, BM);
-    dim3 grid(S, ceil_div(p.N, BN), p.mtiles * G);
+    dim3 grid(S, ceil_div(p.N, BN), p.mtiles);
     hipLaunchKernelGGL(kern, grid, dim3(64 * WM * WN), lds, s, p);
 }
 
@@ -464,21 +516,13 @@
     const int wave = __builtin_amdgcn_readfirstlane(tid >> 6);
     const int wm = wave / WN, wn = wave % WN;
     const int l31 = lane & 31, kk = lane >> 5;
-    const int grp = p.G > 0 ? (int)blockIdx.z / p.mtiles : 0;
-    const int m0 = (p.G > 0 ? (int)blockIdx.z - grp * p.mtiles : (int)blockIdx.z) * BM, n0 = blockIdx.y * BN;
-    const WgOperands ops_ = wg_operands(p, grp);
-    const float* const pa_ = ops_.a;
-    const float* const pb_ = ops_.b;
-    const float* const pb2_ = ops_.b2;
-    float* const pgw_ = ops_.gw;
+    const int m0 = blockIdx.z * BM, n0 = blockIdx.y * BN;
+    const float* pa_ = p.a;
+    const float* pb_ = p.b;
+    const float* pb2_ = p.b2;
+    float* pgw_ = p.gw;
 
     f32x16 acc[TM][TN];
-#pragma unroll
-    for (int i = 0; i < TM; ++i)
-#pragma unroll
-        for (int j = 0; j < TN; ++j)
-#pragma unroll
-            for (int r = 0; r < 16; ++r) acc[i][j][r] = 0.f;
 
     const float* prow[PPW];
 #pragma unroll
@@ -499,6 +543,7 @@
     const float* uplane[BU];
     long uns[BU];
     int udy[BU], udx[BU];
+    bool uin1[BU];
 #pragma unroll
     for (int u = 0; u < BU; ++u) {
         int row = n0 + r0 + u * (NT / NU);
@@ -506,19 +551,19 @@
         const int ci = row / 9, tap = row - ci * 9;
         udy[u] = tap / 3 - 1;
         udx[u] = tap % 3 - 1;
-        const bool first = ci < p.C1;
-        uplane[u] = first ? pb_ + (long)ci * p.HW : pb2_ + (long)(ci - p.C1) * p.HW;
-        uns[u] = first ? p.b_ns : p.b2_ns;
+        uin1[u] = ci < p.C1;
+        uplane[u] = uin1[u] ? pb_ + (long)ci * p.HW : pb2_ + (long)(ci - p.C1) * p.HW;
+        uns[u] = uin1[u] ? p.b_ns : p.b2_ns;
     }
     const unsigned uHW = (unsigned)p.HW;
     const int S = gridDim.x;
-    const int nmine = (p.n_stages - (int)blockIdx.x + S - 1) / S;
+    int first = blockIdx.x, step = S, nmine = (p.n_stages - (int)blockIdx.x + S - 1) / S;
     float4 bst[BU][2];
     float bedge[BU];
     unsigned rowmask = 0, edgemask = 0;
     auto fetch = [&](int t, const int slot) {
         t = t < nmine ? t : nmine - 1;
-        const unsigned q0 = (unsigned)(blockIdx.x + t * S) * KP;
+        const unsigned q0 = (unsigned)(first + t * step) * KP;
         const unsigned f = q0 / uHW, px = q0 - f * uHW;
         const long offa = (long)f * p.a_ns + px;
 #pragma unroll
@@ -577,64 +622,96 @@
     };
     const int brow = (wn * TN * 32 + l31) * RS + kk;
 
-    fetch(0, 0);
-    commit(0);
-    int slot = 0;
-    for (int it = 0; it < nmine; ++it) {
+    WgPart part;
+    long pos = p.G > 0 ? wg_split_begin(p.G, p.n_stages, S, blockIdx.x) : 0;
+    for (int part_i = 0; p.G > 0 ? wg_split_part(p.G, p.n_stages, S, blockIdx.x, pos, part) : part_i == 0; ++part_i) {
+        if (p.G > 0) {
+            const WgOperands o = wg_operands_kernarg(part.grp);
+#pragma unroll
+            for (int j = 0; j < PPW; ++j) prow[j] = wg_rebase(prow[j], pa_, o.a);
+#pragma unroll
+            for (int u = 0; u < BU; ++u) uplane[u] = uin1[u] ? wg_rebase(uplane[u], pb_, o.b) : wg_rebase(uplane[u], pb2_, o.b2);
+            pa_ = o.a;
+            pb_ = o.b;
+            pb2_ = o.b2;
+            pgw_ = o.gw;
+            first = part.s0;
+            step = 1;
+            nmine = part.cnt;
+        }
+        if (part_i > 0) {
+            wg_wait_vm<0>();
+            asm volatile("s_waitcnt lgkmcnt(0)" ::: "memory");
+            __builtin_amdgcn_s_barrier();
+        }
+#pragma unroll
+        for (int i = 0; i < TM; ++i)
+#pragma unroll
+            for (int j = 0; j < TN; ++j)
+#pragma unroll
+                for (int r = 0; r < 16; ++r) acc[i][j][r] = 0.f;
+
+        fetch(0, 0);
+        commit(0);
+        int slot = 0;
+        for (int it = 0; it < nmine; ++it) {
+            wg_wait_vm<0>();
+            asm volatile("s_waitcnt lgkmcnt(0)" ::: "memory");
+            __builtin_amdgcn_s_barrier();
+            fetch(it + 1, slot ^ 1);
+            const unsigned char* sb = lds_raw + slot * ASLOT;
+            const bf16x8* Bh = Bbase + slot * 2 * BPLANE;
+            const bf16x8* Bl = Bh + BPLANE;
+            f32x4 ra[2][TM][2];
+            bf16x8 ah[2][TM], al[2][TM];
+#pragma unroll
+            for (int i = 0; i < TM; ++i) rawA(sb, i, 0, ra[0][i]);
+#pragma unroll
+            for (int i = 0; i < TM; ++i) wg_split8(ra[0][i][0], ra[0][i][1], ah[0][i], al[0][i]);
+#pragma unroll
+            for (int s_ = 0; s_ < NK; ++s_) {
+                const int cur = s_ & 1;
+                if (s_ + 1 < NK) {
+#pragma unroll
+                    for (int i = 0; i < TM; ++i) rawA(sb, i, s_ + 1, ra[cur ^ 1][i]);
+                }
+                bf16x8 bh[TN], bl[TN];
+#pragma unroll
+                for (int j = 0; j < TN; ++j) {
+                    bh[j] = Bh[brow + j * 32 * RS + 2 * s_];
+                    bl[j] = Bl[brow + j * 32 * RS + 2 * s_];
+                }
+#pragma unroll
+                for (int i = 0; i < TM; ++i)
+#pragma unroll
+                    for (int j = 0; j < TN; ++j) {
+                        acc[i][j] = __builtin_amdgcn_mfma_f32_32x32x16_bf16(al[cur][i], bh[j], acc[i][j], 0, 0, 0);
+                        acc[i][j] = __builtin_amdgcn_mfma_f32_32x32x16_bf16(ah[cur][i], bl[j], acc[i][j], 0, 0, 0);
+                        acc[i][j] = __builtin_amdgcn_mfma_f32_32x32x16_bf16(ah[cur][i], bh[j], acc[i][j], 0, 0, 0);
+                    }
+                if (s_ + 1 < NK) {
+#pragma unroll
+                    for (int i = 0; i < TM; ++i) wg_split8(ra[cur ^ 1][i][0], ra[cur ^ 1][i][1], ah[cur ^ 1][i], al[cur ^ 1][i]);
+                }
+            }
+            commit(slot ^ 1);
+            slot ^= 1;
+        }
         wg_wait_vm<0>();
-        asm volatile("s_waitcnt lgkmcnt(0)" ::: "memory");
-        __builtin_amdgcn_s_barrier();
-        fetch(it + 1, slot ^ 1);
-        const unsigned char* sb = lds_raw + slot * ASLOT;
-        const bf16x8* Bh = Bbase + slot * 2 * BPLANE;
-        const bf16x8* Bl = Bh + BPLANE;
-        f32x4 ra[2][TM][2];
-        bf16x8 ah[2][TM], al[2][TM];
-#pragma unroll
-        for (int i = 0; i < TM; ++i) rawA(sb, i, 0, ra[0][i]);
-#pragma unroll
-        for (int i = 0; i < TM; ++i) wg_split8(ra[0][i][0], ra[0][i][1], ah[0][i], al[0][i]);
-#pragma unroll
-        for (int s_ = 0; s_ < NK; ++s_) {
-            const int cur = s_ & 1;
-            if (s_ + 1 < NK) {
-#pragma unroll
-                for (int i = 0; i < TM; ++i) rawA(sb, i, s_ + 1, ra[cur ^ 1][i]);
-            }
-            bf16x8 bh[TN], bl[TN];
+        int m0e = m0, n0e = n0;
+        asm volatile("" : "+s"(m0e), "+s"(n0e));
+#pragma unroll
+        for (int i = 0; i < TM; ++i)
 #pragma unroll
             for (int j = 0; j < TN; ++j) {
-                bh[j] = Bh[brow + j * 32 * RS + 2 * s_];
-                bl[j] = Bl[brow + j * 32 * RS + 2 * s_];
-            }
-#pragma unroll
-            for (int i = 0; i < TM; ++i)
-#pragma unroll
-                for (int j = 0; j < TN; ++j) {
-                    acc[i][j] = __builtin_amdgcn_mfma_f32_32x32x16_bf16(al[cur][i], bh[j], acc[i][j], 0, 0, 0);
-                    acc[i][j] = __builtin_amdgcn_mfma_f32_32x32x16_bf16(ah[cur][i], bl[j], acc[i][j], 0, 0, 0);
-                    acc[i][j] = __builtin_amdgcn_mfma_f32_32x32x16_bf16(ah[cur][i], bh[j], acc[i][j], 0, 0, 0);
-                }
-            if (s_ + 1 < NK) {
-#pragma unroll
-                for (int i = 0; i < TM; ++i) wg_split8(ra[cur ^ 1][i][0], ra[cur ^ 1][i][1], ah[cur ^ 1][i], al[cur ^ 1][i]);
-            }
-        }
-        commit(slot ^ 1);
-        slot ^= 1;
-    }
-    wg_wait_vm<0>();
-#pragma unroll
-    for (int i = 0; i < TM; ++i)
-#pragma unroll
-        for (int j = 0; j < TN; ++j) {
-            const int n = n0 + (wn * TN + j) * 32 + l31;
-#pragma unroll
-            for (int r = 0; r < 16; ++r) {
-                const int m = m0 + (wm * TM + i) * 32 + (r & 3) + 8 * (r >> 2) + 4 * kk;
-                if (m < p.M && n < p.N) atomicAdd(&pgw_[(long)m * p.N + n], acc[i][j][r]);
-            }
-        }
+                const int n = n0e + (wn * TN + j) * 32 + l31;
+#pragma unroll
+                for (int r = 0; r < 16; ++r) {
+                    const int m = m0e + (wm * TM + i) * 32 + (r & 3) + 8 * (r >> 2) + 4 * kk;
+                    if (m < p.M && n < p.N) atomicAdd(&pgw_[(long)m * p.N + n], acc[i][j][r]);
+                }
+            }
+    }
 }
 
 template <int WM, int WN, int TM, int TN>
@@ -643,14 +720,12 @@
     p.n_stages = (int)(p.total / 32);
     const size_t lds = (size_t)2 * BM * 128 + (size_t)2 * 2 * BN * 5 * 16;
     const int tiles = ceil_div(p.M, BM) * ceil_div(p.N, BN);
-    const int G = p.G > 0 ? p.G : 1;
-    int S = 256 / (tiles * G);
-    if (S > p.n_stages / 8) S = p.n_stages / 8;
-    if (S < 1) S = 1;
+    const int S = wg_split_workgroups(tiles, p.G > 0 ? p.G : 1, p.n_stages);
     auto kern = gemm_wgrad_dma_impl_kernel<WM, WN, TM, TN>;
+    static_assert(wg_sole_argument(decltype(kern){}), "wg_operands_kernarg reads p from the kernel-argument segment");
     (void)hipFuncSetAttribute((const void*)kern, hipFuncAttributeMaxDynamicSharedMemorySize, (int)lds);
     p.mtiles = ceil_div(p.M, BM);
-    dim3 grid(S, ceil_div(p.N, BN), p.mtiles * G);
+    dim3 grid(S, ceil_div(p.N, BN), p.mtiles);
     hipLaunchKernelGGL(kern, grid, dim3(64 * WM * WN), lds, s, p);
 }
 
@@ -728,6 +803,23 @@
 }
 extern "C" const char* rfn_conv3x3_wgrad_implicit_kernel_label_bf16x3(int Cout, long g_ns, int G, int F, int H, int W) {
     return kWgradB3Labels[choose_wgrad_implicit(wgrad_shape(Cout, 0, g_ns, 0, G, F, H * W))];
+}
+
+extern "C" int rfn_wgrad_split_workgroups(int tiles, int G, int n_stages) {
+    RFN_CHECK_ARG(tiles >= 1 && G >= 1 && G <= 16 && n_stages >= 1, -1);
+    return wg_split_workgroups(tiles, G, n_stages);
+}
+extern "C" int rfn_wgrad_split_parts(int G, int n_stages, int Wt, int w, long long* parts, int max_parts) {
+    RFN_CHECK_ARG(G >= 1 && G <= 16 && n_stages >= 1 && Wt >= 1 && w >= 0 && w < Wt && (parts || max_parts == 0), -1);
+    int n = 0;
+    WgPart part;
+    for (long pos = wg_split_begin(G, n_stages, Wt, w); wg_split_part(G, n_stages, Wt, w, pos, part); ++n)
+        if (n < max_parts) {
+            parts[3 * n] = part.grp;
+            parts[3 * n + 1] = part.s0;
+            parts[3 * n + 2] = part.cnt;
+        }
+    return n;
 }
 
 static void launch_wgrad_route(GemmWgradParams& p, WgradB3Route r, hipStream_t s) {
diff --git a/recurrent-flows-msc_amd/rfn_hip/lib.py b/recurrent-flows-msc_amd/rfn_hip/lib.py
--- a/recurrent-flows-msc_amd/rfn_hip/lib.py
+++ b/recurrent-flows-msc_amd/rfn_hip/lib.py
@@ -76,6 +76,8 @@
                                           _c_s],
     "rfn_gemm_wgrad_kernel_label_bf16x3": [_c_i, _c_i, _c_l, _c_l, _c_i, _c_i, _c_i],
     "rfn_conv3x3_wgrad_implicit_kernel_label_bf16x3": [_c_i, _c_l, _c_i, _c_i, _c_i, _c_i],
+    "rfn_wgrad_split_workgroups": [_c_i, _c_i, _c_i],
+    "rfn_wgrad_split_parts": [_c_i, _c_i, _c_i, _c_i, ctypes.c_void_p, _c_i],
     "rfn_im2col3x3_f32": [_c_f, _c_l, _c_i, _c_f, _c_l, _c_i, _c_f, _c_i, _c_i, _c_i, _c_s],
     "rfn_packed_weight_size": [_c_i, _c_i, _c_i],
     "rfn_pack_conv_weight_f32": [_c_f, _c_f, _c_i, _c_i, _c_i, _c_i, _c_s],
diff --git a/recurrent-flows-msc_amd/rfn_hip/ops.py b/recurrent-flows-msc_amd/rfn_hip/ops.py
--- a/recurrent-flows-msc_amd/rfn_hip/ops.py
+++ b/recurrent-flows-msc_amd/rfn_hip/ops.py
@@ -427,7 +427,26 @@
     return gw
 
 
-GROUPED_WGRAD_MAX_PIX = 100000
+_grouped_wgrad_budget = {}
+
+
+def grouped_wgrad_budget(device):
+    env = os.environ.get("RFN_WGRAD_GROUPED_MAX_BYTES")
+    if env is not None:
+        return int(env)
+    idx = device.index if device.index is not None else torch.cuda.current_device()
+    if idx not in _grouped_wgrad_budget:
+        _grouped_wgrad_budget[idx] = torch.cuda.get_device_properties(idx).total_memory // 8
+    return _grouped_wgrad_budget[idx]
+
+
+def grouped_wgrad_retained_bytes(Kn, N, Hd, HW, o_numel):
+    return 4 * Kn * (2 * N * Hd * HW + o_numel)
+
+
+def group_level_wgrad(Kn, N, Hd, HW, o_numel, device):
+    return (1 < Kn <= 16 and os.environ.get("RFN_WGRAD_GROUPED") != "0" and
+            grouped_wgrad_retained_bytes(Kn, N, Hd, HW, o_numel) <= grouped_wgrad_budget(device))
 
 
 def conv2d_wgrad_grouped(in1_list, in2_list, g_list, Cout, ks, arena=None, g_stacked=None):
@@ -969,15 +988,12 @@
         gcond = torch.empty_like(cond) if Cc > 0 else torch.zeros_like(cond)
         grads = [None] * nf
         (_, _, _, _, _, _, _, _, _, _, l3, scale, scale_shift) = prm[Kn - 1]
-        go_all = (torch.empty((Kn,) + tuple(os_[0].shape), device=x.device, dtype=torch.float32)
-                  if (N * HW <= GROUPED_WGRAD_MAX_PIX and 1 < Kn <= 16 and os.environ.get("RFN_WGRAD_GROUPED") != "0")
-                  else None)
+        grouped = group_level_wgrad(Kn, N, int(w1.shape[0]), HW, os_[0].numel(), x.device)
+        go_all = torch.empty((Kn,) + tuple(os_[0].shape), device=x.device, dtype=torch.float32) if grouped else None
         gz, go, gscale, gshift, gb3, gl3 = _affine_zeros_bwd(outs[Kn - 1], os_[Kn - 1], gout, gdl, scale, scale_shift, l3,
                                                             clamp_type, arena, None if go_all is None else go_all[Kn - 1])
         gx = None
-        defer = ({"w1": [], "w2": [], "w3": []}
-                 if (N * HW <= GROUPED_WGRAD_MAX_PIX and 1 < Kn <= 16 and os.environ.get("RFN_WGRAD_GROUPED") != "0")
-                 else None)
+        defer = {"w1": [], "w2": [], "w3": []} if grouped else None
         for k in range(Kn - 1, -1, -1):
             (an_bias, an_logs, w1, n1b, n1l, w2, n2b, n2l, w3, b3, l3, scale, scale_shift) = prm[k]
             nfin = len(fin)
```

New measurement: 11470 frames/s, median of 6. 5.1% higher.
